# skycrapers/TecoGAN-PyTorch

Measured on AMD Instinct MI355X. Metric: HR frames/sec/GPU at 4xSR 3x134x320 LR; Vid4 PSNR vs reference, higher is better.
Workload: dtype f32; 1 GPU; TecoGAN 4xSR BD generator-only inference (FRNet.infer_sequence) of a synthetic 2140-frame 3x134x320 LR clip -> 3x536x1280 HR uint8, 1 clip/GPU, random-init weights (BASELINE configs[1]); a step = one recurrent frame; parallelism=clip-sharded x1, no data-path collective, launches_per_frame=29

## Files before the change

### include/tecogan_hip.h

```cpp
#ifndef TECOGAN_HIP_H
#define TECOGAN_HIP_H

#include <stddef.h>
#include <stdint.h>

#ifdef __cplusplus
extern "C" {
#endif

typedef void* tg_stream_t;

enum {
  TG_OK = 0,
  TG_E_SHAPE = -1,
  TG_E_ARG = -2,
  TG_E_HIP = -3
};

enum {
  TG_ACT_NONE = 0,
  TG_ACT_RELU = 1,
  TG_ACT_LRELU02 = 2,
  TG_ACT_TANH24 = 3
};

enum {
  TG_UP_NONE = 0,
  TG_UP_BICUBIC = 1,
  TG_UP_BILINEAR = 2
};

#define TG_ABI_MAJOR 2
int tg_version(void);
const char* tg_last_error_string(void);
const char* tg_build_info(void);

int tg_conv3x3_pick_ocb(int cout);
size_t tg_conv3x3_packed_floats(int cin, int cout, int ocb);
int tg_conv3x3_pack(const float* w, float* w_packed, int cin, int cout, int ocb,
                    int transposed, tg_stream_t stream);

int tg_conv3x3_fwd(
    const float* x, int64_t x_nstride, int c1,
    const float* x2, int64_t x2_nstride,
    const float* w_packed, int ocb, const float* bias ,
    const float* res, int64_t res_nstride,
    float* y, int64_t y_nstride,
    int n, int cin, int cout, int h, int w, int act, tg_stream_t stream);

int tg_conv3x3_fwd_phased(const float* x, int64_t x_nstride, const float* w_packed, int ocb,
                          const float* bias, float* y, int64_t y_nstride, int n, int cin,
                          int cout, int h, int w, int act, int tapsel, int cphase,
                          int taps_phase0, int taps_phase1, tg_stream_t stream);
int tg_conv4x4s2_supported(int n, int ci, int co, int h, int w);
size_t tg_conv4x4s2_packed_floats(int ci, int co);
int tg_conv4x4s2_pack(const float* w, float* w_fwd, float* w_dgrad, int ci, int co, tg_stream_t stream);
size_t tg_conv4x4s2_workspace_floats(int n, int ci, int co, int h, int w, int dgrad);
int tg_conv4x4s2_fwd(const float* x, const float* w_fwd, float* y, float* workspace, int n, int ci, int co, int h, int w,
                     tg_stream_t stream);
int tg_conv4x4s2_dgrad(const float* g, const float* w_dgrad, const float* act_y, int act, float* dx, float* workspace,
                       int n, int ci, int co, int h, int w, tg_stream_t stream);
int tg_conv3x3s2_supported(int n, int cin, int cout, int h_out, int w_out);
int tg_conv3x3s2_fwd(const float* x, int64_t x_nstride, const float* w_packed, const float* bias,
                     const float* relu_mask, int64_t mask_nstride, float* y, int64_t y_nstride, int n,
                     int cin, int cout, int h_out, int w_out, int act, tg_stream_t stream);
int tg_conv3x3_fwd_phased_masked(const float* x, int64_t x_nstride, const float* w_packed, int ocb,
                                 const float* bias, const float* relu_mask, int64_t mask_nstride,
                                 float* y, int64_t y_nstride, int n, int cin, int cout, int h, int w,
                                 int act, int tapsel, int cphase, int taps_phase0, int taps_phase1,
                                 tg_stream_t stream);
int tg_conv3x3_phased_pick_ksplit(int n, int cin, int cout, int h, int w, int ocb);
int tg_conv3x3_fwd_phased_splitk(const float* x, int64_t x_nstride, const float* w_packed, int ocb,
                                 const float* bias, float* y, int n, int cin, int cout, int h, int w,
                                 int act, int tapsel, int cphase, int taps_phase0, int taps_phase1,
                                 int ksplit, float* partials, tg_stream_t stream);
int tg_conv3x3_fwd_masked(const float* x, int64_t x_nstride, int c1, const float* x2,
                          int64_t x2_nstride, const float* w_packed, int ocb,
                          const float* bias, const float* res, int64_t res_nstride,
                          const float* relu_mask, int64_t mask_nstride, float* y,
                          int64_t y_nstride, int n, int cin, int cout, int h, int w, int act,
                          tg_stream_t stream);

int64_t tg_conv3x3_wino_packed_floats(int cin, int cout);
int tg_conv3x3_prefers_wino(int n, int cin, int cout, int h, int w);
int tg_pack_conv3x3_wino(const float* w, float* out, int cin, int cout, int transposed,
                         tg_stream_t stream);
int tg_conv3x3_wino_fwd(const float* x, int64_t x_nstride, int c1, const float* x2,
                        int64_t x2_nstride, const float* u_packed, const float* bias,
                        const float* res, int64_t res_nstride, const float* relu_mask,
                        int64_t mask_nstride, float* y, int64_t y_nstride, int n, int cin,
                        int cout, int h, int w, int act, tg_stream_t stream);

typedef struct {
  const float* x; const float* x2; const float* u_packed; const float* bias; const float* res;
  float* y;
  int64_t x_nstride, x2_nstride, res_nstride, y_nstride;
  int c1, cin, act;
} tg_wino_layer;
int64_t tg_conv3x3_wino_chain_flag_ints(int n_layers, int n, int h, int w);
int tg_conv3x3_wino_chain(const tg_wino_layer* layers, int n_layers, int n, int cout, int h, int w,
                          int32_t* flags, int epoch, tg_stream_t stream);

int tg_conv3x3_wino_resident_supported(int n, int cout, int h, int w);
int64_t tg_conv3x3_wino_resident_ws_bytes(int h, int w);
int tg_conv3x3_wino_resident(const tg_wino_layer* layers, int n_layers, int cout, int h, int w,
                             void* workspace, int epoch, tg_stream_t stream);
typedef struct tg_wres_convt {
  const float* u_packed;
  const float* bias;
  float* y;
  int act;
} tg_wres_convt;
size_t tg_conv3x3_wino_resident_ct_floats(void);
int tg_conv3x3_wino_resident_ct_pack(const float* w_iohw, float* out, tg_stream_t stream);
int tg_conv3x3_wino_resident_ct(const tg_wino_layer* layers, int n_layers, int cout, int h, int w,
                                void* workspace, int epoch, const tg_wres_convt* convt, tg_stream_t stream);

typedef struct {
  const float* x; const float* x2; const float* w_packed; const float* bias; const float* res;
  const float* relu_mask;
  float* y;
  int64_t x_nstride, x2_nstride, res_nstride, mask_nstride, y_nstride;
  int c1, cin, cout, act;
} tg_chain_layer;
int64_t tg_conv3x3_chain_flag_ints(int n_layers, int n, int h, int w);
int tg_conv3x3_chain_supported(int n, int h, int w, int cmax);
size_t tg_conv3x3_pack16_floats(void);
int tg_conv3x3_pack16(const float* w, float* w_packed, int cin, int cout, int transposed, tg_stream_t stream);
typedef struct tg_pack_item {
  const float* w;
  float* out;
  int cin, cout, transposed, i_total, i_off;
} tg_pack_item;
size_t tg_conv3x3_chain_packed_floats(int pack_layout, int cin);
int tg_conv3x3_chain_pack(const tg_pack_item* items, int n_items, int pack_layout, tg_stream_t stream);
int tg_conv3x3_chain(const tg_chain_layer* layers, int n_layers, int n, int h, int w, int pack_layout,
                     int32_t* flags, int32_t* err, uint32_t epoch, int poll_limit, tg_stream_t stream);
typedef struct { const float* w; const float* b; } tg_packed_layer;
int tg_srnet_body_fwd(const tg_packed_layer* layers, int pack_layout, int nb, const float* lr, int c_lr,
                      const float* tran, int c_tran, float* acts, int n, int nf, int h, int w, int32_t* flags,
                      int32_t* err, uint32_t epoch, int poll_limit, tg_stream_t stream);
int tg_srnet_body_bwd(const tg_packed_layer* dgrad, int pack_layout, int nb, const float* acts, float* dz,
                      float* d_tran, int c_tran, int n, int nf, int h, int w, int32_t* flags, int32_t* err,
                      uint32_t epoch, int poll_limit, tg_stream_t stream);

size_t tg_wgrad3x3_body_workspace_floats(int nframes, int n_per_frame, int nlayers, int c, int h, int w);
int tg_wgrad3x3_body(const float* const* dz_bases, const float* const* act_bases, int nframes, int64_t layer_stride, int nlayers, float* const* grads, float* workspace,
                     int n_per_frame, int c, int h, int w, int accumulate, tg_stream_t stream);
int tg_wgrad3x3_body_bias(const float* const* dz_bases, const float* const* act_bases, int nframes,
                          int64_t layer_stride, int nlayers, float* const* grads, float* const* dbs,
                          float* workspace, int n_per_frame, int c, int h, int w, int accumulate,
                          tg_stream_t stream);
int tg_bias_grad_body(const float* const* dz_bases, int nframes,
                      int64_t layer_stride, int nlayers, float* const* dbs, int n_per_frame, int c, int hw,
                      tg_stream_t stream);

int tg_conv3x3_pick_ksplit(int n, int cin, int cout, int h, int w);
int tg_conv3x3_splitk_fwd(const float* x, int64_t x_nstride, int c1, const float* x2,
                          int64_t x2_nstride, const float* w_packed, int ocb,
                          const float* bias, float* y, int n, int cin, int cout, int h,
                          int w, int act, int ksplit, float* partials, int pool,
                          tg_stream_t stream);

int tg_convt3x3s2_fwd(const float* x, int64_t x_nstride, const float* w_packed,
                      const float* bias, float* y, int64_t y_nstride, int n,
                      int cin, int cout, int h, int w, int act,
                      tg_stream_t stream);
int tg_convt_pack_wz(const float* w_out_oihw, float* wz, int cz, int nf, tg_stream_t stream);
int tg_convt3x3s2_z_fwd(const float* x, int64_t x_nstride, const float* w_packed,
                        const float* bias, const float* wz, int cz, float* z,
                        int64_t z_nstride, int n, int cin, int cout, int h, int w, int act,
                        tg_stream_t stream);
int tg_convt3x3s2_z_fwd_form(const float* x, int64_t x_nstride, const float* w_packed,
                             const float* bias, const float* wz, int cz, float* z,
                             int64_t z_nstride, int n, int cin, int cout, int h, int w, int act,
                             int form, tg_stream_t stream);
#define TG_CONVT_WINO_FLOATS (16 * 64 * 64)
int tg_convt_pack_wino(const float* w_packed, float* w_wino, int cin, int cout, tg_stream_t stream);
int tg_convt3x3s2_z_wino_fwd(const float* x, int64_t x_nstride, const float* w_wino, const float* bias,
                             const float* wz, int cz, float* z, int64_t z_nstride, int n, int cin, int cout,
                             int h, int w, int act, int split, tg_stream_t stream);
int tg_convout_tail(const float* z, int64_t z_nstride, int cz, const float* bias,
                    const float* up_src, int up_mode, int up_scale, float* y,
                    int64_t y_nstride, uint8_t* u8_out, int n, int h, int w,
                    tg_stream_t stream);
int tg_convout_tail_form(const float* z, int64_t z_nstride, int cz, const float* bias,
                         const float* up_src, int up_mode, int up_scale, float* y,
                         int64_t y_nstride, uint8_t* u8_out, int n, int h, int w, int form,
                         tg_stream_t stream);

int tg_conv3x3_small_fwd(const float* x, int64_t x_nstride, const float* w_oihw,
                         const float* bias, const float* up_src, int up_mode,
                         int up_scale, float* y, int64_t y_nstride, int n,
                         int cin, int cout, int h, int w, int act,
                         tg_stream_t stream);
int tg_conv3x3_small_fwd_u8(const float* x, int64_t x_nstride, const float* w_oihw,
                            const float* bias, const float* up_src, int up_mode,
                            int up_scale, float* y, int64_t y_nstride, uint8_t* u8_out,
                            int n, int cin, int cout, int h, int w, int act,
                            tg_stream_t stream);
int tg_conv3x3_small_can_fuse_u8(const float* x, int64_t x_nstride, const float* y,
                                 int64_t y_nstride, int n, int cin, int h, int w);
int tg_conv3x3_fewin_fwd(const float* x, int64_t x_nstride, const float* w_oihw, const float* relu_mask,
                         int64_t mask_nstride, float* y, int64_t y_nstride, int n, int cin, int cout,
                         int h, int w, tg_stream_t stream);
int tg_conv3x3_small_fwd_res(const float* x, int64_t x_nstride, const float* w_oihw, const float* bias,
                             const float* res, int64_t res_nstride, float* y, int64_t y_nstride, int n,
                             int cin, int cout, int h, int w, int act, tg_stream_t stream);

int tg_flowup_warp_s2d_fwd(const float* lr_flow, int fh, int fw,
                           const float* hr_prev, float* out,
                           int64_t out_nstride, float* hr_flow_out, int n,
                           int c, int h, int w, int scale, int up_mode,
                           tg_stream_t stream);
int tg_copy_ceiling(const void* src, void* dst, int64_t bytes, int blocks, int threads, tg_stream_t stream);

int tg_backward_warp_fwd(const float* x, const float* flow, float* y, int n,
                         int c, int h, int w, tg_stream_t stream);

int tg_space_to_depth(const float* x, float* y, int64_t y_nstride, int n, int c,
                      int h, int w, int scale, tg_stream_t stream);

int tg_upsample_fwd(const float* x, float* y, int nc, int h, int w, int scale,
                    int up_mode, float mul, tg_stream_t stream);

int tg_maxpool2_fwd(const float* x, float* y, int nc, int h, int w,
                    tg_stream_t stream);

int tg_quantize_u8_hwc(const float* x, uint8_t* y, int c, int h, int w,
                       tg_stream_t stream);

int tg_dequantize_u8_hwc(const uint8_t* x, float* y, int n, int c, int h, int w,
                         tg_stream_t stream);

int tg_psnr_sse_u8(const uint8_t* true_hwc, const uint8_t* pred_hwc, uint64_t* sse,
                   int frames, int h, int w, int y_only, tg_stream_t stream);
int tg_luma_u8(const uint8_t* rgb, uint8_t* y, int64_t n, tg_stream_t stream);

int tg_lpips_conv_fwd(const void* x0, const void* x1, int n0, const float* lut, const float* wt,
                      const float* bias, float* y, int n, int cin, int h, int w, int cout, int ks,
                      int stride, int pad, tg_stream_t stream);
int tg_maxpool3s2_fwd(const float* x, float* y, int nc, int h, int w, tg_stream_t stream);
int64_t tg_lpips_head_workspace_bytes(int frames, int h, int w);
int tg_lpips_head(const float* feat_true, const float* feat_pred, const float* lin, int frames, int c,
// ... 210 lines not shown
```

### tecogan-pytorch_amd/_lib.py

```python
import ctypes as C
import os

_HERE = os.path.dirname(os.path.abspath(__file__))
LIB_PATH = os.environ.get('TECOGAN_HIP_LIB') or os.path.join(_HERE, 'libtecogan_hip.so')

TG_OK = 0
ABI_MAJOR = 2
ACT_NONE, ACT_RELU, ACT_LRELU02, ACT_TANH24 = 0, 1, 2, 3
UP_NONE, UP_BICUBIC, UP_BILINEAR = 0, 1, 2
PREC_F32, PREC_F16 = 0, 1

P, I, I64, F, SZ = C.c_void_p, C.c_int, C.c_int64, C.c_float, C.c_size_t


class FrnetCfg(C.Structure):
    _fields_ = [(k, C.c_int) for k in
                ('in_nc', 'out_nc', 'nf', 'nb', 'scale', 'up_mode', 'n', 'h', 'w', 'fnet_only')]


class WinoLayer(C.Structure):
    _fields_ = [('x', C.c_void_p), ('x2', C.c_void_p), ('u_packed', C.c_void_p), ('bias', C.c_void_p),
                ('res', C.c_void_p), ('y', C.c_void_p), ('x_nstride', C.c_int64), ('x2_nstride', C.c_int64),
                ('res_nstride', C.c_int64), ('y_nstride', C.c_int64), ('c1', C.c_int), ('cin', C.c_int),
                ('act', C.c_int)]


class ChainLayer(C.Structure):
    _fields_ = [('x', C.c_void_p), ('x2', C.c_void_p), ('w_packed', C.c_void_p), ('bias', C.c_void_p),
                ('res', C.c_void_p), ('relu_mask', C.c_void_p), ('y', C.c_void_p),
                ('x_nstride', C.c_int64), ('x2_nstride', C.c_int64), ('res_nstride', C.c_int64),
                ('mask_nstride', C.c_int64), ('y_nstride', C.c_int64),
                ('c1', C.c_int), ('cin', C.c_int), ('cout', C.c_int), ('act', C.c_int)]


class PackedLayer(C.Structure):
    _fields_ = [('w', C.c_void_p), ('b', C.c_void_p)]


class PackItem(C.Structure):
    _fields_ = [('w', C.c_void_p), ('out', C.c_void_p), ('cin', C.c_int), ('cout', C.c_int), ('transposed', C.c_int),
                ('i_total', C.c_int), ('i_off', C.c_int)]


class WresConvT(C.Structure):
    _fields_ = [('u_packed', C.c_void_p), ('bias', C.c_void_p), ('y', C.c_void_p), ('act', C.c_int)]


class LayerWeights(C.Structure):
    _fields_ = [('w', C.c_void_p), ('b', C.c_void_p), ('u', C.c_void_p)]


SIGNATURES = {
    'tg_version': (I, []),
    'tg_last_error_string': (C.c_char_p, []),
    'tg_build_info': (C.c_char_p, []),
    'tg_conv3x3_pick_ocb': (I, [I]),
    'tg_conv3x3_packed_floats': (SZ, [I, I, I]),
    'tg_conv3x3_pack': (I, [P, P, I, I, I, I, P]),
    'tg_conv3x3_fwd': (I, [P, I64, I, P, I64, P, I, P, P, I64, P, I64, I, I, I, I, I, I, P]),
    'tg_conv3x3_fwd_phased': (I, [P, I64, P, I, P, P, I64, I, I, I, I, I, I, I, I, I, I, P]),
    'tg_conv3x3_fwd_phased_masked': (I, [P, I64, P, I, P, P, I64, P, I64, I, I, I, I, I, I, I, I, I, I, P]),
    'tg_conv3x3s2_supported': (I, [I, I, I, I, I]),
    'tg_conv3x3s2_fwd': (I, [P, I64, P, P, P, I64, P, I64, I, I, I, I, I, I, P]),
    'tg_conv3x3_fwd_masked': (I, [P, I64, I, P, I64, P, I, P, P, I64, P, I64, P, I64, I, I, I, I, I, I, P]),
    'tg_conv3x3_pick_ksplit': (I, [I, I, I, I, I]),
    'tg_conv3x3_splitk_fwd': (I, [P, I64, I, P, I64, P, I, P, P, I, I, I, I, I, I, I, P, I, P]),
    'tg_convt3x3s2_fwd': (I, [P, I64, P, P, P, I64, I, I, I, I, I, I, P]),
    'tg_convt_pack_wz': (I, [P, P, I, I, P]),
    'tg_convt3x3s2_z_fwd': (I, [P, I64, P, P, P, I, P, I64, I, I, I, I, I, I, P]),
    'tg_convt3x3s2_z_fwd_form': (I, [P, I64, P, P, P, I, P, I64, I, I, I, I, I, I, I, P]),
    'tg_convt_pack_wino': (I, [P, P, I, I, P]),
    'tg_convt3x3s2_z_wino_fwd': (I, [P, I64, P, P, P, I, P, I64, I, I, I, I, I, I, I, P]),
    'tg_convout_tail': (I, [P, I64, I, P, P, I, I, P, I64, P, I, I, I, P]),
    'tg_convout_tail_form': (I, [P, I64, I, P, P, I, I, P, I64, P, I, I, I, I, P]),
    'tg_conv3x3_small_fwd': (I, [P, I64, P, P, P, I, I, P, I64, I, I, I, I, I, I, P]),
    'tg_conv3x3_fewin_fwd': (I, [P, I64, P, P, I64, P, I64, I, I, I, I, I, P]),
    'tg_conv3x3_small_fwd_res': (I, [P, I64, P, P, P, I64, P, I64, I, I, I, I, I, I, P]),
    'tg_conv3x3_small_fwd_u8': (I, [P, I64, P, P, P, I, I, P, I64, P, I, I, I, I, I, I, P]),
    'tg_conv3x3_small_can_fuse_u8': (I, [P, I64, P, I64, I, I, I, I]),
    'tg_flowup_warp_s2d_fwd': (I, [P, I, I, P, P, I64, P, I, I, I, I, I, I, P]),
    'tg_copy_ceiling': (I, [P, P, I64, I, I, P]),
    'tg_backward_warp_fwd': (I, [P, P, P, I, I, I, I, P]),
    'tg_space_to_depth': (I, [P, P, I64, I, I, I, I, I, P]),
    'tg_upsample_fwd': (I, [P, P, I, I, I, I, I, F, P]),
    'tg_maxpool2_fwd': (I, [P, P, I, I, I, P]),
    'tg_quantize_u8_hwc': (I, [P, P, I, I, I, P]),
    'tg_dequantize_u8_hwc': (I, [P, P, I, I, I, I, P]),
    'tg_psnr_sse_u8': (I, [P, P, P, I, I, I, I, P]),
    'tg_luma_u8': (I, [P, P, I64, P]),
    'tg_lpips_conv_fwd': (I, [P, P, I, P, P, P, P, I, I, I, I, I, I, I, I, P]),
    'tg_maxpool3s2_fwd': (I, [P, P, I, I, I, P]),
    'tg_lpips_head_workspace_bytes': (I64, [I, I, I]),
    'tg_lpips_head': (I, [P, P, P, I, I, I, I, P, P, I, P, P]),
    'tg_ssim_workspace_bytes': (I64, [I, I, I]),
    'tg_ssim_y_u8': (I, [P, P, I, I, I, I, I, I, I, I, I, P, P, SZ, P]),
    'tg_psnr_yfloat_partials': (I64, [I, I]),
    'tg_psnr_yfloat_sse_u8': (I, [P, P, I, I, I, I, I, I, I, I, I, P, P]),
    'tg_wgrad3x3_workspace_floats': (SZ, [I, I, I, I, I]),
    'tg_wgrad3x3': (I, [P, I64, P, I64, P, P, I, I, I, I, I, I, I, I, P]),
    'tg_wgrad3x3_multi': (I, [P, P, I, I64, I64, P, P, I, I, I, I, I, I, I, I, P]),
    'tg_wgrad3x3_multi_bias': (I, [P, P, I, I64, I64, P, P, P, I, I, I, I, I, I, I, I, P]),
    'tg_wgrad3x3_multi_phased': (I, [P, P, I, I64, I64, P, P, I, I, I, I, I, I, I, I, I, P]),
    'tg_conv3x3_phased_pick_ksplit': (I, [I, I, I, I, I, I]),
    'tg_conv3x3_fwd_phased_splitk': (I, [P, I64, P, I, P, P, I, I, I, I, I, I, I, I, I, I, I, P, P]),
    'tg_wgrad3x3_convt_workspace_floats': (SZ, [I, I, I, I, I]),
    'tg_wgrad3x3_convt_multi': (I, [P, P, I, P, P, P, I, I, I, I, I, I, P]),
    'tg_bias_grad_multi': (I, [P, I, P, I, I, I, I, P]),
    'tg_act_bwd': (I, [P, P, P, I64, I, P]),
    'tg_bias_grad': (I, [P, P, I, I, I, I, P]),
    'tg_maxpool2_bwd': (I, [P, P, P, I, I, I, P]),
    'tg_upsample_bwd': (I, [P, P, I, I, I, I, I, F, P]),
    'tg_backward_warp_bwd': (I, [P, P, P, P, P, I, I, I, I, P]),
    'tg_backward_warp_bwd_acc': (I, [P, P, P, P, P, I, I, I, I, P]),
    'tg_conv3x3_wino_resident_ct_floats': (SZ, []),
    'tg_conv3x3_wino_resident_ct_pack': (I, [P, P, P]),
    'tg_conv3x3_wino_resident_ct': (I, [P, I, I, I, I, P, I, P, P]),
    'tg_conv4x4s2_supported': (I, [I, I, I, I, I]),
    'tg_conv4x4s2_packed_floats': (SZ, [I, I]),
    'tg_conv4x4s2_pack': (I, [P, P, P, I, I, P]),
    'tg_conv4x4s2_workspace_floats': (SZ, [I, I, I, I, I, I]),
    'tg_conv4x4s2_fwd': (I, [P, P, P, P, I, I, I, I, I, P]),
    'tg_conv4x4s2_dgrad': (I, [P, P, P, I, P, P, I, I, I, I, I, P]),
    'tg_backward_warp_s2d_fwd': (I, [P, P, P, I, I, I, I, I, P]),
    'tg_backward_warp_s2d_bwd': (I, [P, P, P, P, I, P, I, I, I, I, I, P]),
    'tg_depth_to_space': (I, [P, P, I, I, I, I, I, P]),
    'tg_depth_to_space_act_bwd_supported': (I, [P, P, P, I, I]),
    'tg_depth_to_space_act_bwd': (I, [P, P, I, P, I, I, I, I, I, P]),
    'tg_charbonnier': (I, [P, P, I64, F, F, P, F, P, P]),
    'tg_channel_norm': (I, [P, P, P, P, I, I, I64, P]),
    'tg_cosine_loss': (I, [P, P, I, I, I64, F, F, P, F, P, P]),
    'tg_pixel_loss': (I, [P, P, I64, I, F, P, F, P, P]),
    'tg_bce_logits': (I, [P, I64, F, F, P, F, P, P]),
    'tg_lsgan_loss': (I, [P, I64, F, F, P, F, P, P]),
    'tg_adam_step': (I, [P, P, P, P, I64, F, F, F, F, F, I, P]),
    'tg_adam_step_guarded': (I, [P, P, P, P, I64, F, F, F, F, F, I, P, P]),
    'tg_fault_to_slot': (I, [P, P, P]),
    'tg_axpy': (I, [P, P, F, I64, P]),
    'tg_div_scalar': (I, [P, P, F, I64, P]),
    'tg_bn_lrelu_train_fwd': (I, [P, P, P, P, P, F, F, F, P, P, P, I, I, I, P]),
    'tg_bn_lrelu_train_bwd': (I, [P, P, P, P, P, P, F, P, P, P, I, P, I, I, I, P]),
    'tg_bn_local_stats': (I, [P, P, I, I, I, P]),
    'tg_bn_merge_stats': (I, [P, I, F, F, F, P, P, P, P, I, P]),
    'tg_bn_lrelu_apply': (I, [P, P, P, P, P, F, P, I, I, I, P]),
    'tg_bn_lrelu_bwd_reduce': (I, [P, P, P, P, P, F, P, I, I, I, P]),
    'tg_bn_lrelu_bwd_apply': (I, [P, P, P, P, P, P, P, F, F, P, I, I, I, P]),
    'tg_linear1_fwd': (I, [P, P, P, P, I, I, P]),
    'tg_linear1_bwd': (I, [P, P, P, P, P, P, I, I, I, P]),
    'tg_downsample_bd': (I, [P, P, P, I, I, I, I, I, I, P]),
    'tg_conv3x3_wino_packed_floats': (I64, [I, I]),
    'tg_conv3x3_wino_chain_flag_ints': (I64, [I, I, I, I]),
    'tg_conv3x3_wino_chain': (I, [C.POINTER(WinoLayer), I, I, I, I, I, P, I, P]),
    'tg_conv3x3_wino_resident_supported': (I, [I, I, I, I]),
    'tg_conv3x3_wino_resident_ws_bytes': (I64, [I, I]),
    'tg_conv3x3_wino_resident': (I, [C.POINTER(WinoLayer), I, I, I, I, P, I, P]),
    'tg_conv3x3_chain_flag_ints': (I64, [I, I, I, I]),
    'tg_conv3x3_chain_supported': (I, [I, I, I, I]),
    'tg_conv3x3_pack16_floats': (SZ, []),
    'tg_conv3x3_pack16': (I, [P, P, I, I, I, P]),
    'tg_conv3x3_chain_packed_floats': (SZ, [I, I]),
    'tg_conv3x3_chain_pack': (I, [P, I, I, P]),
    'tg_conv3x3_chain': (I, [C.POINTER(ChainLayer), I, I, I, I, I, P, P, C.c_uint32, I, P]),
    'tg_srnet_body_fwd': (I, [C.POINTER(PackedLayer), I, I, P, I, P, I, P, I, I, I, I, P, P, C.c_uint32, I, P]),
    'tg_srnet_body_bwd': (I, [C.POINTER(PackedLayer), I, I, P, P, P, I, I, I, I, I, P, P, C.c_uint32, I, P]),
    'tg_wgrad3x3_body_workspace_floats': (SZ, [I, I, I, I, I, I]),
    'tg_wgrad3x3_body': (I, [P, P, I, I64, I, P, P, I, I, I, I, I, P]),
    'tg_wgrad3x3_body_bias': (I, [P, P, I, I64, I, P, P, P, I, I, I, I, I, P]),
    'tg_bias_grad_body': (I, [P, I, I64, I, P, I, I, I, P]),
    'tg_conv3x3_prefers_wino': (I, [I, I, I, I, I]),
    'tg_pack_conv3x3_wino': (I, [P, P, I, I, I, P]),
    'tg_conv3x3_wino_fwd': (I, [P, I64, I, P, I64, P, P, P, I64, P, I64, P, I64, I, I, I, I, I, I, P]),
    'tg_time_gather': (I, [P, P, P, I, I, I, I64, P]),
    'tg_transpose01': (I, [P, P, I, I, I64, P]),
    'tg_stack_time': (I, [P, I, P, I, I64, P]),
    'tg_index_gather': (I, [P, P, P, I64, I64, I, P]),
    'tg_pingpong_grad': (I, [P, P, I, I, I64, P]),
    'tg_d_assemble_fwd': (I, [P, I, P, P, I, P, I, I, I, I, I, I, I, P]),
    'tg_d_assemble_bwd': (I, [P, P, I, P, I, I, I, I, I, I, I, P]),
    'tg_gather_clips_u8': (I, [P, P, P, P, I, I, I, I, P]),
    'tg_comm_get_unique_id': (I, [P]),
    'tg_comm_init_rank': (I, [P, I, I, C.POINTER(C.c_void_p)]),
    'tg_comm_destroy': (I, [P]),
    'tg_comm_world': (I, [P]),
    'tg_comm_rank': (I, [P]),
    'tg_comm_query': (I, [P, C.POINTER(C.c_int), C.POINTER(C.c_int)]),
    'tg_comm_library_origin': (C.c_char_p, []),
    'tg_allreduce_sum_f32': (I, [P, P, I64, P]),
    'tg_allgather_f32': (I, [P, P, P, I64, P]),
    'tg_frnet_workspace_floats': (SZ, [C.POINTER(FrnetCfg)]),
    'tg_frnet_plan_create': (I, [C.POINTER(FrnetCfg), C.POINTER(LayerWeights), I, P,
                                 C.POINTER(C.c_void_p)]),
    'tg_frnet_plan_destroy': (None, [P]),
    'tg_frnet_plan_chain_status': (I, [P, C.POINTER(C.c_int), C.POINTER(C.c_int)]),
    'tg_frnet_plan_set_chain_poll_limit': (I, [P, I]),
    'tg_frnet_plan_set_chain_rearm': (I, [P, I]),
    'tg_frnet_plan_chain_rearms': (I, [P, P, P]),
    'tg_frnet_step': (I, [P, P, P, P, P, P, P]),
    'tg_frnet_step_phase': (I, [P, I, I, P, P, P, P, P, P]),
    'tg_frnet_plan_launches': (I, [P]),
    'tg_frnet_plan_flow': (P, [P, I]),
    'tg_frnet_step_srnet': (I, [P, P, P, P, P, P, P]),
    'tg_frnet_plan_kinds': (I, []),
    'tg_frnet_kind_name': (C.c_char_p, [I]),
    'tg_frnet_plan_kind_stats': (I, [P, I, C.POINTER(C.c_int), C.POINTER(C.c_double),
                                     C.POINTER(C.c_double)]),
    'tg_frnet_replay': (I, [P, P, P, P, P, C.c_uint, I, P]),
    'tg_frnet_step_masked': (I, [P, P, P, P, P, P, C.c_uint, P]),
    'tg_conv3x3_f16_supported': (I, [I, I, I, I, I]),
    'tg_conv3x3_f16_packed_halves': (SZ, [I, I]),
    'tg_conv3x3_f16_act_halves': (I64, [I, I, I]),
    'tg_conv3x3_f16_pack_weights': (I, [P, I, I, I, P, P]),
    'tg_conv3x3_f16_pack_input': (I, [P, I64, I, P, I64, I, P, I, I, I, P]),
    'tg_conv3x3_f16_fwd': (I, [P, P, P, P, P, I, I, I, I, I, I, P]),
    'tg_convt3x3s2_f16_fwd': (I, [P, P, P, P, I64, I, I, I, I, I, I, P]),
    'tg_frnet_f16_workspace_bytes': (SZ, [C.POINTER(FrnetCfg)]),
    'tg_frnet_plan_set_precision': (I, [P, I, C.POINTER(LayerWeights), I, P]),
    'tg_frnet_plan_precision': (I, [P]),
}

_lib = None


class TecoganHipError(RuntimeError):
    pass


def lib():
    global _lib
    if _lib is None:
        if not os.path.isfile(LIB_PATH):
            raise TecoganHipError(
                f'{LIB_PATH} not found: build it with '
                f'`bash {os.path.join(_HERE, "csrc", "build.sh")}` '
                '(hipcc --offload-arch=gfx950).  There is no CPU/ATen fallback.')
        import torch
        handle = C.CDLL(LIB_PATH)
        handle.tg_version.restype = I
        if handle.tg_version() // 100 != ABI_MAJOR:
            raise TecoganHipError(f'{LIB_PATH}: ABI {handle.tg_version()} but this binding is written for '
                                  f'major {ABI_MAJOR} (include/tecogan_hip.h TG_ABI_MAJOR): rebuild the library')
        for name, (res, args) in SIGNATURES.items():
            fn = getattr(handle, name)
            fn.restype = res
            fn.argtypes = args
        _lib = handle
    return _lib


def check(rc, what):
    if rc != TG_OK:
        msg = lib().tg_last_error_string().decode('utf-8', 'replace')
        raise TecoganHipError(f'{what} failed (code {rc}): {msg}')
```

### tecogan-pytorch_amd/csrc/tg_api.hip

```cpp
#include <new>
#include <vector>

#include "tg_common.h"

namespace tg {
static thread_local char g_err[512] = "ok";
void set_error(const char* fmt, ...) {
  va_list ap;
  va_start(ap, fmt);
  vsnprintf(g_err, sizeof(g_err), fmt, ap);
  va_end(ap);
}
}

extern "C" int tg_version(void) { return TG_ABI_MAJOR * 100 + 1; }
extern "C" const char* tg_last_error_string(void) { return tg::g_err; }

#ifndef TG_BUILD_FLAGS_STR
#define TG_BUILD_FLAGS_STR "unknown (not built by csrc/build.sh)"
#endif
#ifndef TG_FILE_FLAGS_STR
#define TG_FILE_FLAGS_STR ""
#endif
namespace tg { int wres_lab_bits(); }
// ... 119 lines not shown
  off[5] = o; o += (c->scale == 4) ? sr * align64(n * c->nf * 16 * hw) : 0;
  off[6] = o; o += sr * align64(fnet_partial_floats(c));
  off[7] = o; o += align64(n * 64 * hw);
  off[8] = o; o += align64(n * 64 * hw);
  off[9] = o; o += align64(fnet_partial_floats(c));
  off[10] = o; o += align64(n * 2 * hw);
  off[11] = o; o += sr * (2048 + TG_CONVT_WINO_FLOATS);
  off[12] = o;
  o += sr * align64((size_t)CHAIN_MAX_LAYERS * n * ((c->h + 1) / 2) * ((c->w + 31) / 32) + 16);
  off[13] = o;
  {
    const int64_t rb = (sr && n == 1) ? tg::conv3x3_wino_resident_ws_bytes(c->h, c->w) : 0;
    o += align64((size_t)(rb + 3) / 4);
  }
  off[14] = o;
}

static int cfg_ok(const tg_frnet_cfg* c) {
  return c && c->in_nc == 3 && c->out_nc >= 1 && c->out_nc <= 4 && c->nf >= 1 && c->nf <= 64 &&
         c->nb >= 0 && (c->scale == 2 || c->scale == 4) &&
         (c->up_mode == TG_UP_BICUBIC || c->up_mode == TG_UP_BILINEAR) && c->n >= 1 &&
         c->h >= 8 && c->w >= 8;
}

extern "C" size_t tg_frnet_workspace_floats(const tg_frnet_cfg* cfg) {
  if (!cfg_ok(cfg)) return 0;
  size_t off[15];
  carve(cfg, off);
  return off[14];
}

extern "C" int tg_frnet_plan_create(const tg_frnet_cfg* cfg, const tg_layer_weights* layers,
                                    int n_layers, float* workspace, tg_frnet_plan** out) {
  TG_REQUIRE(cfg && layers && workspace && out, TG_E_ARG, "frnet_plan_create: null pointer");
  TG_REQUIRE(cfg_ok(cfg), TG_E_SHAPE,
             "frnet_plan_create: unsupported cfg (in_nc=3, out_nc<=4, nf<=64, scale 2|4, h,w>=8)");
  int nup = cfg->scale == 4 ? 2 : 1;
  int need = 14 + 1 + 2 * cfg->nb + nup + 1;
  TG_REQUIRE(n_layers == need, TG_E_ARG, "frnet_plan_create: %d layers given, %d expected",
             n_layers, need);
  for (int i = 0; i < n_layers; ++i)
    TG_REQUIRE(layers[i].w && layers[i].b, TG_E_ARG, "frnet_plan_create: layer %d null", i);
  tg_frnet_plan* p = new (std::nothrow) tg_frnet_plan();
  TG_REQUIRE(p, TG_E_ARG, "frnet_plan_create: out of host memory");
  p->cfg = *cfg;
  p->L.assign(layers, layers + n_layers);
  size_t off[15];
  carve(cfg, off);
  p->f16 = false; p->f16_ready = false; p->HWT = p->HA = p->HB = nullptr;
  p->WZ = workspace + off[11]; p->wz_ready = false;
  p->WA = p->WZ + 2048; p->wa_ready = false;
  p->RESWS = workspace + off[13]; p->res_ready = false;
  p->CHAINF = reinterpret_cast<int32_t*>(workspace + off[12]); p->chain_ready = false; p->epoch = 0; p->chain_layers = 0;
  p->chain_err = nullptr; p->chain_disabled = false; p->chain_faults = 0; p->chain_poll_limit = tg::TG_CHAIN_POLL_LIMIT_DEFAULT;
  p->rearm_first = 64; p->rearm_wait = 0; p->clean_frames = 0; p->rearms = 0; p->rearm_fence = nullptr; p->fence_set = false;
  if (!cfg->fnet_only) {
    void* hp = nullptr;
    if (hipHostMalloc(&hp, 64, hipHostMallocMapped | hipHostMallocCoherent) == hipSuccess && hp) {
      p->chain_err = static_cast<int32_t*>(hp);
      for (int i = 0; i < 16; ++i) p->chain_err[i] = 0;
    } else {
      (void)hipGetLastError();
    }
  }
  p->FA = workspace + off[7]; p->FB = workspace + off[8]; p->FPART = workspace + off[9];
  p->FLOW2 = workspace + off[10];
  p->PART = workspace + off[6];
  p->A = workspace + off[0]; p->B = workspace + off[1]; p->FLOW = workspace + off[2];
  p->S2D = workspace + off[3]; p->U1 = workspace + off[4];
  p->U2 = cfg->scale == 4 ? workspace + off[5] : nullptr;
  p->fh = cfg->h / 8 * 8; p->fw = cfg->w / 8 * 8;
  account(p);
  *out = p;
  return TG_OK;
}

extern "C" void tg_frnet_plan_destroy(tg_frnet_plan* plan) {
  if (!plan) return;
  if (plan->chain_err) (void)hipHostFree(plan->chain_err);
  if (plan->rearm_fence) (void)hipEventDestroy(plan->rearm_fence);
  delete plan;
}
extern "C" int tg_frnet_plan_launches(const tg_frnet_plan* plan) { return plan ? plan->launches : 0; }

enum {
  K_CONV64_R2 = 0,
  K_CONV64_R4 = 1,
  K_CONV32 = 2,
  K_CONVT = 3,
  K_SMALL = 4,
  K_WARP = 5,
  K_POOL = 6,
  K_UPSAMPLE = 7,
  K_QUANT = 8,
  K_FINAL = 9,
  K_CONV64_KS = 10,
  K_CONVT_Z = 11,
  K_TAIL = 12,
  K_CONV_ONESHOT = 13,
  K_CONV_WINO = 14,
  K_WINO_CHAIN = 15,
  K_WINO_RES = 16,
  K_F16_PACK = 17,
  K_F16_CONV = 18,
  K_F16_CONVT = 19,
  K_COUNT = 20
};

static bool hr_fuse_enabled() {
  static const int v = TG_LAB_ENV("TG_HR_FUSE", 1);
  return v != 0;
}
static bool convtz_wino_enabled() {
  static const int v = TG_LAB_ENV("TG_CONVTZ_WINO", 1);
  return v != 0;
}
static bool chain_wanted(long long ntile) {
  static const int v = [] { const char* e = getenv("TG_WINO_CHAIN"); return e && *e ? atoi(e) : -1; }();
  if (v >= 0) return v != 0;
  return ntile > 768 && ntile <= 3000;
}
static bool resident_wanted(bool layer_prefers_wino) {
  static const int v = [] { const char* e = getenv("TG_WINO_RES"); return e && *e ? atoi(e) : -1; }();
  return v >= 0 ? v != 0 : layer_prefers_wino;
}
static bool plan_u8_ok(const tg_frnet_plan* p) {
  if (p->f16 && p->cfg.scale == 2) return p->cfg.n == 1;
  return p->cfg.n == 1 || (hr_fuse_enabled() && p->cfg.out_nc <= 3 && p->cfg.nf <= 64);
}

static int step_impl(tg_frnet_plan* p, const float* lr_curr, const float* lr_prev,
                     const float* hr_prev, float* hr_out, uint8_t* u8_out, tg_stream_t st,
                     unsigned mask, bool dry, int phases, int slot, const float* flow_ext) {
  const tg_frnet_cfg& c = p->cfg;
  float* const flow_buf = flow_ext ? const_cast<float*>(flow_ext) : (slot ? p->FLOW2 : p->FLOW);
  bool active = (phases & 1) != 0;
  float* part_buf = p->FPART;
  const int n = c.n, h = c.h, w = c.w, s = c.scale;
  const int64_t hw = (int64_t)h * w;
  int li = 0;
  float *A = p->FA, *B = p->FB;
  int rc = TG_OK;
  if (!dry && (phases & 2) && mask == 0xFFFFFFFFu) chain_rearm_tick(p, st);
  auto go = [&](int kind, double flops, double bytes, auto&& fn) {
    if (rc != TG_OK) return;
    if (dry) {
      p->st_launch[kind] += 1; p->st_flops[kind] += flops; p->st_bytes[kind] += bytes;
      return;
    }
    if (active && (mask & (1u << kind))) rc = fn();
  };
  auto conv = [&](const float* x, int64_t xns, int c1, const float* x2, int64_t x2ns, int cin,
                  int cout, int hh, int ww, int act, const float* res, int64_t rns, float* y,
                  int64_t yns, bool pool = false, float* pool_tmp = nullptr) {
    const tg_layer_weights lw = p->L[li++];
    int ocb = tg_conv3x3_pick_ocb(cout);
    int kind = ocb == 32 ? K_CONV32
                         : (tg::conv3x3_rows_per_wg(ocb, (long long)n * hh * ww) == 4 ? K_CONV64_R4
                                                                                       : K_CONV64_R2);
    double px = (double)n * hh * ww;
    double fl = 2.0 * cin * 9 * cout * px;
    double by = 4.0 * px * (cin + cout + (res ? cout : 0)) + 4.0 * 9 * cin * cout;
    if (lw.u && tg_conv3x3_prefers_wino(n, cin, cout, hh, ww)) {
      float* yw = pool ? pool_tmp : y;
      go(K_CONV_WINO, fl, by, [&] {
        return tg::conv3x3_wino_launch(x, xns, c1, x2, x2ns, lw.u, lw.b, res, rns, nullptr, 0, yw,
                                       pool ? (int64_t)cout * hh * ww : yns, n, cin, cout, hh, ww, act, st);
      });
      if (pool)
        go(K_POOL, 0, 4.0 * n * cout * (hh * ww + (hh / 2) * (ww / 2)),
           [&] { return tg_maxpool2_fwd(yw, y, n * cout, hh, ww, st); });
      return;
    }
    int ks = res ? 1 : tg_conv3x3_pick_ksplit(n, cin, cout, hh, ww);
    if (ks == 1 && kind == K_CONV64_R2 && tg::conv3x3_uses_wg_ksplit(n, cin, cout, hh, ww))
      kind = tg::conv3x3_uses_oneshot(n, cin, cout, hh, ww) ? K_CONV_ONESHOT : K_CONV64_KS;
    if (ks > 1) {
      go(kind, fl, by, [&] {
        return tg::conv3x3_splitk_conv(x, xns, c1, x2, x2ns, lw.w, ocb, n, cin, cout, hh, ww, ks,
                                       part_buf, st);
      });
      go(K_FINAL, 0, 4.0 * px * cout * (ks + 1), [&] {
        return tg::conv3x3_splitk_finalize(part_buf, ks, lw.b, act, pool ? 1 : 0, y, n, cout, hh, ww,
                                           st);
      });
      return;
    }
    float* yc = pool ? pool_tmp : y;
    go(kind, fl, by, [&] {
      return tg_conv3x3_fwd(x, xns, c1, x2, x2ns, lw.w, ocb, lw.b, res, rns, yc,
                            pool ? (int64_t)cout * hh * ww : yns, n, cin, cout, hh, ww, act, st);
    });
    if (pool)
      go(K_POOL, 0, 4.0 * n * cout * (hh * ww + (hh / 2) * (ww / 2)),
         [&] { return tg_maxpool2_fwd(yc, y, n * cout, hh, ww, st); });
  };
  int hh = h, ww = w;
  const int enc[3] = {32, 64, 128};
  int cin = 2 * c.in_nc;
  const float* src = nullptr;
  for (int e = 0; e < 3; ++e) {
    int co = enc[e];
    if (e == 0)
      conv(lr_curr, c.in_nc * hw, c.in_nc, lr_prev, c.in_nc * hw, cin, co, hh, ww, TG_ACT_LRELU02,
           nullptr, 0, A, (int64_t)co * hh * ww);
    else
      conv(src, (int64_t)cin * hh * ww, cin, nullptr, 0, cin, co, hh, ww, TG_ACT_LRELU02, nullptr,
           0, A, (int64_t)co * hh * ww);
    conv(A, (int64_t)co * hh * ww, co, nullptr, 0, co, co, hh, ww, TG_ACT_LRELU02, nullptr, 0, A,
         (int64_t)co * (hh / 2) * (ww / 2), true, B);
    hh /= 2; ww /= 2; cin = co;
    float* t = A; A = B; B = t;
    src = B;
  }
  const int dec[3] = {256, 128, 64};
  for (int d = 0; d < 3; ++d) {
    int co = dec[d];
    conv(src, (int64_t)cin * hh * ww, cin, nullptr, 0, cin, co, hh, ww, TG_ACT_LRELU02, nullptr, 0,
         A, (int64_t)co * hh * ww);
    conv(A, (int64_t)co * hh * ww, co, nullptr, 0, co, co, hh, ww, TG_ACT_LRELU02, nullptr, 0, B,
         (int64_t)co * hh * ww);
    {
      float *pi = B, *po = A; int ph = hh, pw = ww;
      go(K_UPSAMPLE, 0, 4.0 * n * co * ph * pw * 5.0,
         [&] { return tg_upsample_fwd(pi, po, n * co, ph, pw, 2, TG_UP_BILINEAR, 1.0f, st); });
    }
    hh *= 2; ww *= 2; cin = co;
    float* t = A; A = B; B = t;
    src = B;
  }
  conv(src, (int64_t)cin * hh * ww, cin, nullptr, 0, cin, 32, hh, ww, TG_ACT_LRELU02, nullptr, 0, A,
       (int64_t)32 * hh * ww);
  {
    const tg_layer_weights lw = p->L[li++];
    float* ai = A; int fh_ = hh, fw_ = ww;
    go(K_SMALL, 2.0 * 32 * 9 * 2 * n * fh_ * fw_, 4.0 * n * fh_ * fw_ * 34, [&] {
      return tg_conv3x3_small_fwd(ai, (int64_t)32 * fh_ * fw_, lw.w, lw.b, nullptr, TG_UP_NONE, 1,
                                  flow_buf, (int64_t)2 * fh_ * fw_, n, 32, 2, fh_, fw_,
                                  TG_ACT_TANH24, st);
    });
  }
  active = (phases & 2) != 0;
  part_buf = p->PART;
  const int s2dc = s * s * c.in_nc;
  go(K_WARP, 0,
     4.0 * n * ((double)c.in_nc * s * s * hw * 2 + 2.0 * p->fh * p->fw), [&] {
       return tg_flowup_warp_s2d_fwd(flow_buf, p->fh, p->fw, hr_prev, p->S2D, s2dc * hw, nullptr, n,
                                     c.in_nc, h, w, s, c.up_mode, st);
     });
  A = p->A; B = p->B;
  const int nf = c.nf;
  const bool in_wino = p->L[li].u && tg_conv3x3_prefers_wino(n, c.in_nc + s2dc, nf, h, w);
  const int skip = in_wino ? 0 : 1;
  const int nchain = 1 + 2 * c.nb - skip;
  bool chain = p->chain_err && !p->chain_disabled && nf <= 64 && nchain >= 2 && nchain <= CHAIN_MAX_LAYERS &&
               chain_wanted((long long)n * tg::cdiv(h, 2) * tg::cdiv(w, 32)) &&
               tg_conv3x3_prefers_wino(n, nf, nf, h, w);
  for (int i = skip; i < 1 + 2 * c.nb && chain; ++i) chain = p->L[li + i].u != nullptr;
  bool resident = p->chain_err && !p->chain_disabled && n == 1 && nchain >= 2 && nchain <= CHAIN_MAX_LAYERS &&
                  resident_wanted(tg_conv3x3_prefers_wino(n, nf, nf, h, w) != 0) && (skip || c.in_nc + s2dc <= 64) && tg::conv3x3_wino_resident_ok(n, nf, h, w);
  for (int i = skip; i < 1 + 2 * c.nb && resident; ++i) resident = p->L[li + i].u != nullptr && p->L[li + i].b != nullptr;
  if (resident) chain = true;
  bool ct_fold = false;
  if (p->f16) {
    const int nbody = 1 + 2 * c.nb;
    const size_t wstep = tg_conv3x3_f16_packed_halves(64, 64);
    if (!dry && !p->f16_ready && (phases & 2)) {
      for (int k = 0; k <= nbody && rc == TG_OK; ++k)
        rc = tg_conv3x3_f16_pack_weights(p->HL[k].w, k == 0 ? c.in_nc + s2dc : nf, nf, k == nbody ? 1 : 0,
                                         p->HWT + k * wstep, st);
      p->f16_ready = rc == TG_OK;
    }
    const double px = (double)n * h * w;
    const double lfl = 2.0 * nf * 9 * nf * px, lby = 2.0 * px * 2 * nf + 2.0 * 9 * nf * nf;
    uint16_t *HA = p->HA, *HB = p->HB;
    go(K_F16_PACK, 0, px * (4.0 * (c.in_nc + s2dc) + 2.0 * 64), [&] {
      return tg_conv3x3_f16_pack_input(lr_curr, c.in_nc * hw, c.in_nc, p->S2D, s2dc * hw, s2dc, HB, n, h, w, st);
    });
    auto hconv = [&](int k, const uint16_t* xin, const uint16_t* res, uint16_t* y, int act) {
      go(K_F16_CONV, lfl, lby + (res ? 2.0 * px * nf : 0), [&] {
        return tg_conv3x3_f16_fwd(xin, p->HWT + k * wstep, p->HL[k].b, res, y, n, 64, 64, h, w, act, st);
      });
    };
    hconv(0, HB, nullptr, HA, TG_ACT_RELU);
    for (int b = 0; b < c.nb; ++b) {
      hconv(1 + 2 * b, HA, nullptr, HB, TG_ACT_RELU);
      hconv(2 + 2 * b, HB, HA, HA, TG_ACT_NONE);
    }
    go(K_F16_CONVT, lfl, 2.0 * px * nf + 4.0 * px * nf * 4 + 2.0 * 9 * nf * nf, [&] {
      return tg_convt3x3s2_f16_fwd(HA, p->HWT + nbody * wstep, p->HL[nbody].b, p->U1, (int64_t)nf * 4 * hw, n, 64, 64,
                                   h, w, TG_ACT_RELU, st);
    });
    li += nbody;
    ct_fold = true;
  } else if (chain) {
    if (skip)
      conv(lr_curr, c.in_nc * hw, c.in_nc, p->S2D, s2dc * hw, c.in_nc + s2dc, nf, h, w, TG_ACT_RELU,
           nullptr, 0, A, nf * hw);
    tg_wino_layer cl[CHAIN_MAX_LAYERS];
    double fl = 0, by = 0;
    const double px = (double)n * h * w;
    for (int k = 0; k < nchain; ++k) {
      const int i = k + skip;
      const tg_layer_weights lw = p->L[li + k];
      tg_wino_layer& d = cl[k];
      const bool first = i == 0, conv2 = !first && (i % 2 == 0);
      d.x = first ? lr_curr : (conv2 ? B : A);
      d.x2 = first ? p->S2D : nullptr;
      d.u_packed = lw.u; d.bias = lw.b;
      d.res = conv2 ? A : nullptr;
      d.y = (first || conv2) ? A : B;
      d.x_nstride = first ? c.in_nc * hw : nf * hw;
      d.x2_nstride = first ? s2dc * hw : 0;
      d.res_nstride = nf * hw; d.y_nstride = nf * hw;
      d.c1 = first ? c.in_nc : nf;
      d.cin = first ? c.in_nc + s2dc : nf;
      d.act = conv2 ? TG_ACT_NONE : TG_ACT_RELU;
      fl += 2.0 * d.cin * 9 * nf * px;
      by += 4.0 * px * (d.cin + nf + (conv2 ? nf : 0)) + 4.0 * 9 * d.cin * nf;
    }
    li += nchain;
    p->chain_layers = nchain;
    if (resident) {
      ct_fold = s == 4 && p->L[li].u != nullptr && p->L[li].b != nullptr;
      if (ct_fold) { fl += 2.0 * nf * 9 * nf * px; by += 4.0 * px * nf * 4.0 + 4.0 * 9 * nf * nf; }
      go(K_WINO_RES, fl, by, [&] {
        if (!p->res_ready) {
          if (hipMemsetAsync(p->RESWS, 0, (size_t)tg::conv3x3_wino_resident_ws_bytes(h, w), (hipStream_t)st) != hipSuccess)
            return tg::check_launch("wino_resident workspace memset");
          p->res_ready = true;
        }
        if (++p->epoch == 0) p->epoch = 1;
        tg_wres_convt ct{p->L[li].u, p->L[li].b, p->U1, TG_ACT_RELU};
        return tg::conv3x3_wino_resident_launch(cl, nchain, nf, h, w, p->RESWS, p->chain_err, p->epoch << 5,
                                                p->chain_poll_limit, st, ct_fold ? &ct : nullptr);
      });
    } else
    go(K_WINO_CHAIN, fl, by, [&] {
      if (!p->chain_ready) {
        const size_t ints = (size_t)tg_conv3x3_wino_chain_flag_ints(nchain, n, h, w);
        if (hipMemsetAsync(p->CHAINF, 0, ints * sizeof(int32_t), (hipStream_t)st) != hipSuccess)
          return tg::check_launch("wino_chain flags memset");
        p->chain_ready = true;
      }
      if (++p->epoch == 0) p->epoch = 1;
      return tg::conv3x3_wino_chain_launch(cl, nchain, n, nf, h, w, p->CHAINF, p->chain_err, p->epoch,
                                           p->chain_poll_limit, st);
    });
  } else {
    conv(lr_curr, c.in_nc * hw, c.in_nc, p->S2D, s2dc * hw, c.in_nc + s2dc, nf, h, w, TG_ACT_RELU,
         nullptr, 0, A, nf * hw);
    for (int b = 0; b < c.nb; ++b) {
      conv(A, nf * hw, nf, nullptr, 0, nf, nf, h, w, TG_ACT_RELU, nullptr, 0, B, nf * hw);
      conv(B, nf * hw, nf, nullptr, 0, nf, nf, h, w, TG_ACT_NONE, A, nf * hw, A, nf * hw);
    }
  }
  const bool fuse = hr_fuse_enabled() && c.out_nc <= 3 && nf <= 64 && !(p->f16 && s == 2);
  const tg_layer_weights lw_up1 = p->L[li++];
  const tg_layer_weights lw_up2 = s == 4 ? p->L[li++] : tg_layer_weights{nullptr, nullptr, nullptr};
  const tg_layer_weights lw_out = p->L[li++];
  const double hpx = (double)n * s * s * hw;
  if (fuse) {
    if (!dry && !p->wz_ready && (phases & 2)) {
      rc = tg_convt_pack_wz(lw_out.w, p->WZ, c.out_nc, nf, st);
      p->wz_ready = rc == TG_OK;
    }
    float* zbuf = s == 4 ? p->U2 : p->U1;
    const int zh = s * h / 2, zw = s * w / 2;
    const float* zin = A;
    if (s == 4) {
      float* ai = A;
      if (!ct_fold)
        go(K_CONVT, 2.0 * nf * 9 * nf * n * hw, 4.0 * n * hw * nf * 5.0, [&] {
          return tg_convt3x3s2_fwd(ai, nf * hw, lw_up1.w, lw_up1.b, p->U1, nf * 4 * hw, n, nf, nf, h, w,
                                   TG_ACT_RELU, st);
        });
      zin = p->U1;
    }
    const tg_layer_weights lw_last = s == 4 ? lw_up2 : lw_up1;
    const bool wino = convtz_wino_enabled() && nf == 64;
    if (wino && !dry && !p->wa_ready && (phases & 2) && rc == TG_OK) {
      rc = tg_convt_pack_wino(lw_last.w, p->WA, nf, nf, st);
      p->wa_ready = rc == TG_OK;
    }
    if (dry && (wino ? tg::convt_z_wino_split_rule(n, zh, zw, -1) : tg::convt_z_split_rule(n, zh, zw, -1)))
// ... 198 lines not shown
```

### tecogan-pytorch_amd/csrc/tg_common.h

```cpp
#pragma once
#include <hip/hip_runtime.h>
#include <stdarg.h>
#include <stdint.h>
#include <stdio.h>

#include <stdlib.h>

#include "../../include/tecogan_hip.h"

#ifndef TG_LAB
#define TG_LAB 0
#endif
#if TG_LAB
#define TG_LAB_ENV(name, dflt) ([] { const char* e_ = getenv(name); return e_ ? atoi(e_) : (dflt); }())
#else
#define TG_LAB_ENV(name, dflt) (dflt)
#endif

namespace tg {

void set_error(const char* fmt, ...);

inline int check_launch(const char* what) {
  hipError_t e = hipGetLastError();
  if (e != hipSuccess) {
    set_error("%s: %s", what, hipGetErrorString(e));
    return TG_E_HIP;
  }
  return TG_OK;
}

#define TG_REQUIRE(cond, code, ...) \
  do {                              \
    if (!(cond)) {                  \
      tg::set_error(__VA_ARGS__);   \
      return (code);                \
    }                               \
  } while (0)

bool convt_z_split_rule(int n, int h, int w, int form);
bool convt_z_wino_split_rule(int n, int h, int w, int split);

int conv3x3_splitk_conv(const float* x, int64_t x_nstride, int c1, const float* x2,
                        int64_t x2_nstride, const float* w_packed, int ocb, int n, int cin,
                        int cout, int h, int w, int ksplit, float* partials, tg_stream_t stream);
int conv3x3_splitk_finalize(const float* partials, int ksplit, const float* bias, int act, int pool,
                            float* y, int n, int cout, int h, int w, tg_stream_t stream);

inline int conv3x3_rows_per_wg(int ocb, long long pixels) {
  if (ocb == 32) return 4;
  return pixels >= 200000 ? 4 : 2;
}

__host__ __device__ inline int cdiv(int a, int b) { return (a + b - 1) / b; }

bool conv3x3_uses_wg_ksplit(int n, int cin, int cout, int h, int w);
bool conv3x3_uses_oneshot(int n, int cin, int cout, int h, int w);
int conv3x3_wino_launch(const float* x, int64_t x_ns, int c1, const float* x2, int64_t x2_ns, const float* u,
                        const float* bias, const float* res, int64_t res_ns, const float* mask,
                        int64_t mask_ns, float* y, int64_t y_ns, int n, int cin, int cout, int h, int w,
                        int act, tg_stream_t stream);

constexpr int TG_CHAIN_POLL_LIMIT_DEFAULT = 1 << 21;
int conv3x3_wino_chain_launch(const tg_wino_layer* layers, int n_layers, int n, int cout, int h, int w,
                              int32_t* flags, int32_t* err, unsigned epoch, int poll_limit, tg_stream_t stream);

bool conv3x3_wino_resident_ok(int n, int cout, int h, int w);
int64_t conv3x3_wino_resident_ws_bytes(int h, int w);
int conv3x3_wino_resident_launch(const tg_wino_layer* layers, int n_layers, int cout, int h, int w, void* ws,
                                 int32_t* err, unsigned base, int poll_limit, tg_stream_t stream,
                                 const tg_wres_convt* ct = nullptr);

typedef float f32x16 __attribute__((ext_vector_type(16)));
typedef float f32x4 __attribute__((ext_vector_type(4)));

constexpr int CK = 8;

__device__ __forceinline__ float apply_act(float v, int act) {
  switch (act) {
    case TG_ACT_RELU: return v > 0.f ? v : 0.f;
    case TG_ACT_LRELU02: return v >= 0.f ? v : v * 0.2f;
    case TG_ACT_TANH24: return tanhf(v) * 24.f;
    default: return v;
  }
}

__device__ __forceinline__ float act_slope(int act) {
  return act == TG_ACT_RELU ? 0.f : (act == TG_ACT_LRELU02 ? 0.2f : 1.f);
}

inline float act_slope_host(int act) {
  return act == TG_ACT_RELU ? 0.f : (act == TG_ACT_LRELU02 ? 0.2f : 1.f);
}

__device__ __forceinline__ void bicubic_w(int d, int f, float k[4]) {
  const float a = -0.75f;
  float s = (float)d / (float)f;
  float s2 = s * s, s3 = s2 * s;
  k[0] = ((0.f * 1.f + a * s) + (-2.f * a) * s2) + a * s3;
  k[1] = ((1.f * 1.f + 0.f * s) + (-(a + 3.f)) * s2) + (a + 2.f) * s3;
  k[2] = ((0.f * 1.f + (-a) * s) + (2.f * a + 3.f) * s2) + (-(a + 2.f)) * s3;
  k[3] = ((0.f * 1.f + 0.f * s) + a * s2) + (-a) * s3;
}

__device__ __forceinline__ void bilinear_src(int dst, int scale, int in_size,
                                             int& i0, int& i1, float& l0,
                                             float& l1) {
  float src = ((float)dst + 0.5f) * (1.0f / (float)scale) - 0.5f;
  src = src < 0.f ? 0.f : src;
  i0 = (int)floorf(src);
  i1 = i0 + 1 < in_size ? i0 + 1 : in_size - 1;
  l1 = src - (float)i0;
  l0 = 1.0f - l1;
}

__device__ __forceinline__ float linspace_m1p1(int i, int n, float step) {
  const int mirror = n - 1 - i;
  const int j = i < mirror ? i : mirror;
  const unsigned flip = (unsigned)(n / 2 - 1 - i) & 0x80000000u;
  return __builtin_bit_cast(float, __builtin_bit_cast(unsigned, __builtin_fmaf(step, (float)j, -1.0f)) ^ flip);
}

__device__ __forceinline__ float warp_coord(int i, int n, float flow) {
  float step = 2.0f / (float)(n - 1);
  float half = (float)(n - 1) / 2.0f;
  float g = linspace_m1p1(i, n, step) + flow / half;
  float p = (g + 1.0f) * half;
  p = __builtin_fmaxf(p, 0.f);
  p = __builtin_fminf(p, (float)(n - 1));
  return p;
}

}
```

### tecogan-pytorch_amd/csrc/tg_conv3x3_mfma.hip

```cpp
#include "tg_common.h"
#include <cstdlib>

namespace tg {

constexpr int TW = 32;
constexpr int PW = TW + 2;
constexpr int RS = 34;

struct Conv3x3Args {
  const float* x;
  const float* x2;
  const float* wpk;
  const float* bias;
  const float* res;
  float* y;
  long long x_ns, x2_ns, res_ns, y_ns;
  int c1, cin, cout, h, w, act;
  int tiles_x, tiles_y, nchunk, nocg;
  int ksplit;
  float* part;
  long long part_ss;
  int vec_ok;
  long long* dbg;
  int nblocks;
  const float* mask;
  long long mask_ns;
  int tapsel, cphase;
  unsigned char rowsets[2];
};

__global__ void pack3x3_kernel(const float* __restrict__ w, float* __restrict__ out,
                               int cin, int cout, int ocb, int nchunk, int nocg,
                               int transposed) {
  int total = nocg * nchunk * 9 * CK * ocb;
  for (int i = blockIdx.x * blockDim.x + threadIdx.x; i < total;
       i += gridDim.x * blockDim.x) {
    int j = i & 3;
    int t = i >> 2;
    int o = t % ocb; t /= ocb;
    int half = t & 1; t >>= 1;
    int tap = t % 9; t /= 9;
    int ch = t % nchunk;
    int g = t / nchunk;
    int oc = g * ocb + o, ci = ch * CK + 4 * half + j;
    float v = 0.f;
    if (oc < cout && ci < cin) {
      if (transposed == 2) v = w[((size_t)ci * cout + oc) * 9 + (8 - tap)];
      else if (transposed == 1) v = w[((size_t)ci * cout + oc) * 9 + tap];
      else v = w[((size_t)oc * cin + ci) * 9 + tap];
    }
    out[i] = v;
  }
}

__device__ __forceinline__ float buf_load(__amdgpu_buffer_rsrc_t r, unsigned voff) {
  return __builtin_bit_cast(float, __builtin_amdgcn_raw_buffer_load_b32(r, (int)voff, 0, 0));
}

constexpr unsigned OOB = 0x80000000u;

enum { TAPS_ALL = 0, TAPS_01 = 1, TAPS_12 = 2, TAPS_1 = 3 };
__host__ __device__ constexpr int taps_first(int code) { return (code == TAPS_12 || code == TAPS_1) ? 1 : 0; }
__host__ __device__ constexpr int taps_count(int code) { return code == TAPS_ALL ? 3 : (code == TAPS_1 ? 1 : 2); }

template <int NT, int OCB, int RY, int RX>
__device__ __forceinline__ void chunk_taps(const float* si, const float* sw, f32x16 (&acc)[NT]) {
  constexpr int Y0 = taps_first(RY), NY = taps_count(RY), X0 = taps_first(RX), NX = taps_count(RX);
  constexpr int N = NY * NX;
  f32x4 bq[2], aq[2][NT];
  auto fetch = [&](int i, int slot) {
    const int ky = Y0 + i / NX, kx = X0 + i % NX;
    bq[slot] = *reinterpret_cast<const f32x4*>(si + (ky * 2 * 34 + kx) * 4);
#pragma unroll
    for (int t = 0; t < NT; ++t)
      aq[slot][t] = *reinterpret_cast<const f32x4*>(sw + (ky * 3 + kx) * (2 * OCB * 4) + t * 128);
  };
  fetch(0, 0);
#pragma unroll
  for (int i = 0; i < N; ++i) {
    const int cur = i & 1;
    if (i + 1 < N) fetch(i + 1, cur ^ 1);
#pragma unroll
    for (int kk = 0; kk < 4; ++kk) {
#pragma unroll
      for (int t = 0; t < NT; ++t)
        acc[t] = __builtin_amdgcn_mfma_f32_32x32x2f32(aq[cur][t][kk], bq[cur][kk], acc[t], 0, 0, 0);
    }
  }
}

template <int NT, int OCB>
__device__ __forceinline__ void chunk_taps_sel(int ry, int rx, const float* si, const float* sw,
                                               f32x16 (&acc)[NT]) {
  switch (ry * 4 + rx) {
    case TAPS_01 * 4 + TAPS_01: chunk_taps<NT, OCB, TAPS_01, TAPS_01>(si, sw, acc); break;
    case TAPS_01 * 4 + TAPS_12: chunk_taps<NT, OCB, TAPS_01, TAPS_12>(si, sw, acc); break;
    case TAPS_12 * 4 + TAPS_01: chunk_taps<NT, OCB, TAPS_12, TAPS_01>(si, sw, acc); break;
    case TAPS_12 * 4 + TAPS_12: chunk_taps<NT, OCB, TAPS_12, TAPS_12>(si, sw, acc); break;
    case TAPS_01 * 4 + TAPS_1: chunk_taps<NT, OCB, TAPS_01, TAPS_1>(si, sw, acc); break;
    case TAPS_1 * 4 + TAPS_01: chunk_taps<NT, OCB, TAPS_1, TAPS_01>(si, sw, acc); break;
    case TAPS_1 * 4 + TAPS_1: chunk_taps<NT, OCB, TAPS_1, TAPS_1>(si, sw, acc); break;
    case TAPS_12 * 4 + TAPS_1: chunk_taps<NT, OCB, TAPS_12, TAPS_1>(si, sw, acc); break;
    case TAPS_1 * 4 + TAPS_12: chunk_taps<NT, OCB, TAPS_1, TAPS_12>(si, sw, acc); break;
    default: chunk_taps<NT, OCB, TAPS_ALL, TAPS_ALL>(si, sw, acc); break;
  }
}

template <int WM, int WN, int NT, bool DUAL, int ABL = 0, int KS = 1>
__global__ __launch_bounds__(WM* WN* KS * 64) void conv3x3_mfma_kernel(Conv3x3Args a) {
  static_assert(KS == 1 || KS == 2, "wave groups over K: one or two");
  constexpr int NTHREADS = WM * WN * KS * 64;
  constexpr int OCB = WN * NT * 32;
  constexpr int PH = WM + 2;
  constexpr int IN_ITEMS = PH * 2 * PW;
  constexpr int IN_FLOATS = PH * 2 * RS * 4;
  constexpr int W_FLOATS = 9 * CK * OCB;
  constexpr int I_PER_T = (IN_ITEMS + NTHREADS - 1) / NTHREADS;

  extern __shared__ __attribute__((aligned(16))) float smem[];
  float* s_in = smem;
  float* s_w = smem + 2 * KS * IN_FLOATS;

  const int tid = threadIdx.x;
  const int lane = tid & 63;
  const int wave = tid >> 6;
  const int wm = wave % WM;
  const int wn = (wave / WM) % WN;
  const int wk = wave / (WM * WN);
  auto bufof = [](int ch) { return KS == 1 ? (ch & 1) : ((ch >> 1) & 1); };

  int b = blockIdx.x;
  if (a.nblocks > 0) {
    const int per = (a.nblocks + 7) >> 3;
    b = (b & 7) * per + (b >> 3);
    if (b >= a.nblocks) return;
  }
  const int tx = b % a.tiles_x; b /= a.tiles_x;
  const int ty = b % a.tiles_y; b /= a.tiles_y;
  const int ocg = b % a.nocg; b /= a.nocg;
  const int ks = b % a.ksplit;
  const int n = b / a.ksplit;
  const int x0 = tx * TW, y0 = ty * WM;
  const int hw = a.h * a.w;
  const int ch_begin = (int)((long long)ks * a.nchunk / a.ksplit);
  const int ch_end = (int)((long long)(ks + 1) * a.nchunk / a.ksplit);

  unsigned voff[I_PER_T];
  int lds_item[I_PER_T];
#pragma unroll
  for (int i = 0; i < I_PER_T; ++i) {
    int q = tid + i * NTHREADS;
    int r = q / (2 * PW), rem = q - r * (2 * PW);
    int hf = rem / PW, col = rem - hf * PW;
    int gy = y0 - 1 + r, gx = x0 - 1 + col;
    bool ok = q < IN_ITEMS && gy >= 0 && gy < a.h && gx >= 0 && gx < a.w;
    voff[i] = ok ? (unsigned)((4 * hf * hw + gy * a.w + gx) * 4) : OOB;
    lds_item[i] = q < IN_ITEMS ? ((r * 2 + hf) * RS + col) * 4 : -1;
  }
  const __amdgpu_buffer_rsrc_t rs1 = __builtin_amdgcn_make_buffer_rsrc(
      const_cast<float*>(a.x + (long long)n * a.x_ns), 0, a.c1 * hw * 4, 0x00020000);
  const __amdgpu_buffer_rsrc_t rs2 = __builtin_amdgcn_make_buffer_rsrc(
      const_cast<float*>(DUAL ? a.x2 + (long long)n * a.x2_ns : a.x), 0,
      DUAL ? (a.cin - a.c1) * hw * 4 : 0, 0x00020000);
  const unsigned plane = (unsigned)hw * 4u;

  const f32x4* wsrc =
      reinterpret_cast<const f32x4*>(a.wpk + (size_t)ocg * a.nchunk * W_FLOATS);

  f32x4 rin[KS][I_PER_T];

  auto load_chunk = [&](int ch) {
    if (!((ABL & 32) && ch != ch_begin))
#pragma unroll
    for (int k = 0; k < KS; ++k) {
      const unsigned cbase = (unsigned)((ch + k) * CK) * plane;
#pragma unroll
      for (int i = 0; i < I_PER_T; ++i) {
#pragma unroll
        for (int j = 0; j < 4; ++j) {
          unsigned o1 = voff[i] + cbase + (unsigned)j * plane;
          float v = buf_load(rs1, o1);
          if (DUAL) v += buf_load(rs2, o1 - (unsigned)a.c1 * plane);
          rin[k][i][j] = v;
        }
      }
    }
    if ((ABL & 64) && ch != ch_begin) return;
    constexpr int PIECES = W_FLOATS * 4 / 1024;
    constexpr int NWAVES = NTHREADS / 64;
    const char* src = reinterpret_cast<const char*>(wsrc + (size_t)ch * (W_FLOATS / 4)) + lane * 16;
    char* dst = reinterpret_cast<char*>(s_w + bufof(ch) * KS * W_FLOATS);
    const int valid = (ch_end - ch < KS ? ch_end - ch : KS) * PIECES;
#pragma unroll
    for (int i = 0; i < (KS * PIECES + NWAVES - 1) / NWAVES; ++i) {
      int piece = wave + i * NWAVES;
      if (piece < valid)
        __builtin_amdgcn_global_load_lds(
            (const __attribute__((address_space(1))) void*)(src + piece * 1024),
            (__attribute__((address_space(3))) void*)(dst + piece * 1024), 16, 0, 0);
    }
  };
  auto store_chunk = [&](int buf) {
#pragma unroll
    for (int k = 0; k < KS; ++k) {
      float* si = s_in + (buf * KS + k) * IN_FLOATS;
#pragma unroll
      for (int i = 0; i < I_PER_T; ++i)
        if (lds_item[i] >= 0) *reinterpret_cast<f32x4*>(si + lds_item[i]) = rin[k][i];
    }
  };

  f32x16 acc[NT];
#pragma unroll
  for (int t = 0; t < NT; ++t)
#pragma unroll
    for (int r = 0; r < 16; ++r) acc[t][r] = 0.f;

  const int lh = lane >> 5, ll = lane & 31;
  const int b_off = ((wm * 2 + lh) * RS + ll) * 4;
  const int a_off = (lh * OCB + wn * (NT * 32) + ll) * 4;

  long long tk0 = 0, tk1 = 0, t_mfma = 0, t_sync = 0, t_issue = 0;
  if constexpr (ABL & 16) tk0 = clock64();
  load_chunk(ch_begin);
  store_chunk(bufof(ch_begin));
  __syncthreads();
  if constexpr (ABL & 16) tk1 = clock64();

  for (int ch = ch_begin; ch < ch_end; ch += KS) {
    long long ta = 0, tb = 0, tc = 0;
    if constexpr (ABL & 16) ta = clock64();
    const int buf = bufof(ch);
    const bool more = (ch + KS < ch_end) && !(ABL & 1);
    if (more) load_chunk(ch + KS);

    if constexpr (ABL & 16) tb = clock64();
    const float* si = s_in + (buf * KS + wk) * IN_FLOATS + b_off;
    const float* sw = s_w + (buf * KS + wk) * W_FLOATS + a_off;
    if (KS == 1 || ch + wk < ch_end) {
    if (a.tapsel) {
      const int ph = a.tapsel == 1 ? ((ch + wk) * CK) / a.cphase : (ocg * OCB) / a.cphase;
      chunk_taps_sel<NT, OCB>(a.rowsets[(ph >> 1) & 1], a.rowsets[ph & 1], si, sw, acc);
    } else {
    f32x4 bq[2], aq[2][NT];
    bq[0] = *reinterpret_cast<const f32x4*>(si);
#pragma unroll
    for (int t = 0; t < NT; ++t) aq[0][t] = *reinterpret_cast<const f32x4*>(sw + t * 128);
#pragma unroll
    for (int tap = 0; tap < 9; ++tap) {
      const int cur = tap & 1, nxt = cur ^ 1;
      if (tap + 1 < 9 && !(ABL & 8)) {
        const int ky = (tap + 1) / 3, kx = (tap + 1) % 3;
        bq[nxt] = *reinterpret_cast<const f32x4*>(si + (ky * 2 * RS + kx) * 4);
#pragma unroll
        for (int t = 0; t < NT; ++t)
          aq[nxt][t] = *reinterpret_cast<const f32x4*>(sw + (tap + 1) * (2 * OCB * 4) + t * 128);
      }
#pragma unroll
      for (int kk = 0; kk < 4; ++kk) {
#pragma unroll
        for (int t = 0; t < NT; ++t)
          acc[t] = __builtin_amdgcn_mfma_f32_32x32x2f32(aq[cur][t][kk], bq[cur][kk], acc[t], 0, 0, 0);
      }
    }
    }
    }
    if constexpr (ABL & 16) {
      asm volatile("s_nop 0" ::"v"(acc[0][0]));
      tc = clock64();
    }
    if (more) store_chunk(buf ^ 1);
    if (!(ABL & 2)) __syncthreads();
    if constexpr (ABL & 16) {
      long long td = clock64();
      t_issue += tb - ta; t_mfma += tc - tb; t_sync += td - tc;
    }
  }
  if constexpr (ABL & 16) {
    if (a.dbg && tid == 0) {
      long long* d = a.dbg + (long long)blockIdx.x * 8;
      d[0] = tk0; d[1] = tk1 - tk0; d[2] = t_issue; d[3] = t_mfma; d[4] = t_sync; d[5] = clock64();
      d[6] = __builtin_amdgcn_s_getreg((20 << 0) | (0 << 6) | ((4 - 1) << 11));
    }
  }

  if constexpr (KS == 2) {
    float* red = smem;
    if (wk == 1) {
#pragma unroll
      for (int t = 0; t < NT; ++t)
#pragma unroll
        for (int r = 0; r < 16; ++r)
          red[(((wn * WM + wm) * NT + t) * 16 + r) * 64 + lane] = acc[t][r];
    }
    __syncthreads();
    if (wk == 0) {
#pragma unroll
      for (int t = 0; t < NT; ++t)
#pragma unroll
        for (int r = 0; r < 16; ++r)
          acc[t][r] += red[(((wn * WM + wm) * NT + t) * 16 + r) * 64 + lane];
    }
    __syncthreads();
  }
  const bool do_ep = wk == 0;
  const int px = x0 + ll, py = y0 + wm;
  const bool inimg = px < a.w && py < a.h;
  const long long opix = (long long)py * a.w + px;
  const int ocb0 = ocg * OCB + wn * (NT * 32) + 4 * lh;
  if (a.ksplit > 1) {
    if (inimg) {
      float* pb = a.part + (long long)ks * a.part_ss + (long long)n * a.cout * hw + opix;
#pragma unroll
      for (int t = 0; t < NT; ++t)
#pragma unroll
        for (int r = 0; r < 16; ++r) {
          int oc = ocb0 + t * 32 + (r & 3) + 8 * (r >> 2);
          if (oc < a.cout) pb[(long long)oc * hw] = acc[t][r];
        }
    }
    return;
  }
  const float slope = act_slope(a.act);
  if (a.vec_ok) {
    constexpr int ES = 36;
    float* ep = smem + (wave % (WM * WN)) * (NT * 32 * ES);
    if (do_ep) {
#pragma unroll
      for (int t = 0; t < NT; ++t)
#pragma unroll
        for (int r = 0; r < 16; ++r)
          ep[(t * 32 + (r & 3) + 8 * (r >> 2) + 4 * lh) * ES + ll] = acc[t][r];
    }
    __syncthreads();
    const int ocw = ocg * OCB + wn * (NT * 32);
    if (do_ep && py < a.h) {
#pragma unroll
      for (int j = 0; j < NT * 4; ++j) {
        int idx4 = j * 64 + lane;
        int ol = idx4 >> 3, p4 = (idx4 & 7) * 4;
        int oc = ocw + ol;
        int gx = x0 + p4;
        if (oc < a.cout && gx < a.w) {
          f32x4 v = *reinterpret_cast<const f32x4*>(ep + ol * ES + p4);
          float bb = a.bias ? a.bias[oc] : 0.f;
          long long off = (long long)oc * hw + (long long)py * a.w + gx;
          f32x4 rr = {0.f, 0.f, 0.f, 0.f};
          if (a.res) rr = *reinterpret_cast<const f32x4*>(a.res + (long long)n * a.res_ns + off);
          f32x4 mm = {1.f, 1.f, 1.f, 1.f};
          if (a.mask) mm = *reinterpret_cast<const f32x4*>(a.mask + (long long)n * a.mask_ns + off);
#pragma unroll
          for (int e = 0; e < 4; ++e) {
            float q = v[e] + bb;
            q = (q >= 0.f ? q : q * slope + 0.f) + rr[e];
            v[e] = mm[e] > 0.f ? q : 0.f;
          }
          *reinterpret_cast<f32x4*>(a.y + (long long)n * a.y_ns + off) = v;
        }
      }
    }
    return;
  }
  if (!do_ep) return;
  float bv[NT][16], rv[NT][16];
  unsigned dead[NT];
#pragma unroll
  for (int t = 0; t < NT; ++t) dead[t] = 0u;
#pragma unroll
  for (int t = 0; t < NT; ++t)
#pragma unroll
    for (int r = 0; r < 16; ++r) {
      int oc = ocb0 + t * 32 + (r & 3) + 8 * (r >> 2);
      int occ = oc < a.cout ? oc : a.cout - 1;
      bv[t][r] = a.bias ? a.bias[occ] : 0.f;
      rv[t][r] = (a.res && inimg) ? a.res[(long long)n * a.res_ns + opix + (long long)occ * hw] : 0.f;
      if (a.mask && inimg && a.mask[(long long)n * a.mask_ns + opix + (long long)occ * hw] <= 0.f)
        dead[t] |= 1u << r;
    }
  if (inimg) {
    float* yb = a.y + (long long)n * a.y_ns + opix;
#pragma unroll
    for (int t = 0; t < NT; ++t)
#pragma unroll
      for (int r = 0; r < 16; ++r) {
        int oc = ocb0 + t * 32 + (r & 3) + 8 * (r >> 2);
        float v = acc[t][r] + bv[t][r];
        v = (v >= 0.f ? v : v * slope + 0.f) + rv[t][r];
        if (dead[t] & (1u << r)) v = 0.f;
        if (oc < a.cout && (!(ABL & 4) || v == 12345.678f)) yb[(long long)oc * hw] = v;
      }
  }
}

template <bool DUAL>
__global__ __launch_bounds__(512) void conv3x3_oneshot_kernel(Conv3x3Args a) {
  constexpr int OCB = 64, KG = 4, MAXCH = 8;
  constexpr int IN_FLOATS = 3 * 2 * RS * 4;
  constexpr int ITEMS_PER_CH = 3 * 2 * PW;
  constexpr int W_VEC4 = 9 * CK * OCB / 4;
  extern __shared__ __attribute__((aligned(16))) float smem[];
  float* s_in = smem;
  float* red = smem + MAXCH * IN_FLOATS;

  const int tid = threadIdx.x, lane = tid & 63, wave = tid >> 6;
  const int wn = wave & 1, wk = wave >> 1;
  const int lh = lane >> 5, ll = lane & 31;
  int b = blockIdx.x;
  const int tx = b % a.tiles_x; b /= a.tiles_x;
  const int ty = b % a.tiles_y;
  const int n = b / a.tiles_y;
  const int x0 = tx * TW, y0 = ty;
  const int hw = a.h * a.w;
  const unsigned plane = (unsigned)hw * 4u;
  const int nchunk = a.nchunk;
  const __amdgpu_buffer_rsrc_t rs1 = __builtin_amdgcn_make_buffer_rsrc(
      const_cast<float*>(a.x + (long long)n * a.x_ns), 0, a.c1 * hw * 4, 0x00020000);
  const __amdgpu_buffer_rsrc_t rs2 = __builtin_amdgcn_make_buffer_rsrc(
      const_cast<float*>(DUAL ? a.x2 + (long long)n * a.x2_ns : a.x), 0,
      DUAL ? (a.cin - a.c1) * hw * 4 : 0, 0x00020000);

  const int cpw = (nchunk + KG - 1) / KG;
  const int c0 = wk * cpw;
  const f32x4* wlane = reinterpret_cast<const f32x4*>(a.wpk) + (lh * OCB + wn * 32 + ll);
  f32x4 aw[2][9];
#pragma unroll
  for (int ci = 0; ci < 2; ++ci) {
    const int c = c0 + ci;
    const bool on = ci < cpw && c < nchunk;
#pragma unroll
    for (int tap = 0; tap < 9; ++tap) {
      f32x4 v = {0.f, 0.f, 0.f, 0.f};
      if (on) v = wlane[(size_t)c * W_VEC4 + tap * (2 * OCB)];
      aw[ci][tap] = v;
    }
  }
  const int total = nchunk * ITEMS_PER_CH;
  constexpr int MAXQ = (MAXCH * ITEMS_PER_CH + 511) / 512;
#pragma unroll
  for (int k0 = 0; k0 < MAXQ; k0 += 2) {
    f32x4 v[2];
#pragma unroll
    for (int k = 0; k < 2; ++k) {
      const int q = tid + (k0 + k) * 512;
      const int ch = q / ITEMS_PER_CH, rem = q - ch * ITEMS_PER_CH;
      const int r = rem / (2 * PW), rem2 = rem - r * (2 * PW);
      const int hf = rem2 / PW, col = rem2 - hf * PW;
      const int gy = y0 - 1 + r, gx = x0 - 1 + col;
      const bool ok = q < total && gy >= 0 && gy < a.h && gx >= 0 && gx < a.w;
      const unsigned base = ok ? (unsigned)(((ch * CK + 4 * hf) * hw + gy * a.w + gx) * 4) : OOB;
#pragma unroll
      for (int j = 0; j < 4; ++j) {
        const unsigned o1 = base + (unsigned)j * plane;
        float t = buf_load(rs1, o1);
        if (DUAL) t += buf_load(rs2, o1 - (unsigned)a.c1 * plane);
        v[k][j] = t;
      }
    }
#pragma unroll
    for (int k = 0; k < 2; ++k) {
      const int q = tid + (k0 + k) * 512;
      const int ch = q / ITEMS_PER_CH, rem = q - ch * ITEMS_PER_CH;
      const int r = rem / (2 * PW), rem2 = rem - r * (2 * PW);
      const int hf = rem2 / PW, col = rem2 - hf * PW;
      if (q < total) *reinterpret_cast<f32x4*>(s_in + ch * IN_FLOATS + ((r * 2 + hf) * RS + col) * 4) = v[k];
    }
  }
  __syncthreads();

  f32x16 acc;
#pragma unroll
  for (int r = 0; r < 16; ++r) acc[r] = 0.f;
#pragma unroll
  for (int ci = 0; ci < 2; ++ci) {
    const int c = c0 + ci;
    if (ci < cpw && c < nchunk) {
      const float* si = s_in + c * IN_FLOATS + (lh * RS + ll) * 4;
// ... 23 lines not shown
    for (int r = 0; r < 16; ++r) ep[(wn * 32 + (r & 3) + 8 * (r >> 2) + 4 * lh) * ES + ll] = acc[r];
  }
  __syncthreads();
  const float slope = act_slope(a.act);
  const int py = y0;
  if (a.vec_ok) {
    const int oc = tid >> 3, p4 = (tid & 7) * 4;
    const int gx = x0 + p4;
    if (oc < a.cout && gx < a.w) {
      f32x4 v = *reinterpret_cast<const f32x4*>(ep + oc * ES + p4);
      const float bb = a.bias ? a.bias[oc] : 0.f;
      const long long off = (long long)oc * hw + (long long)py * a.w + gx;
      f32x4 rr = {0.f, 0.f, 0.f, 0.f};
      if (a.res) rr = *reinterpret_cast<const f32x4*>(a.res + (long long)n * a.res_ns + off);
      f32x4 mm = {1.f, 1.f, 1.f, 1.f};
      if (a.mask) mm = *reinterpret_cast<const f32x4*>(a.mask + (long long)n * a.mask_ns + off);
#pragma unroll
      for (int e = 0; e < 4; ++e) {
        float q = v[e] + bb;
        q = (q >= 0.f ? q : q * slope + 0.f) + rr[e];
        v[e] = mm[e] > 0.f ? q : 0.f;
      }
      *reinterpret_cast<f32x4*>(a.y + (long long)n * a.y_ns + off) = v;
    }
  } else {
    for (int i = tid; i < 64 * TW; i += 512) {
      const int oc = i >> 5, p = i & 31;
      const int gx = x0 + p;
      if (oc < a.cout && gx < a.w) {
        const long long off = (long long)oc * hw + (long long)py * a.w + gx;
        float q = ep[oc * ES + p] + (a.bias ? a.bias[oc] : 0.f);
        q = (q >= 0.f ? q : q * slope + 0.f) + (a.res ? a.res[(long long)n * a.res_ns + off] : 0.f);
        if (a.mask && a.mask[(long long)n * a.mask_ns + off] <= 0.f) q = 0.f;
        a.y[(long long)n * a.y_ns + off] = q;
      }
    }
  }
}

constexpr int RS2 = 2 * TW + 2;
__global__ __launch_bounds__(512) void conv3x3s2_oneshot_kernel(Conv3x3Args a) {
  constexpr int OCB = 64, KG = 4, MAXCH = 8;
  constexpr int IN_FLOATS = 3 * 2 * RS2 * 4;
  constexpr int ITEMS_PER_CH = 3 * 2 * RS2;
  constexpr int W_VEC4 = 9 * CK * OCB / 4;
  extern __shared__ __attribute__((aligned(16))) float smem[];
  float* s_in = smem;
  float* red = smem + MAXCH * IN_FLOATS;
  const int tid = threadIdx.x, lane = tid & 63, wave = tid >> 6;
  const int wn = wave & 1, wk = wave >> 1;
  const int lh = lane >> 5, ll = lane & 31;
  int b = blockIdx.x;
  const int tx = b % a.tiles_x; b /= a.tiles_x;
  const int ty = b % a.tiles_y;
  const int n = b / a.tiles_y;
  const int x0 = tx * TW, y0 = ty;
  const int hw = a.h * a.w;
  const int ih = 2 * a.h, iw = 2 * a.w, ihw = ih * iw;
  const unsigned plane = (unsigned)ihw * 4u;
  const int nchunk = a.nchunk;
  const __amdgpu_buffer_rsrc_t rs1 = __builtin_amdgcn_make_buffer_rsrc(
      const_cast<float*>(a.x + (long long)n * a.x_ns), 0, a.cin * ihw * 4, 0x00020000);
  const int cpw = (nchunk + KG - 1) / KG;
  const int c0 = wk * cpw;
  const f32x4* wlane = reinterpret_cast<const f32x4*>(a.wpk) + (lh * OCB + wn * 32 + ll);
  f32x4 aw[2][9];
#pragma unroll
  for (int ci = 0; ci < 2; ++ci) {
    const int c = c0 + ci;
    const bool on = ci < cpw && c < nchunk;
#pragma unroll
    for (int tap = 0; tap < 9; ++tap) {
      f32x4 v = {0.f, 0.f, 0.f, 0.f};
      if (on) v = wlane[(size_t)c * W_VEC4 + tap * (2 * OCB)];
      aw[ci][tap] = v;
    }
  }
  const int total = nchunk * ITEMS_PER_CH;
  constexpr int MAXQ = (MAXCH * ITEMS_PER_CH + 511) / 512;
#pragma unroll
  for (int k0 = 0; k0 < MAXQ; k0 += 2) {
    f32x4 v[2];
#pragma unroll
    for (int k = 0; k < 2; ++k) {
      const int q = tid + (k0 + k) * 512;
      const int ch = q / ITEMS_PER_CH, rem = q - ch * ITEMS_PER_CH;
      const int r = rem / (2 * RS2), rem2 = rem - r * (2 * RS2);
      const int hf = rem2 / RS2, col = rem2 - hf * RS2;
      const int gy = 2 * y0 - 1 + r, gx = 2 * x0 - 1 + col;
      const bool ok = (k0 + k) < MAXQ && q < total && gy >= 0 && gy < ih && gx >= 0 && gx < iw;
      const unsigned base = ok ? (unsigned)(((ch * CK + 4 * hf) * ihw + gy * iw + gx) * 4) : OOB;
#pragma unroll
      for (int j = 0; j < 4; ++j) v[k][j] = buf_load(rs1, base + (unsigned)j * plane);
    }
#pragma unroll
    for (int k = 0; k < 2; ++k) {
      const int q = tid + (k0 + k) * 512;
      const int ch = q / ITEMS_PER_CH, rem = q - ch * ITEMS_PER_CH;
      const int r = rem / (2 * RS2), rem2 = rem - r * (2 * RS2);
      const int hf = rem2 / RS2, col = rem2 - hf * RS2;
      if ((k0 + k) < MAXQ && q < total) *reinterpret_cast<f32x4*>(s_in + ch * IN_FLOATS + ((r * 2 + hf) * RS2 + col) * 4) = v[k];
    }
  }
  __syncthreads();
  f32x16 acc;
#pragma unroll
  for (int r = 0; r < 16; ++r) acc[r] = 0.f;
#pragma unroll
  for (int ci = 0; ci < 2; ++ci) {
    const int c = c0 + ci;
    if (ci < cpw && c < nchunk) {
      const float* si = s_in + c * IN_FLOATS + (lh * RS2 + 2 * ll) * 4;
#pragma unroll
      for (int tap = 0; tap < 9; ++tap) {
        const int ky = tap / 3, kx = tap % 3;
        const f32x4 bq = *reinterpret_cast<const f32x4*>(si + (ky * 2 * RS2 + kx) * 4);
#pragma unroll
        for (int kk = 0; kk < 4; ++kk)
          acc = __builtin_amdgcn_mfma_f32_32x32x2f32(aw[ci][tap][kk], bq[kk], acc, 0, 0, 0);
      }
    }
  }
  if (wk > 0) {
#pragma unroll
    for (int r = 0; r < 16; ++r) red[((wn * (KG - 1) + wk - 1) * 16 + r) * 64 + lane] = acc[r];
  }
  __syncthreads();
  constexpr int ES = 36;
  float* ep = smem;
  if (wk == 0) {
#pragma unroll
    for (int g = 0; g < KG - 1; ++g)
#pragma unroll
      for (int r = 0; r < 16; ++r) acc[r] += red[((wn * (KG - 1) + g) * 16 + r) * 64 + lane];
#pragma unroll
    for (int r = 0; r < 16; ++r) ep[(wn * 32 + (r & 3) + 8 * (r >> 2) + 4 * lh) * ES + ll] = acc[r];
  }
  __syncthreads();
  const float slope = act_slope(a.act);
  for (int i = tid; i < 64 * TW; i += 512) {
    const int oc = i >> 5, p = i & 31;
    const int gx = x0 + p;
    if (oc < a.cout && gx < a.w) {
      const long long off = (long long)oc * hw + (long long)y0 * a.w + gx;
      float q = ep[oc * ES + p] + (a.bias ? a.bias[oc] : 0.f);
      q = (q >= 0.f ? q : q * slope + 0.f) + (a.res ? a.res[(long long)n * a.res_ns + off] : 0.f);
      if (a.mask && a.mask[(long long)n * a.mask_ns + off] <= 0.f) q = 0.f;
      a.y[(long long)n * a.y_ns + off] = q;
    }
  }
}


template <int WM, int WN, int NT, int KS = 1>
static int launch_conv(const Conv3x3Args& a0, int n, hipStream_t stream) {
  Conv3x3Args a = a0;
  a.vec_ok = (a.w % 4 == 0) && ((uintptr_t)a.y % 16 == 0) && (a.y_ns % 4 == 0) &&
             (!a.res || (((uintptr_t)a.res % 16 == 0) && (a.res_ns % 4 == 0))) &&
             (!a.mask || (((uintptr_t)a.mask % 16 == 0) && (a.mask_ns % 4 == 0)));
  constexpr int OCB = WN * NT * 32;
  a.tiles_x = cdiv(a.w, TW);
  a.tiles_y = cdiv(a.h, WM);
  a.nocg = cdiv(a.cout, OCB);
  a.nchunk = cdiv(a.cin, CK);
  size_t lds = 2 * KS * (size_t)((WM + 2) * 2 * RS * 4 + 9 * CK * OCB) * sizeof(float);
  if (a.ksplit < 1) a.ksplit = 1;
  TG_REQUIRE(KS == 1 || a.ksplit == 1, TG_E_ARG, "conv3x3: in-workgroup K split excludes ksplit");
  if (KS > 1) {
    static bool attr_set = false;
    if (!attr_set) {
      (void)hipFuncSetAttribute(reinterpret_cast<const void*>(
                              conv3x3_mfma_kernel<WM, WN, NT, true, 0, KS>),
                          hipFuncAttributeMaxDynamicSharedMemorySize, (int)lds);
      (void)hipFuncSetAttribute(reinterpret_cast<const void*>(
                              conv3x3_mfma_kernel<WM, WN, NT, false, 0, KS>),
                          hipFuncAttributeMaxDynamicSharedMemorySize, (int)lds);
      attr_set = true;
    }
  }
  long long blocks = (long long)a.tiles_x * a.tiles_y * a.nocg * n * a.ksplit;
  TG_REQUIRE(blocks > 0 && blocks < (1ll << 31), TG_E_SHAPE, "conv3x3: grid %lld", blocks);
  static const int xcd_env = TG_LAB_ENV("TG_CONV_XCD", -1);
  const bool xcd = xcd_env >= 0 ? xcd_env != 0 : blocks >= 512;
  a.nblocks = xcd ? (int)blocks : 0;
  const unsigned grid = xcd ? (unsigned)(8 * ((blocks + 7) / 8)) : (unsigned)blocks;
  if (a.x2)
    hipLaunchKernelGGL((conv3x3_mfma_kernel<WM, WN, NT, true, 0, KS>),
                       dim3(grid), dim3(WM * WN * KS * 64), lds, stream, a);
  else
    hipLaunchKernelGGL((conv3x3_mfma_kernel<WM, WN, NT, false, 0, KS>),
                       dim3(grid), dim3(WM * WN * KS * 64), lds, stream, a);
  return check_launch("conv3x3_mfma");
}

__global__ void splitk_finalize_kernel(const float* __restrict__ part, int S, long long part_ss,
                                       const float* __restrict__ bias, float slope, int pool,
                                       float* __restrict__ y, int n, int c, int h, int w) {
  const int oh = pool ? h / 2 : h, ow = pool ? w / 2 : w;
  const long long total = (long long)n * c * oh * ow;
  for (long long i = (long long)blockIdx.x * blockDim.x + threadIdx.x; i < total;
       i += (long long)gridDim.x * blockDim.x) {
    int ox = (int)(i % ow); long long t = i / ow;
    int oy = (int)(t % oh); t /= oh;
    int ch = (int)(t % c);
    long long plane = t * h * (long long)w;
    float b = bias ? bias[ch] : 0.f;
    auto at = [&](int yy, int xx) {
      const float* p = part + plane + (long long)yy * w + xx;
      float v = 0.f;
      for (int s = 0; s < S; ++s) v += p[(long long)s * part_ss];
      v += b;
      return v >= 0.f ? v : v * slope + 0.f;
    };
    float v;
    if (pool) {
      v = fmaxf(fmaxf(at(2 * oy, 2 * ox), at(2 * oy, 2 * ox + 1)),
                fmaxf(at(2 * oy + 1, 2 * ox), at(2 * oy + 1, 2 * ox + 1)));
    } else {
      v = at(oy, ox);
    }
    y[i] = v;
  }
}

}

namespace tg {
bool conv3x3_uses_oneshot(int n, int cin, int cout, int h, int w) {
  static const int env = TG_LAB_ENV("TG_CONV_ONESHOT", 1);
  return env && cout <= 64 && cdiv(cin, CK) <= 8 && conv3x3_uses_wg_ksplit(n, cin, cout, h, w);
}

bool conv3x3_uses_wg_ksplit(int n, int cin, int cout, int h, int w) {
  static const int ks_env = TG_LAB_ENV("TG_CONV_WG_KSPLIT", 1);
  if (!ks_env || tg_conv3x3_pick_ocb(cout) != 64 || conv3x3_rows_per_wg(64, (long long)n * h * w) != 2)
    return false;
  const long long wgs2 = (long long)cdiv(w, TW) * cdiv(h, 2) * cdiv(cout, 64) * n;
  return wgs2 <= 128 && cdiv(cin, CK) >= 6;
}
}

using namespace tg;

extern "C" int tg_conv3x3_pick_ksplit(int n, int cin, int cout, int h, int w) {
  int ocb = tg_conv3x3_pick_ocb(cout);
  int rows = conv3x3_rows_per_wg(ocb, (long long)n * h * w);
  const double wgs = (double)cdiv(w, TW) * cdiv(h, rows) * cdiv(cout, ocb) * n;
  const int nchunk = cdiv(cin, CK);
  if (conv3x3_uses_oneshot(n, cin, cout, h, w)) return 1;
  static const int legacy = TG_LAB_ENV("TG_KSPLIT_LEGACY", 0);
  if (legacy) {
    if (wgs >= 400 || nchunk < 4) return 1;
    int ks = 1;
    while (ks < 8 && wgs * ks < 640 && nchunk / (ks * 2) >= 2) ks *= 2;
    return ks;
  }
  auto cost = [&](int ks) {
    double share = wgs * ks / 256.0;
    return 4.0 + 1.15 * ((double)nchunk / ks) * (share > 1.0 ? share : 1.0) + (ks > 1 ? 4.5 : 0.0);
  };
  int best = 1;
  double tbest = cost(1);
  for (int ks = 2; ks <= 8 && nchunk / ks >= 2; ks *= 2) {
    double t = cost(ks);
    if (t < 0.85 * tbest) { best = ks; tbest = t; }
  }
  return best;
}

extern "C" int tg_conv3x3_pick_ocb(int cout) { return cout <= 32 ? 32 : 64; }

extern "C" size_t tg_conv3x3_packed_floats(int cin, int cout, int ocb) {
  if (cin <= 0 || cout <= 0 || (ocb != 32 && ocb != 64)) return 0;
  return (size_t)cdiv(cout, ocb) * cdiv(cin, CK) * 9 * CK * ocb;
}

extern "C" int tg_conv3x3_pack(const float* w, float* w_packed, int cin, int cout,
                               int ocb, int transposed, tg_stream_t stream) {
  TG_REQUIRE(w && w_packed, TG_E_ARG, "conv3x3_pack: null pointer");
  TG_REQUIRE(cin > 0 && cout > 0 && (ocb == 32 || ocb == 64), TG_E_SHAPE,
             "conv3x3_pack: cin=%d cout=%d ocb=%d", cin, cout, ocb);
  int nchunk = cdiv(cin, CK), nocg = cdiv(cout, ocb);
  int total = nocg * nchunk * 9 * CK * ocb;
  int blocks = cdiv(total, 256);
  if (blocks > 4096) blocks = 4096;
  hipLaunchKernelGGL(pack3x3_kernel, dim3(blocks), dim3(256), 0, (hipStream_t)stream, w,
                     w_packed, cin, cout, ocb, nchunk, nocg, transposed);
  return check_launch("pack3x3");
}

static int conv3x3_impl(const float* x, int64_t x_nstride, int c1, const float* x2,
                        int64_t x2_nstride, const float* w_packed, int ocb, const float* bias,
                        const float* res, int64_t res_nstride, float* y, int64_t y_nstride, int n,
                        int cin, int cout, int h, int w, int act, int ksplit, float* partials,
                        tg_stream_t stream, const float* mask = nullptr, int64_t mask_nstride = 0,
                        int tapsel = 0, int cphase = 0, int set_p0 = 0, int set_p1 = 0) {
  TG_REQUIRE(x && w_packed && y, TG_E_ARG, "conv3x3_fwd: null pointer");
  TG_REQUIRE(!mask || ksplit <= 1, TG_E_ARG, "conv3x3_fwd: the ReLU mask is applied in the epilogue (no split-K)");
  TG_REQUIRE(n > 0 && cin > 0 && cout > 0 && h > 0 && w > 0, TG_E_SHAPE,
             "conv3x3_fwd: n=%d cin=%d cout=%d h=%d w=%d", n, cin, cout, h, w);
  TG_REQUIRE(c1 > 0 && c1 <= cin && (c1 == cin || x2), TG_E_ARG,
             "conv3x3_fwd: c1=%d cin=%d needs a second source", c1, cin);
  TG_REQUIRE(act >= TG_ACT_NONE && act <= TG_ACT_LRELU02, TG_E_ARG,
             "conv3x3_fwd: act=%d (none|relu|lrelu; tanh*24 only in tg_conv3x3_small_fwd)", act);
  TG_REQUIRE(ocb == 32 || ocb == 64, TG_E_ARG, "conv3x3_fwd: ocb=%d", ocb);
  TG_REQUIRE((long long)(cin + CK) * h * w * 4 < (1ll << 31), TG_E_SHAPE,
             "conv3x3_fwd: one batch item must be < 2 GiB (cin=%d h=%d w=%d)", cin, h, w);
  Conv3x3Args a{};
  a.x = x; a.x2 = (c1 < cin) ? x2 : nullptr; a.wpk = w_packed; a.bias = bias; a.res = res;
  a.y = y; a.x_ns = x_nstride; a.x2_ns = x2_nstride; a.res_ns = res_nstride; a.y_ns = y_nstride;
  a.c1 = c1; a.cin = cin; a.cout = cout; a.h = h; a.w = w; a.act = act;
  a.ksplit = ksplit; a.part = partials; a.part_ss = (long long)n * cout * h * w;
  a.mask = mask; a.mask_ns = mask_nstride;
  a.tapsel = tapsel; a.cphase = cphase; a.rowsets[0] = (unsigned char)set_p0; a.rowsets[1] = (unsigned char)set_p1;
  if (tapsel) {
    TG_REQUIRE((tapsel == 1 || tapsel == 2) && cphase > 0 && cphase % CK == 0 && set_p0 >= 0 && set_p0 <= 3 &&
                   set_p1 >= 0 && set_p1 <= 3, TG_E_ARG, "conv3x3: tapsel=%d cphase=%d sets %d/%d", tapsel,
               cphase, set_p0, set_p1);
    TG_REQUIRE(tapsel == 1 ? cin == 4 * cphase : (cout == 4 * cphase && cphase % 64 == 0), TG_E_SHAPE,
               "conv3x3: phased taps need 4 phases of %d channels (cin=%d cout=%d)", cphase, cin, cout);
  }
  hipStream_t s = (hipStream_t)stream;
  if (ocb == 32) return launch_conv<4, 1, 1>(a, n, s);
  if (conv3x3_rows_per_wg(ocb, (long long)n * h * w) == 4) return launch_conv<4, 1, 2>(a, n, s);
  if (a.ksplit <= 1 && !tapsel && conv3x3_uses_oneshot(n, cin, cout, h, w)) {
    a.vec_ok = (a.w % 4 == 0) && ((uintptr_t)a.y % 16 == 0) && (a.y_ns % 4 == 0) &&
               (!a.res || (((uintptr_t)a.res % 16 == 0) && (a.res_ns % 4 == 0))) &&
               (!a.mask || (((uintptr_t)a.mask % 16 == 0) && (a.mask_ns % 4 == 0)));
    a.tiles_x = cdiv(a.w, TW); a.tiles_y = a.h; a.nocg = 1; a.nchunk = cdiv(a.cin, CK);
    const size_t lds = (size_t)(8 * 3 * 2 * RS * 4 + 2 * 3 * 16 * 64) * sizeof(float);
    static bool attr_set = false;
    if (!attr_set) {
      (void)hipFuncSetAttribute(reinterpret_cast<const void*>(conv3x3_oneshot_kernel<true>),
                                hipFuncAttributeMaxDynamicSharedMemorySize, (int)lds);
      (void)hipFuncSetAttribute(reinterpret_cast<const void*>(conv3x3_oneshot_kernel<false>),
                                hipFuncAttributeMaxDynamicSharedMemorySize, (int)lds);
      attr_set = true;
    }
    const unsigned grid = (unsigned)(a.tiles_x * a.tiles_y * n);
    if (a.x2) hipLaunchKernelGGL(conv3x3_oneshot_kernel<true>, dim3(grid), dim3(512), lds, s, a);
    else hipLaunchKernelGGL(conv3x3_oneshot_kernel<false>, dim3(grid), dim3(512), lds, s, a);
    return check_launch("conv3x3_oneshot");
  }
  if (a.ksplit <= 1 && conv3x3_uses_wg_ksplit(n, cin, cout, h, w)) return launch_conv<1, 2, 1, 2>(a, n, s);
  return launch_conv<2, 2, 1>(a, n, s);
}

extern "C" int tg_conv3x3_fwd(const float* x, int64_t x_nstride, int c1, const float* x2,
                              int64_t x2_nstride, const float* w_packed, int ocb,
                              const float* bias, const float* res, int64_t res_nstride,
                              float* y, int64_t y_nstride, int n, int cin, int cout, int h,
                              int w, int act, tg_stream_t stream) {
  return conv3x3_impl(x, x_nstride, c1, x2, x2_nstride, w_packed, ocb, bias, res, res_nstride, y,
                      y_nstride, n, cin, cout, h, w, act, 1, nullptr, stream);
}

extern "C" int tg_conv3x3_fwd_phased(const float* x, int64_t x_nstride, const float* w_packed, int ocb,
                                     const float* bias, float* y, int64_t y_nstride, int n, int cin,
                                     int cout, int h, int w, int act, int tapsel, int cphase,
                                     int taps_phase0, int taps_phase1, tg_stream_t stream) {
  TG_REQUIRE(tapsel == 1 || tapsel == 2, TG_E_ARG, "conv3x3_fwd_phased: tapsel=%d (1 input | 2 output phases)", tapsel);
  return conv3x3_impl(x, x_nstride, cin, nullptr, 0, w_packed, ocb, bias, nullptr, 0, y, y_nstride, n, cin,
                      cout, h, w, act, 1, nullptr, stream, nullptr, 0, tapsel, cphase, taps_phase0,
                      taps_phase1);
}

extern "C" int tg_conv3x3_fwd_phased_masked(const float* x, int64_t x_nstride, const float* w_packed, int ocb,
                                            const float* bias, const float* relu_mask, int64_t mask_nstride,
                                            float* y, int64_t y_nstride, int n, int cin, int cout, int h,
                                            int w, int act, int tapsel, int cphase, int taps_phase0,
                                            int taps_phase1, tg_stream_t stream) {
  TG_REQUIRE(tapsel == 1 || tapsel == 2, TG_E_ARG, "conv3x3_fwd_phased: tapsel=%d (1 input | 2 output phases)", tapsel);
  return conv3x3_impl(x, x_nstride, cin, nullptr, 0, w_packed, ocb, bias, nullptr, 0, y, y_nstride, n, cin,
                      cout, h, w, act, 1, nullptr, stream, relu_mask, mask_nstride, tapsel, cphase, taps_phase0,
                      taps_phase1);
}

extern "C" int tg_conv3x3_phased_pick_ksplit(int n, int cin, int cout, int h, int w, int ocb) {
  if (n <= 0 || cin <= 0 || cout <= 0 || h <= 0 || w <= 0 || (ocb != 32 && ocb != 64)) return 1;
  const int rows = conv3x3_rows_per_wg(ocb, (long long)n * h * w);
  const long long wgs = (long long)cdiv(w, TW) * cdiv(h, rows) * cdiv(cout, ocb) * n;
  const int nchunk = cdiv(cin, CK);
  if (wgs >= 384 || nchunk < 16) return 1;
  int ks = 2;
  while (ks < 8 && wgs * ks * 2 <= 1024 && nchunk / (ks * 2) >= 4) ks *= 2;
  return ks;
}

extern "C" int tg_conv3x3_fwd_phased_splitk(const float* x, int64_t x_nstride, const float* w_packed, int ocb,
                                            const float* bias, float* y, int n, int cin, int cout, int h, int w,
                                            int act, int tapsel, int cphase, int taps_phase0, int taps_phase1,
                                            int ksplit, float* partials, tg_stream_t stream) {
  TG_REQUIRE(y && partials, TG_E_ARG, "conv3x3_fwd_phased_splitk: null pointer");
  TG_REQUIRE(tapsel == 1 || tapsel == 2, TG_E_ARG, "conv3x3_fwd_phased_splitk: tapsel=%d", tapsel);
  TG_REQUIRE(ksplit >= 2 && ksplit <= 16 && ksplit <= cdiv(cin, CK), TG_E_ARG,
             "conv3x3_fwd_phased_splitk: ksplit=%d for cin=%d", ksplit, cin);
  TG_REQUIRE(act >= TG_ACT_NONE && act <= TG_ACT_LRELU02, TG_E_ARG, "conv3x3_fwd_phased_splitk: act=%d", act);
  int rc = conv3x3_impl(x, x_nstride, cin, nullptr, 0, w_packed, ocb, nullptr, nullptr, 0, partials,
                        (int64_t)cout * h * w, n, cin, cout, h, w, TG_ACT_NONE, ksplit, partials, stream, nullptr, 0,
                        tapsel, cphase, taps_phase0, taps_phase1);
  if (rc != TG_OK) return rc;
  return conv3x3_splitk_finalize(partials, ksplit, bias, act, 0, y, n, cout, h, w, stream);
}

static const int S2_MAX_TILES = 1024;
extern "C" int tg_conv3x3s2_supported(int n, int cin, int cout, int h_out, int w_out) {
  if (n <= 0 || cin <= 0 || cin > 64 || cout <= 0 || cout > 64 || h_out <= 0 || w_out <= 0) return 0;
  return (long long)n * h_out * cdiv(w_out, TW) <= S2_MAX_TILES ? 1 : 0;
}

extern "C" int tg_conv3x3s2_fwd(const float* x, int64_t x_nstride, const float* w_packed, const float* bias,
                                const float* relu_mask, int64_t mask_nstride, float* y, int64_t y_nstride, int n,
                                int cin, int cout, int h_out, int w_out, int act, tg_stream_t stream) {
  TG_REQUIRE(x && w_packed && y, TG_E_ARG, "conv3x3s2_fwd: null pointer");
  TG_REQUIRE(tg_conv3x3s2_supported(n, cin, cout, h_out, w_out), TG_E_SHAPE,
             "conv3x3s2_fwd: n=%d cin=%d cout=%d out %dx%d (cin, cout <= 64, <= 1024 row tiles)", n, cin, cout, h_out, w_out);
  TG_REQUIRE(act >= TG_ACT_NONE && act <= TG_ACT_LRELU02, TG_E_ARG, "conv3x3s2_fwd: act=%d", act);
  TG_REQUIRE((long long)(cin + CK) * 4 * h_out * w_out * 4 < (1ll << 31), TG_E_SHAPE, "conv3x3s2_fwd: item too large");
  Conv3x3Args a{};
  a.x = x; a.wpk = w_packed; a.bias = bias; a.y = y; a.x_ns = x_nstride; a.y_ns = y_nstride;
  a.mask = relu_mask; a.mask_ns = mask_nstride;
  a.c1 = cin; a.cin = cin; a.cout = cout; a.h = h_out; a.w = w_out; a.act = act;
  a.tiles_x = cdiv(w_out, TW); a.tiles_y = h_out; a.nocg = 1; a.nchunk = cdiv(cin, CK);
  const size_t lds = (size_t)(8 * 3 * 2 * RS2 * 4 + 2 * 3 * 16 * 64) * sizeof(float);
  static bool attr_set = false;
  if (!attr_set) {
    (void)hipFuncSetAttribute(reinterpret_cast<const void*>(conv3x3s2_oneshot_kernel),
                              hipFuncAttributeMaxDynamicSharedMemorySize, (int)lds);
    attr_set = true;
  }
  hipLaunchKernelGGL(conv3x3s2_oneshot_kernel, dim3((unsigned)(a.tiles_x * a.tiles_y * n)), dim3(512), lds,
                     (hipStream_t)stream, a);
  return check_launch("conv3x3s2_oneshot");
}

extern "C" int tg_conv3x3_fwd_masked(const float* x, int64_t x_nstride, int c1, const float* x2,
                                     int64_t x2_nstride, const float* w_packed, int ocb,
                                     const float* bias, const float* res, int64_t res_nstride,
                                     const float* relu_mask, int64_t mask_nstride, float* y,
                                     int64_t y_nstride, int n, int cin, int cout, int h, int w,
                                     int act, tg_stream_t stream) {
  return conv3x3_impl(x, x_nstride, c1, x2, x2_nstride, w_packed, ocb, bias, res, res_nstride, y,
                      y_nstride, n, cin, cout, h, w, act, 1, nullptr, stream, relu_mask, mask_nstride);
}

namespace tg {
int conv3x3_splitk_conv(const float* x, int64_t x_nstride, int c1, const float* x2,
                        int64_t x2_nstride, const float* w_packed, int ocb, int n, int cin,
                        int cout, int h, int w, int ksplit, float* partials, tg_stream_t stream) {
  return conv3x3_impl(x, x_nstride, c1, x2, x2_nstride, w_packed, ocb, nullptr, nullptr, 0,
                      partials, (int64_t)cout * h * w, n, cin, cout, h, w, TG_ACT_NONE, ksplit,
                      partials, stream);
}
int conv3x3_splitk_finalize(const float* partials, int ksplit, const float* bias, int act, int pool,
                            float* y, int n, int cout, int h, int w, tg_stream_t stream) {
  long long total = (long long)n * cout * (pool ? (h / 2) * (w / 2) : h * w);
  int blocks = (int)((total + 255) / 256);
  if (blocks > 4096) blocks = 4096;
  hipLaunchKernelGGL(splitk_finalize_kernel, dim3(blocks), dim3(256), 0, (hipStream_t)stream,
                     partials, ksplit, (long long)n * cout * h * w, bias, act_slope_host(act), pool,
                     y, n, cout, h, w);
  return check_launch("splitk_finalize");
}
}

extern "C" int tg_conv3x3_splitk_fwd(const float* x, int64_t x_nstride, int c1, const float* x2,
                                     int64_t x2_nstride, const float* w_packed, int ocb,
                                     const float* bias, float* y, int n, int cin, int cout, int h,
                                     int w, int act, int ksplit, float* partials, int pool,
                                     tg_stream_t stream) {
  TG_REQUIRE(y && partials, TG_E_ARG, "conv3x3_splitk_fwd: null pointer");
  TG_REQUIRE(ksplit >= 2 && ksplit <= 16 && ksplit <= cdiv(cin, CK), TG_E_ARG,
             "conv3x3_splitk_fwd: ksplit=%d for cin=%d", ksplit, cin);
  TG_REQUIRE(act >= TG_ACT_NONE && act <= TG_ACT_LRELU02, TG_E_ARG, "conv3x3_splitk_fwd: act=%d", act);
  TG_REQUIRE(!pool || (h >= 2 && w >= 2), TG_E_SHAPE, "conv3x3_splitk_fwd: pool needs h,w >= 2");
  int rc = conv3x3_splitk_conv(x, x_nstride, c1, x2, x2_nstride, w_packed, ocb, n, cin, cout, h, w,
                               ksplit, partials, stream);
  if (rc != TG_OK) return rc;
  return conv3x3_splitk_finalize(partials, ksplit, bias, act, pool, y, n, cout, h, w, stream);
}
```

### tecogan-pytorch_amd/csrc/tg_conv3x3_wino.hip

```cpp
#include <stdlib.h>

#include "tg_common.h"

namespace tg {

struct WinoArgs {
  const float* x;
  const float* x2;
  const float* u;
  const float* bias;
  const float* res;
  const float* mask;
  float* y;
  long long x_ns, x2_ns, res_ns, mask_ns, y_ns;
  int c1, cin, cout, h, w, act;
  int tiles_x, tiles_y, nstage, nocg, nocb;
  int nblocks;
  int vec_ok;
};

constexpr int W_ICS = 16;
constexpr int W_RS = 40;
constexpr int W_ICSTR = 4 * W_RS;
constexpr int W_VS = 20;

__global__ void wino_pack_kernel(const float* __restrict__ w, float* __restrict__ out, int cin, int cout,
                                 int nchunk, int nocb, int transposed) {
  const int total = nchunk * nocb * 4 * 64 * 4;
  for (int i = blockIdx.x * blockDim.x + threadIdx.x; i < total; i += gridDim.x * blockDim.x) {
    const int e = i & 3, lane = (i >> 2) & 63, j = (i >> 8) & 3;
    const int rest = i >> 10;
    const int ocb = rest % nocb, chunk = rest / nocb;
    const int p = 4 * j + e;
    const int oc = 16 * ocb + (lane & 15), ic = 4 * chunk + (lane >> 4);
    float v = 0.f;
    if (oc < cout && ic < cin) {
      float g[3][3];
#pragma unroll
      for (int a = 0; a < 3; ++a)
#pragma unroll
        for (int b = 0; b < 3; ++b)
          g[a][b] = transposed == 2 ? w[((size_t)ic * cout + oc) * 9 + (8 - (a * 3 + b))]
                                    : w[((size_t)oc * cin + ic) * 9 + a * 3 + b];
      const int pi = p >> 2, pj = p & 3;
      float col[3];
#pragma unroll
      for (int b = 0; b < 3; ++b) {
        col[b] = pi == 0 ? g[0][b]
               : pi == 1 ? 0.5f * ((g[0][b] + g[1][b]) + g[2][b])
               : pi == 2 ? 0.5f * ((g[0][b] - g[1][b]) + g[2][b])
                         : g[2][b];
      }
      v = pj == 0 ? col[0]
        : pj == 1 ? 0.5f * ((col[0] + col[1]) + col[2])
        : pj == 2 ? 0.5f * ((col[0] - col[1]) + col[2])
                  : col[2];
    }
    out[i] = v;
  }
}

template <bool COH> __device__ __forceinline__ float2 ld2(const float* p) {
  if constexpr (COH) {
    const unsigned long long v = __hip_atomic_load(reinterpret_cast<const unsigned long long*>(p), __ATOMIC_RELAXED, __HIP_MEMORY_SCOPE_AGENT);
    return make_float2(__builtin_bit_cast(float, (unsigned)v), __builtin_bit_cast(float, (unsigned)(v >> 32)));
  } else {
    return *reinterpret_cast<const float2*>(p);
  }
}
template <bool COH> __device__ __forceinline__ float ld1(const float* p) {
  if constexpr (COH) return __hip_atomic_load(p, __ATOMIC_RELAXED, __HIP_MEMORY_SCOPE_AGENT);
  else return *p;
}
template <bool COH> __device__ __forceinline__ void st2(float* p, float v0, float v1) {
  if constexpr (COH) {
    const unsigned long long v = (unsigned long long)__builtin_bit_cast(unsigned, v0) | ((unsigned long long)__builtin_bit_cast(unsigned, v1) << 32);
    __hip_atomic_store(reinterpret_cast<unsigned long long*>(p), v, __ATOMIC_RELAXED, __HIP_MEMORY_SCOPE_AGENT);
  } else {
    *reinterpret_cast<float2*>(p) = make_float2(v0, v1);
  }
}
template <bool COH> __device__ __forceinline__ void st1(float* p, float v) {
  if constexpr (COH) __hip_atomic_store(p, v, __ATOMIC_RELAXED, __HIP_MEMORY_SCOPE_AGENT);
  else *p = v;
}

constexpr int AUX_SC1 = 16;

template <int TR> struct WGeo3 {
  static constexpr int TC = 16 / TR;
  static constexpr int PR = 2 * TR + 2, PC = 2 * TC + 2;
  static constexpr int PE = PR * PC;
  static constexpr int RS = TR == 1 ? W_RS : (TR == 2 ? 24 : 12);
  static_assert(PR * RS <= W_ICSTR, "patch of one channel fits the channel stride");
};

template <bool COH, int TR = 1>
__device__ __forceinline__ void wino_tile(const WinoArgs& a, int tx, int ty, int ocg, int n) {
  using G = WGeo3<TR>;
  __shared__ __attribute__((aligned(16))) float s_raw[W_ICS * W_ICSTR];
  __shared__ __attribute__((aligned(16))) float s_v[2 * W_ICS * 16 * W_VS];

  const int t = threadIdx.x, l = t & 63;
  const int wv = __builtin_amdgcn_readfirstlane(t >> 6);
  const int x0 = tx * (2 * G::TC), y0 = ty * (2 * TR);
  const int hw = a.h * a.w;

  constexpr int RAW_ELEMS = W_ICS * G::PE;
  constexpr int RAW_PER_T = (RAW_ELEMS + 255) / 256;
  constexpr unsigned OOB = 0x80000000u;
  unsigned roff[RAW_PER_T];
#pragma unroll
  for (int k = 0; k < RAW_PER_T; ++k) {
    const int e = t + 256 * k;
    const int ic = e / G::PE, rem = e - ic * G::PE, r = rem / G::PC, c = rem - r * G::PC;
    const int gy = y0 - 1 + r, gx = x0 - 1 + c;
    roff[k] = (e < RAW_ELEMS && gy >= 0 && gy < a.h && gx >= 0 && gx < a.w)
                  ? (unsigned)(ic * hw + gy * a.w + gx) * 4u : OOB;
  }
  const __amdgpu_buffer_rsrc_t rx = __builtin_amdgcn_make_buffer_rsrc(
      const_cast<float*>(a.x + (size_t)n * a.x_ns), 0, (unsigned)a.c1 * hw * 4u, 0x00020000);
  const __amdgpu_buffer_rsrc_t rx2 = __builtin_amdgcn_make_buffer_rsrc(
      const_cast<float*>(a.x2 ? a.x2 + (size_t)n * a.x2_ns : a.x), 0,
      a.x2 ? (unsigned)(a.cin - a.c1) * hw * 4u : 0u, 0x00020000);
  const bool dual = a.x2 != nullptr;
  auto load_raw = [&](int s, float (&reg)[RAW_PER_T]) {
    const unsigned so = (unsigned)(s * W_ICS) * hw * 4u;
#pragma unroll
    for (int k = 0; k < RAW_PER_T; ++k) {
      float v = __builtin_bit_cast(float, __builtin_amdgcn_raw_buffer_load_b32(rx, (int)(roff[k] + so), 0, COH ? AUX_SC1 : 0));
      if (dual)
        v += __builtin_bit_cast(float, __builtin_amdgcn_raw_buffer_load_b32(
                 rx2, (int)(roff[k] + so - (unsigned)a.c1 * hw * 4u), 0, COH ? AUX_SC1 : 0));
      reg[k] = v;
    }
  };
  auto store_raw = [&](const float (&reg)[RAW_PER_T]) {
#pragma unroll
    for (int k = 0; k < RAW_PER_T; ++k) {
      const int e = t + 256 * k;
      const int ic = e / G::PE, rem = e - ic * G::PE, r = rem / G::PC, c = rem - r * G::PC;
      if (e < RAW_ELEMS) s_raw[ic * W_ICSTR + r * G::RS + c] = reg[k];
    }
  };

  const f32x4* ug = reinterpret_cast<const f32x4*>(a.u) + ((size_t)(ocg * 4 + wv) * 4) * 64 + l;
  const size_t ustep = (size_t)a.nocb * 4 * 64;
  const int ktotal = 4 * a.nstage;
  auto load_uh = [&](int kstep, int half, f32x4 (&u)[4]) {
    kstep = kstep < ktotal ? kstep : ktotal - 1;
    const f32x4* p = ug + (size_t)kstep * ustep + half * 128;
    u[2 * half] = p[0];
    u[2 * half + 1] = p[64];
  };

  f32x4 acc[16];
#pragma unroll
  for (int p = 0; p < 16; ++p) acc[p] = f32x4{0.f, 0.f, 0.f, 0.f};

  constexpr int VBUF4 = W_ICS * 16 * W_VS / 4;
  const float* traw = s_raw + (t >> 4) * W_ICSTR + 2 * ((t & 15) / G::TC) * G::RS + 2 * ((t & 15) % G::TC);
  f32x4* tv = reinterpret_cast<f32x4*>(s_v + t * W_VS);
  const f32x4* bv = reinterpret_cast<const f32x4*>(s_v + ((l >> 4) * 16 + (l & 15)) * W_VS);

  auto mfma8 = [&](const f32x4 (&u)[4], int buf, int ks, int half) {
    f32x4 bq[2];
#pragma unroll
    for (int j = 0; j < 2; ++j) bq[j] = bv[buf * VBUF4 + ks * (4 * 16 * W_VS / 4) + 2 * half + j];
#pragma unroll
    for (int p = 0; p < 8; ++p)
      acc[8 * half + p] = __builtin_amdgcn_mfma_f32_16x16x4f32(u[2 * half + (p >> 2)][p & 3], bq[p >> 2][p & 3],
                                                               acc[8 * half + p], 0, 0, 0);
  };
  auto kstep = [&](int k, f32x4 (&u)[4], int buf, auto&& between) {
    mfma8(u, buf, k & 3, 0);
    __builtin_amdgcn_sched_barrier(0);
    load_uh(k + 2, 0, u);
    between();
    mfma8(u, buf, k & 3, 1);
    __builtin_amdgcn_sched_barrier(0);
    load_uh(k + 2, 1, u);
  };
  auto transform_half = [&](int buf, int hp) {
    float d[3][4];
#pragma unroll
    for (int r = 0; r < 3; ++r) {
      const float2 p0 = *reinterpret_cast<const float2*>(traw + (r + hp) * G::RS);
      const float2 p1 = *reinterpret_cast<const float2*>(traw + (r + hp) * G::RS + 2);
      d[r][0] = p0.x; d[r][1] = p0.y; d[r][2] = p1.x; d[r][3] = p1.y;
    }
    float qa[4], qb[4];
#pragma unroll
    for (int c = 0; c < 4; ++c) {
      qa[c] = hp == 0 ? d[0][c] - d[2][c] : d[1][c] - d[0][c];
      qb[c] = hp == 0 ? d[1][c] + d[2][c] : d[0][c] - d[2][c];
    }
    tv[buf * VBUF4 + 2 * hp] = f32x4{qa[0] - qa[2], qa[1] + qa[2], qa[2] - qa[1], qa[1] - qa[3]};
    tv[buf * VBUF4 + 2 * hp + 1] = f32x4{qb[0] - qb[2], qb[1] + qb[2], qb[2] - qb[1], qb[1] - qb[3]};
  };

  const int ox = x0 + 2 * ((l & 15) % G::TC);
  const int oy0 = y0 + 2 * ((l & 15) / G::TC);
  const int oc_base = ocg * 64 + wv * 16 + 4 * (l >> 4);
  const float* rn = a.res ? a.res + (size_t)n * a.res_ns : nullptr;
  const bool res_pre = rn && a.vec_ok;

  float rawreg[RAW_PER_T];
  f32x4 u0[4], u1[4];
  const int last = a.nstage - 1;
  load_raw(0, rawreg);
  load_uh(0, 0, u0); load_uh(0, 1, u0);
  load_uh(1, 0, u1); load_uh(1, 1, u1);
  store_raw(rawreg);
  __syncthreads();
  if (last > 0) load_raw(1, rawreg);
  transform_half(0, 0);
  transform_half(0, 1);
  __syncthreads();
  if (last > 0) store_raw(rawreg);

  auto nothing = [] {};
  for (int s = 0; s < last; ++s) {
    const int cur = s & 1, nxt = cur ^ 1;
    kstep(4 * s + 0, u0, cur, nothing);
    __syncthreads();
    if (s + 2 <= last) load_raw(s + 2, rawreg);
    kstep(4 * s + 1, u1, cur, [&] { transform_half(nxt, 0); });
    kstep(4 * s + 2, u0, cur, [&] { transform_half(nxt, 1); });
    kstep(4 * s + 3, u1, cur, nothing);
    __syncthreads();
    if (s + 2 <= last) store_raw(rawreg);
  }
  float2 rpre[4][2];
  {
    const int cur = last & 1;
    kstep(4 * last + 0, u0, cur, nothing);
    kstep(4 * last + 1, u1, cur, nothing);
    kstep(4 * last + 2, u0, cur, nothing);
#pragma unroll
    for (int r = 0; r < 4; ++r)
#pragma unroll
      for (int i = 0; i < 2; ++i) {
        rpre[r][i] = make_float2(0.f, 0.f);
        if (res_pre && oc_base + r < a.cout && ox < a.w && oy0 + i < a.h)
          rpre[r][i] = ld2<COH>(rn + (size_t)(oc_base + r) * hw + (size_t)(oy0 + i) * a.w + ox);
      }
    kstep(4 * last + 3, u1, cur, nothing);
  }

  const float slope = act_slope(a.act);
  float* yn = a.y + (size_t)n * a.y_ns;
  const float* mn = a.mask ? a.mask + (size_t)n * a.mask_ns : nullptr;
#pragma unroll
  for (int r = 0; r < 4; ++r) {
    const int oc = oc_base + r;
    float sr[2][4];
#pragma unroll
    for (int j = 0; j < 4; ++j) {
      sr[0][j] = (acc[0 + j][r] + acc[4 + j][r]) + acc[8 + j][r];
      sr[1][j] = (acc[4 + j][r] - acc[8 + j][r]) - acc[12 + j][r];
    }
    if (oc >= a.cout || ox >= a.w) continue;
    const float bz = a.bias ? a.bias[oc] : 0.f;
#pragma unroll
    for (int i = 0; i < 2; ++i) {
      const int oy = oy0 + i;
      if (oy >= a.h) continue;
      float v0 = ((sr[i][0] + sr[i][1]) + sr[i][2]) + bz;
      float v1 = ((sr[i][1] - sr[i][2]) - sr[i][3]) + bz;
      if (a.act == TG_ACT_TANH24) { v0 = apply_act(v0, a.act); v1 = apply_act(v1, a.act); }
      else {
        v0 = __builtin_fmaxf(v0, slope * v0);
        v1 = __builtin_fmaxf(v1, slope * v1);
      }
      const size_t o = (size_t)oc * hw + (size_t)oy * a.w + ox;
      const bool two = ox + 1 < a.w;
      if (a.vec_ok) {
        if (rn) { v0 += rpre[r][i].x; v1 += rpre[r][i].y; }
        if (mn) { const float2 mm = *reinterpret_cast<const float2*>(mn + o); v0 = mm.x > 0.f ? v0 : 0.f; v1 = mm.y > 0.f ? v1 : 0.f; }
        st2<COH>(yn + o, v0, v1);
      } else {
        if (rn) { v0 += ld1<COH>(rn + o); if (two) v1 += ld1<COH>(rn + o + 1); }
        if (mn) { v0 = mn[o] > 0.f ? v0 : 0.f; if (two) v1 = mn[o + 1] > 0.f ? v1 : 0.f; }
        st1<COH>(yn + o, v0);
        if (two) st1<COH>(yn + o + 1, v1);
      }
    }
  }
}

template <int TR>
__global__ __launch_bounds__(256, 3) void conv3x3_wino_kernel(WinoArgs a) {
  int b = blockIdx.x;
  if (a.nblocks > 0) {
    const int per = (a.nblocks + 7) >> 3;
    b = (b & 7) * per + (b >> 3);
    if (b >= a.nblocks) return;
  }
  const int tx = __builtin_amdgcn_readfirstlane(b % a.tiles_x); b /= a.tiles_x;
  const int ty = __builtin_amdgcn_readfirstlane(b % a.tiles_y); b /= a.tiles_y;
  const int ocg = __builtin_amdgcn_readfirstlane(b % a.nocg);
  const int n = __builtin_amdgcn_readfirstlane(b / a.nocg);
  wino_tile<false, TR>(a, tx, ty, ocg, n);
}

struct WinoLayer {
  const float *x, *x2, *u, *bias, *res;
  float* y;
  long long x_ns, x2_ns, res_ns, y_ns;
  int c1, cin, act, nstage;
};
constexpr int W_MAX_CHAIN = 24;
struct WinoChainArgs {
  WinoLayer L[W_MAX_CHAIN];
  int nlayer, bpl;
  int cout, h, w, tiles_x, tiles_y, ntile, vec_ok;
  int* flags;
  int* err;
  unsigned epoch;
  int poll_limit;
};

template <bool COHX>
__global__ __launch_bounds__(256, 3) void conv3x3_wino_chain_kernel(WinoChainArgs c) {
  const int layer = __builtin_amdgcn_readfirstlane((int)blockIdx.x / c.bpl);
  int b = (int)blockIdx.x - layer * c.bpl;
  {
    const int per = c.bpl >> 3;
    b = (b & 7) * per + (b >> 3);
    if (b >= c.ntile) return;
  }
  const int tile = b;
  const int tx = __builtin_amdgcn_readfirstlane(b % c.tiles_x); b /= c.tiles_x;
  const int ty = __builtin_amdgcn_readfirstlane(b % c.tiles_y);
  const int n = __builtin_amdgcn_readfirstlane(b / c.tiles_y);
  const WinoLayer& L = c.L[layer];
  WinoArgs a;
  a.x = L.x; a.x2 = L.x2; a.u = L.u; a.bias = L.bias; a.res = L.res; a.mask = nullptr; a.y = L.y;
  a.x_ns = L.x_ns; a.x2_ns = L.x2_ns; a.res_ns = L.res_ns; a.mask_ns = 0; a.y_ns = L.y_ns;
  a.c1 = L.c1; a.cin = L.cin; a.cout = c.cout; a.h = c.h; a.w = c.w; a.act = L.act;
  a.tiles_x = c.tiles_x; a.tiles_y = c.tiles_y; a.nstage = L.nstage; a.nocg = 1; a.nocb = 4;
  a.nblocks = 0; a.vec_ok = c.vec_ok;
  if (layer > 0) {
    const int t = threadIdx.x;
    if (t < 9) {
      const int ny = ty - 1 + t / 3, nx = tx - 1 + t % 3;
      if (ny >= 0 && ny < c.tiles_y && nx >= 0 && nx < c.tiles_x) {
        const unsigned* f = reinterpret_cast<const unsigned*>(c.flags) + (size_t)(layer - 1) * c.ntile + (n * c.tiles_y + ny) * c.tiles_x + nx;
        int polls = 0;
        bool fault = c.poll_limit < 0;
        while (!fault && __hip_atomic_load(f, __ATOMIC_RELAXED, __HIP_MEMORY_SCOPE_AGENT) != c.epoch) {
          __builtin_amdgcn_s_sleep(4);
          fault = ++polls > c.poll_limit;
        }
        if (fault) __hip_atomic_fetch_add(c.err, 1, __ATOMIC_RELAXED, __HIP_MEMORY_SCOPE_SYSTEM);
      }
    }
    __syncthreads();
  }
  wino_tile<COHX>(a, tx, ty, 0, n);
  __builtin_amdgcn_s_waitcnt(0);
  __syncthreads();
  if (threadIdx.x == 0)
    __hip_atomic_store(reinterpret_cast<unsigned*>(c.flags) + (size_t)layer * c.ntile + tile, c.epoch, __ATOMIC_RELAXED, __HIP_MEMORY_SCOPE_AGENT);
}

}

using namespace tg;

extern "C" int64_t tg_conv3x3_wino_packed_floats(int cin, int cout) {
  if (cin <= 0 || cout <= 0) return -1;
  const int64_t nchunk = 4 * ((cin + 15) / 16), nocb = 4 * ((cout + 63) / 64);
  return nchunk * nocb * 4 * 64 * 4;
}

extern "C" int tg_conv3x3_prefers_wino(int n, int cin, int cout, int h, int w) {
  static const int env = [] { const char* e = getenv("TG_CONV_WINO"); return e && *e ? atoi(e) : -1; }();
  if (env == 0) return 0;
  if (n <= 0 || cin < 16 || cout <= 0 || cout % 64 != 0 || h < 2 || w < 2) return 0;
  const long long wgs = (long long)cdiv(w, 32) * cdiv(h, 2) * (cout / 64) * n;
  return env == 1 ? 1 : (wgs >= 160 ? 1 : 0);
}

extern "C" int tg_pack_conv3x3_wino(const float* w, float* out, int cin, int cout, int transposed,
                                    tg_stream_t stream) {
  TG_REQUIRE(w && out, TG_E_ARG, "pack_conv3x3_wino: null pointer");
  TG_REQUIRE(cin > 0 && cout > 0 && (transposed == 0 || transposed == 2), TG_E_ARG,
             "pack_conv3x3_wino: cin=%d cout=%d transposed=%d (0 or 2)", cin, cout, transposed);
  const int nchunk = 4 * cdiv(cin, 16), nocb = 4 * cdiv(cout, 64);
  const int total = nchunk * nocb * 4 * 64 * 4;
  hipLaunchKernelGGL(wino_pack_kernel, dim3(cdiv(total, 256) > 1024 ? 1024 : cdiv(total, 256)), dim3(256), 0,
                     (hipStream_t)stream, w, out, cin, cout, nchunk, nocb, transposed);
  return check_launch("pack_conv3x3_wino");
}

namespace tg {
int conv3x3_wino_launch(const float* x, int64_t x_ns, int c1, const float* x2, int64_t x2_ns, const float* u,
                        const float* bias, const float* res, int64_t res_ns, const float* mask,
                        int64_t mask_ns, float* y, int64_t y_ns, int n, int cin, int cout, int h, int w,
                        int act, tg_stream_t stream) {
  WinoArgs a{};
  a.x = x; a.x2 = x2; a.u = u; a.bias = bias; a.res = res; a.mask = mask; a.y = y;
  a.x_ns = x_ns; a.x2_ns = x2_ns; a.res_ns = res_ns; a.mask_ns = mask_ns; a.y_ns = y_ns;
  a.c1 = x2 ? c1 : cin; a.cin = cin; a.cout = cout; a.h = h; a.w = w; a.act = act;
  int tr = 1;
  {
    long long best = (long long)cdiv(w, 32) * cdiv(h, 2);
    for (int cand = 2; cand <= 4; cand *= 2) {
      const long long c = (long long)cdiv(w, 32 / cand) * cdiv(h, 2 * cand);
      if (c < best) { best = c; tr = cand; }
    }
    static const int tr_env = TG_LAB_ENV("TG_WINO_TR", 0);
    if (tr_env == 1 || tr_env == 2 || tr_env == 4) tr = tr_env;
  }
  a.tiles_x = cdiv(w, 32 / tr); a.tiles_y = cdiv(h, 2 * tr);
  a.nstage = cdiv(cin, 16); a.nocg = cdiv(cout, 64); a.nocb = 4 * a.nocg;
  auto al8 = [](const void* p, int64_t ns) { return ((uintptr_t)p % 8) == 0 && ns % 2 == 0; };
  a.vec_ok = (w % 2 == 0) && ((int64_t)h * w) % 2 == 0 && al8(y, y_ns) && (!res || al8(res, res_ns)) &&
             (!mask || al8(mask, mask_ns));
  const long long blocks = (long long)a.tiles_x * a.tiles_y * a.nocg * n;
  static const int xcd_env = TG_LAB_ENV("TG_WINO_XCD", -1);
  const bool xcd = xcd_env >= 0 ? xcd_env != 0 : blocks >= 512;
  a.nblocks = xcd ? (int)blocks : 0;
  const unsigned grid = xcd ? (unsigned)(8 * ((blocks + 7) / 8)) : (unsigned)blocks;
  if (tr == 1) hipLaunchKernelGGL(conv3x3_wino_kernel<1>, dim3(grid), dim3(256), 0, (hipStream_t)stream, a);
  else if (tr == 2) hipLaunchKernelGGL(conv3x3_wino_kernel<2>, dim3(grid), dim3(256), 0, (hipStream_t)stream, a);
  else hipLaunchKernelGGL(conv3x3_wino_kernel<4>, dim3(grid), dim3(256), 0, (hipStream_t)stream, a);
  return check_launch("conv3x3_wino");
}
}

extern "C" int tg_conv3x3_wino_fwd(const float* x, int64_t x_nstride, int c1, const float* x2,
                                   int64_t x2_nstride, const float* u_packed, const float* bias,
                                   const float* res, int64_t res_nstride, const float* relu_mask,
                                   int64_t mask_nstride, float* y, int64_t y_nstride, int n, int cin,
                                   int cout, int h, int w, int act, tg_stream_t stream) {
  TG_REQUIRE(x && u_packed && y, TG_E_ARG, "conv3x3_wino: null pointer");
  TG_REQUIRE(n > 0 && cin > 0 && cout > 0 && h > 0 && w > 0, TG_E_SHAPE, "conv3x3_wino: n=%d cin=%d cout=%d h=%d w=%d",
             n, cin, cout, h, w);
  TG_REQUIRE(!x2 || (c1 > 0 && c1 < cin), TG_E_ARG, "conv3x3_wino: c1=%d of cin=%d", c1, cin);
  TG_REQUIRE(act >= TG_ACT_NONE && act <= TG_ACT_TANH24, TG_E_ARG, "conv3x3_wino: act=%d", act);
  TG_REQUIRE((long long)cin * h * w < (1ll << 29), TG_E_SHAPE, "conv3x3_wino: image too large");
  return conv3x3_wino_launch(x, x_nstride, c1, x2, x2_nstride, u_packed, bias, res, res_nstride, relu_mask,
                             mask_nstride, y, y_nstride, n, cin, cout, h, w, act, stream);
}

extern "C" int64_t tg_conv3x3_wino_chain_flag_ints(int n_layers, int n, int h, int w) {
  if (n_layers <= 0 || n_layers > W_MAX_CHAIN || n <= 0 || h <= 0 || w <= 0) return -1;
  return (int64_t)n_layers * n * cdiv(h, 2) * cdiv(w, 32) + 16;
}

namespace tg {
int conv3x3_wino_chain_launch(const tg_wino_layer* layers, int n_layers, int n, int cout, int h, int w,
                              int32_t* flags, int32_t* err, unsigned epoch, int poll_limit, tg_stream_t stream) {
  TG_REQUIRE(layers && flags && err, TG_E_ARG, "conv3x3_wino_chain: null pointer");
  TG_REQUIRE(n_layers >= 1 && n_layers <= W_MAX_CHAIN, TG_E_ARG, "conv3x3_wino_chain: %d layers (1..%d)", n_layers, W_MAX_CHAIN);
  TG_REQUIRE(n > 0 && h > 0 && w > 0 && cout > 0 && cout <= 64, TG_E_SHAPE,
             "conv3x3_wino_chain: n=%d cout=%d (<= 64: one output-channel group) h=%d w=%d", n, cout, h, w);
  TG_REQUIRE(epoch != 0, TG_E_ARG, "conv3x3_wino_chain: epoch 0 is the cleared state of the flags");
  WinoChainArgs c{};
  c.nlayer = n_layers; c.cout = cout; c.h = h; c.w = w;
  c.tiles_x = cdiv(w, 32); c.tiles_y = cdiv(h, 2);
  const long long ntile = (long long)c.tiles_x * c.tiles_y * n;
  TG_REQUIRE(ntile * n_layers < (1ll << 30), TG_E_SHAPE, "conv3x3_wino_chain: too many tiles");
  c.ntile = (int)ntile;
  c.bpl = (int)(8 * ((ntile + 7) / 8));
  c.flags = flags; c.err = err; c.epoch = epoch; c.poll_limit = poll_limit;
  bool vec = (w % 2 == 0) && ((int64_t)h * w) % 2 == 0;
  auto al8 = [](const void* p, int64_t ns) { return ((uintptr_t)p % 8) == 0 && ns % 2 == 0; };
  for (int i = 0; i < n_layers; ++i) {
    const tg_wino_layer& l = layers[i];
    TG_REQUIRE(l.x && l.u_packed && l.y, TG_E_ARG, "conv3x3_wino_chain: layer %d: null pointer", i);
    TG_REQUIRE(l.cin > 0 && (!l.x2 || (l.c1 > 0 && l.c1 < l.cin)), TG_E_ARG, "conv3x3_wino_chain: layer %d: cin=%d c1=%d", i, l.cin, l.c1);
    TG_REQUIRE((long long)l.cin * h * w < (1ll << 29), TG_E_SHAPE, "conv3x3_wino_chain: layer %d too large", i);
    TG_REQUIRE(l.act >= TG_ACT_NONE && l.act <= TG_ACT_TANH24, TG_E_ARG, "conv3x3_wino_chain: layer %d: act=%d", i, l.act);
    WinoLayer& d = c.L[i];
    d.x = l.x; d.x2 = l.x2; d.u = l.u_packed; d.bias = l.bias; d.res = l.res; d.y = l.y;
    d.x_ns = l.x_nstride; d.x2_ns = l.x2_nstride; d.res_ns = l.res_nstride; d.y_ns = l.y_nstride;
    d.c1 = l.x2 ? l.c1 : l.cin; d.cin = l.cin; d.act = l.act; d.nstage = cdiv(l.cin, 16);
    vec = vec && al8(l.y, l.y_nstride) && (!l.res || al8(l.res, l.res_nstride));
  }
  c.vec_ok = vec ? 1 : 0;
  const unsigned grid = (unsigned)(c.bpl * n_layers);
#if TG_LAB
  static const int noncoh = TG_LAB_ENV("TG_WINO_CHAIN_NONCOH", 0);
  static const int pad_lds = TG_LAB_ENV("TG_WINO_CHAIN_LDS", 0);
  if (noncoh) {
    hipLaunchKernelGGL(conv3x3_wino_chain_kernel<false>, dim3(grid), dim3(256), pad_lds, (hipStream_t)stream, c);
    return check_launch("conv3x3_wino_chain");
  }
  hipLaunchKernelGGL(conv3x3_wino_chain_kernel<true>, dim3(grid), dim3(256), pad_lds, (hipStream_t)stream, c);
#else
  hipLaunchKernelGGL(conv3x3_wino_chain_kernel<true>, dim3(grid), dim3(256), 0, (hipStream_t)stream, c);
#endif
  return check_launch("conv3x3_wino_chain");
}
}

extern "C" int tg_conv3x3_wino_chain(const tg_wino_layer* layers, int n_layers, int n, int cout, int h, int w,
                                     int32_t* flags, int epoch, tg_stream_t stream) {
  TG_REQUIRE(flags && n_layers >= 1 && n > 0 && h > 0 && w > 0, TG_E_ARG, "conv3x3_wino_chain: bad argument");
  const long long ntile = (long long)cdiv(w, 32) * cdiv(h, 2) * n;
  return conv3x3_wino_chain_launch(layers, n_layers, n, cout, h, w, flags, flags + (size_t)n_layers * ntile,
                                   (unsigned)epoch, TG_CHAIN_POLL_LIMIT_DEFAULT, stream);
}
```

### tecogan-pytorch_amd/ops.py

```python
import torch

from . import _lib as L
from ._lib import (ACT_NONE, ACT_RELU, ACT_LRELU02, ACT_TANH24,
                   UP_NONE, UP_BICUBIC, UP_BILINEAR)

UP_MODE = {'BD': UP_BICUBIC, 'BI': UP_BILINEAR}


_RAW_STREAM = getattr(torch._C, '_cuda_getCurrentRawStream', None)


def _stream():
    if _RAW_STREAM is not None:
        return _RAW_STREAM(torch.cuda.current_device())
    return torch.cuda.current_stream().cuda_stream


def _chk(t, name, dtype=torch.float32):
    if not (torch.is_tensor(t) and t.is_cuda):
        raise L.TecoganHipError(f'{name}: expected a CUDA/HIP tensor (no CPU path exists)')
    if t.dtype != dtype:
        raise L.TecoganHipError(f'{name}: expected {dtype}, got {t.dtype}')
    if not t.is_contiguous():
        raise L.TecoganHipError(f'{name}: tensor must be contiguous')
# ... 1003 lines not shown
    world = gathered.shape[0]
    count = float(per * h * w * world)
    y = torch.empty_like(x)
    stats = []
    for g in range(groups):
        part = gathered[:, g * 2 * c:(g + 1) * 2 * c].contiguous()
        mean = torch.empty(c, dtype=torch.float32, device=x.device)
        invstd = torch.empty(c, dtype=torch.float32, device=x.device)
        L.check(lib.tg_bn_merge_stats(part.data_ptr(), world, float(per * h * w), float(eps), float(momentum),
                                      mean.data_ptr(), invstd.data_ptr(), _ptr(running_mean), _ptr(running_var), c,
                                      _stream()), 'tg_bn_merge_stats')
        L.check(lib.tg_bn_lrelu_apply(x[g * per:(g + 1) * per].data_ptr(), mean.data_ptr(), invstd.data_ptr(),
                                      gamma.data_ptr(), beta.data_ptr(), float(slope), y[g * per:(g + 1) * per].data_ptr(),
                                      per, c, h * w, _stream()), 'tg_bn_lrelu_apply')
        stats.append((mean, invstd, count))
    return y, stats


def sync_bn_lrelu_train_bwd_groups(x, y, dy, groups, gamma, stats, dgamma=None, dbeta=None, need_dx=True, slope=0.2):
    from .utils import dist_utils
    n, c, h, w = x.shape
    per = n // groups
    lib = L.lib()
    sums = torch.empty(groups * 2 * c, dtype=torch.float32, device=x.device)
    for g in range(groups):
        sl = slice(g * per, (g + 1) * per)
        L.check(lib.tg_bn_lrelu_bwd_reduce(x[sl].data_ptr(), y[sl].data_ptr(), dy[sl].data_ptr(), stats[g][0].data_ptr(),
                                           stats[g][1].data_ptr(), float(slope), sums[g * 2 * c:].data_ptr(), per, c,
                                           h * w, _stream()), 'tg_bn_lrelu_bwd_reduce')
        if dgamma is not None:
            axpy_(dgamma, sums[g * 2 * c + c:(g + 1) * 2 * c], 1.0)
            axpy_(dbeta, sums[g * 2 * c:g * 2 * c + c], 1.0)
    dist_utils.all_reduce_sum_(sums)
    dx = None
    if need_dx:
        dx = torch.empty_like(x)
        for g in range(groups):
            sl = slice(g * per, (g + 1) * per)
            L.check(lib.tg_bn_lrelu_bwd_apply(x[sl].data_ptr(), y[sl].data_ptr(), dy[sl].data_ptr(), stats[g][0].data_ptr(),
                                              stats[g][1].data_ptr(), gamma.data_ptr(), sums[g * 2 * c:].data_ptr(),
                                              float(slope), 1.0 / stats[g][2], dx[sl].data_ptr(), per, c, h * w,
                                              _stream()), 'tg_bn_lrelu_bwd_apply')
    return dx


def time_gather(x, idx):
    import ctypes
    _chk(x, 'x')
    n, t = x.shape[:2]
    inner = x[0, 0].numel()
    out = torch.empty((n, len(idx)) + tuple(x.shape[2:]), dtype=torch.float32, device=x.device)
    arr = (ctypes.c_int * len(idx))(*[int(i) for i in idx])
    L.check(L.lib().tg_time_gather(x.data_ptr(), out.data_ptr(), arr, n, t, len(idx), inner, _stream()),
            'tg_time_gather')
    return out


def pingpong(x):
    t = x.shape[1]
    return time_gather(x, list(range(t)) + list(range(t - 2, -1, -1)))


def pingpong_grad(g, te):
    _chk(g, 'g')
    n = g.shape[0]
    inner = g[0, 0].numel()
    out = torch.empty((n, 2 * te - 1) + tuple(g.shape[2:]), dtype=torch.float32, device=g.device)
    L.check(L.lib().tg_pingpong_grad(g.data_ptr(), out.data_ptr(), n, te, inner, _stream()), 'tg_pingpong_grad')
    return out


def d_assemble_fwd(data, warped, cond, t, pad, crop, out=None):
    _chk(data, 'data'); _chk(warped, 'warped'); _chk(cond, 'cond')
    n, t_data, c, h, w = data.shape
    x = out if out is not None else torch.empty(n * t // 3, 9 * c, h, w, dtype=torch.float32, device=data.device)
    L.check(L.lib().tg_d_assemble_fwd(data.data_ptr(), t_data, warped.data_ptr(), cond.data_ptr(),
                                      cond.shape[1], x.data_ptr(), n, t, c, h, w, pad, crop, _stream()),
            'tg_d_assemble_fwd')
    return x


def d_assemble_bwd(g, n, t, t_data, c, pad, crop):
    _chk(g, 'g')
    h, w = g.shape[2:]
    g_data = torch.empty(n, t_data, c, h, w, dtype=torch.float32, device=g.device)
    g_warped = torch.empty(n * t, c, h, w, dtype=torch.float32, device=g.device)
    L.check(L.lib().tg_d_assemble_bwd(g.data_ptr(), g_data.data_ptr(), t_data, g_warped.data_ptr(), n, t, c,
                                      h, w, pad, crop, _stream()), 'tg_d_assemble_bwd')
    return g_data, g_warped


def transpose01(x):
    _chk(x, 'x')
    a, b = x.shape[:2]
    y = torch.empty((b, a) + tuple(x.shape[2:]), dtype=torch.float32, device=x.device)
    L.check(L.lib().tg_transpose01(x.data_ptr(), y.data_ptr(), a, b, x[0, 0].numel(), _stream()),
            'tg_transpose01')
    return y


def stack_time(frames):
    import ctypes
    for f in frames:
        _chk(f, 'frame')
    n = frames[0].shape[0]
    y = torch.empty((n, len(frames)) + tuple(frames[0].shape[1:]), dtype=torch.float32,
                    device=frames[0].device)
    arr = (ctypes.c_void_p * len(frames))(*[f.data_ptr() for f in frames])
    L.check(L.lib().tg_stack_time(arr, len(frames), y.data_ptr(), n, frames[0][0].numel(), _stream()),
            'tg_stack_time')
    return y


def index_gather(src, idx, out=None, accumulate=False):
    _chk(src, 'src'); _chk(idx, 'idx', torch.int64)
    if out is None:
        assert not accumulate
        out = torch.empty(idx.numel(), dtype=torch.float32, device=src.device)
    else:
        _chk(out, 'out')
        assert out.numel() == idx.numel()
    L.check(L.lib().tg_index_gather(src.data_ptr(), idx.data_ptr(), out.data_ptr(), idx.numel(),
                                    src.numel(), int(accumulate), _stream()), 'tg_index_gather')
    return out


def pack_conv3x3_wino(w, transposed=0):
    _chk(w, 'w')
    co, ci = (w.shape[0], w.shape[1]) if transposed == 0 else (w.shape[1], w.shape[0])
    nflt = L.lib().tg_conv3x3_wino_packed_floats(ci, co)
    out = torch.empty(nflt, dtype=torch.float32, device=w.device)
    L.check(L.lib().tg_pack_conv3x3_wino(w.data_ptr(), out.data_ptr(), ci, co, transposed, _stream()),
            'tg_pack_conv3x3_wino')
    return out


def conv3x3_wino(x, u_packed, bias, cin, cout, act=ACT_NONE, x2=None, res=None, mask=None, out=None):
    _chk(x, 'x'); _chk(u_packed, 'u_packed')
    n, c1, h, w = x.shape
    if x2 is not None:
        _chk(x2, 'x2')
        assert c1 + x2.shape[1] == cin
    else:
        assert c1 == cin
    y = out if out is not None else torch.empty(n, cout, h, w, dtype=torch.float32, device=x.device)
    L.check(L.lib().tg_conv3x3_wino_fwd(
        x.data_ptr(), x.stride(0), c1, _ptr(x2), x2.stride(0) if x2 is not None else 0,
        u_packed.data_ptr(), _ptr(bias), _ptr(res), res.stride(0) if res is not None else 0,
        _ptr(mask), mask.stride(0) if mask is not None else 0, y.data_ptr(), y.stride(0),
        n, cin, cout, h, w, act, _stream()), 'tg_conv3x3_wino_fwd')
    return y


class RowChain:

    def __init__(self, layers, n, h, w):
        lib = L.lib()
        self.n, self.h, self.w = n, h, w
        self.parts = lib.tg_conv3x3_chain_supported(n, h, w, 64)
        if self.parts == 0:
            raise L.TecoganHipError(f'RowChain: {n}x{h}x{w} cannot run as a chained launch on this device')
        self.layout = 16 if self.parts == 4 else 64
        self.keep = [layers]
        self.arr = (L.ChainLayer * len(layers))()
        for i, d in enumerate(layers):
            a = self.arr[i]
            wt = d['w']
            pk = pack_conv3x3_m16(wt) if self.layout == 16 else pack_conv3x3(wt, ocb=64)[0]
            self.keep.append(pk)
            x, x2, res, mask, y = d['x'], d.get('x2'), d.get('res'), d.get('mask'), d['y']
            a.x, a.x2, a.w_packed, a.bias = x.data_ptr(), _ptr(x2), pk.data_ptr(), _ptr(d.get('bias'))
            a.res, a.relu_mask, a.y = _ptr(res), _ptr(mask), y.data_ptr()
            a.x_nstride, a.y_nstride = x.stride(0), y.stride(0)
            a.x2_nstride = x2.stride(0) if x2 is not None else 0
            a.res_nstride = res.stride(0) if res is not None else 0
            a.mask_nstride = mask.stride(0) if mask is not None else 0
            a.c1, a.cin, a.cout, a.act = x.shape[1], wt.shape[1], wt.shape[0], d.get('act', ACT_NONE)
        self.nl = len(layers)
        self.flags = torch.zeros(lib.tg_conv3x3_chain_flag_ints(self.nl, n, h, w) + 16, dtype=torch.int32,
                                 device=layers[0]['x'].device)
        self.err = self.flags[-16:]
        self.epoch = 0

    def run(self, poll_limit=1 << 21):
        self.epoch += 1
        L.check(L.lib().tg_conv3x3_chain(self.arr, self.nl, self.n, self.h, self.w, self.layout, self.flags.data_ptr(),
                                         self.err.data_ptr(), self.epoch, poll_limit, _stream()), 'tg_conv3x3_chain')

    def faults(self):
        return int(self.err[0].item())


class WinoChain:

    def __init__(self, layers, n, cout, h, w):
        import ctypes
        self.n, self.cout, self.h, self.w = n, cout, h, w
        self.keep = layers
        self.arr = (L.WinoLayer * len(layers))()
        for i, d in enumerate(layers):
            a = self.arr[i]
            x, x2, res, y = d['x'], d.get('x2'), d.get('res'), d['y']
            a.x, a.x2, a.u_packed = x.data_ptr(), _ptr(x2), d['u'].data_ptr()
            a.bias, a.res, a.y = _ptr(d.get('bias')), _ptr(res), y.data_ptr()
            a.x_nstride, a.y_nstride = x.stride(0), y.stride(0)
            a.x2_nstride = x2.stride(0) if x2 is not None else 0
            a.res_nstride = res.stride(0) if res is not None else 0
            a.c1, a.cin, a.act = x.shape[1], d['cin'], d.get('act', ACT_NONE)
        nints = L.lib().tg_conv3x3_wino_chain_flag_ints(len(layers), n, h, w)
        self.flags = torch.zeros(nints, dtype=torch.int32, device=layers[0]['x'].device)
        self.epoch = 0

    def run(self):
        self.epoch += 1
        L.check(L.lib().tg_conv3x3_wino_chain(self.arr, len(self.keep), self.n, self.cout, self.h, self.w,
                                              self.flags.data_ptr(), self.epoch, _stream()),
                'tg_conv3x3_wino_chain')

    def bailouts(self):
        return int(self.flags[-16].item())


def pack_wres_convt(w):
    _chk(w, 'w')
    if tuple(w.shape) != (64, 64, 3, 3):
        raise L.TecoganHipError(f'pack_wres_convt: weight {tuple(w.shape)}, expected (64, 64, 3, 3)')
    lib = L.lib()
    out = torch.empty(lib.tg_conv3x3_wino_resident_ct_floats(), dtype=torch.float32, device=w.device)
    L.check(lib.tg_conv3x3_wino_resident_ct_pack(w.data_ptr(), out.data_ptr(), _stream()), 'tg_conv3x3_wino_resident_ct_pack')
    return out


class WinoResident(WinoChain):

    def __init__(self, layers, cout, h, w):
        WinoChain.__init__(self, layers, 1, cout, h, w)
        nbytes = L.lib().tg_conv3x3_wino_resident_ws_bytes(h, w)
        self.ws = torch.zeros(nbytes // 4, dtype=torch.int32, device=layers[0]['x'].device)

    @staticmethod
    def supported(cout, h, w, n=1):
        return bool(L.lib().tg_conv3x3_wino_resident_supported(n, cout, h, w))

    def run(self, convt=None):
        self.epoch += 1
        if convt is None:
            L.check(L.lib().tg_conv3x3_wino_resident(self.arr, len(self.keep), self.cout, self.h, self.w,
                                                     self.ws.data_ptr(), self.epoch, _stream()),
                    'tg_conv3x3_wino_resident')
            return
        import ctypes as C
        ct = L.WresConvT(convt['u'].data_ptr(), convt['bias'].data_ptr(), convt['y'].data_ptr(), convt.get('act', ACT_RELU))
        L.check(L.lib().tg_conv3x3_wino_resident_ct(self.arr, len(self.keep), self.cout, self.h, self.w,
                                                    self.ws.data_ptr(), self.epoch, C.byref(ct), _stream()),
                'tg_conv3x3_wino_resident_ct')

    def bailouts(self):
        return int(self.ws[-64].item())



def f16_supported(n, cin, cout, h, w):
    return bool(L.lib().tg_conv3x3_f16_supported(int(n), int(cin), int(cout), int(h), int(w)))


def f16_pack_index(transposed=False, cin=64, cout=64):
    import numpy as np
    i = np.arange(18 * 4 * 64 * 8, dtype=np.int64)
    j, lane, ct, ks = i & 7, (i >> 3) & 63, (i >> 9) & 3, i >> 11
    co, tap, ci = ct * 16 + (lane & 15), ks >> 1, (ks & 1) * 32 + (lane >> 4) * 8 + j
    src = ((ci * cout + co) if transposed else (co * cin + ci)) * 9 + tap
    return np.where((ci < cin) & (co < cout), src, -1)


def f16_pack_weights(w, transposed=False):
    _chk(w, 'w')
    cin, cout = (w.shape[0], w.shape[1]) if transposed else (w.shape[1], w.shape[0])
    lib = L.lib()
    nh = lib.tg_conv3x3_f16_packed_halves(int(cin), int(cout))
    if nh == 0 or tuple(w.shape[2:]) != (3, 3):
        raise L.TecoganHipError(f'f16_pack_weights: weight {tuple(w.shape)} (3x3, at most 64 channels each way)')
    out = torch.empty(nh, dtype=torch.float16, device=w.device)
    L.check(lib.tg_conv3x3_f16_pack_weights(w.data_ptr(), int(cin), int(cout), 1 if transposed else 0, out.data_ptr(),
                                            _stream()), 'tg_conv3x3_f16_pack_weights')
    return out


def f16_pack_input(x1, x2=None):
    _chk(x1, 'x1')
    n, c1, h, w = x1.shape
    c2 = 0
    if x2 is not None:
        _chk(x2, 'x2')
        c2 = x2.shape[1]
        if (x2.shape[0], x2.shape[2], x2.shape[3]) != (n, h, w):
            raise L.TecoganHipError('f16_pack_input: x1 / x2 shapes differ')
    y = torch.empty(n, h, w, 64, dtype=torch.float16, device=x1.device)
    L.check(L.lib().tg_conv3x3_f16_pack_input(x1.data_ptr(), c1 * h * w, c1, _ptr(x2), c2 * h * w, c2, y.data_ptr(),
                                              n, h, w, _stream()), 'tg_conv3x3_f16_pack_input')
    return y


def conv3x3_f16(x, w_packed, bias, act=ACT_NONE, res=None, out=None):
    _chk(x, 'x', torch.float16); _chk(w_packed, 'w_packed', torch.float16); _chk(bias, 'bias')
    n, h, w, c = x.shape
    if res is not None:
# ... 26 lines not shown
```

Baseline: 1530 frames/s.

## Fuse FNet maxpool into conv epilogue and bilinear upsample into conv input staging

The FNet encoder's 2x2 max-pool is folded into the epilogue of the preceding 3x3 conv, for both the Winograd and the 32-channel MFMA paths. The decoder's 2x bilinear upsample is folded into the input staging of the next conv, which samples the low-resolution tensor directly. This drops the separate pool and upsample launches and the round trips of full-resolution intermediates through memory. In exchange, the fused conv does four gathered loads plus interpolation per input element, and the buffer ping-pong logic becomes conditional, which risks aliasing mistakes.

Measured after the change: 1533 frames/s, median of 6. No clear change (+0.2%).

```diff
diff --git a/include/tecogan_hip.h b/include/tecogan_hip.h
--- a/include/tecogan_hip.h
+++ b/include/tecogan_hip.h
@@ -90,6 +90,18 @@
                         const float* res, int64_t res_nstride, const float* relu_mask,
                         int64_t mask_nstride, float* y, int64_t y_nstride, int n, int cin,
                         int cout, int h, int w, int act, tg_stream_t stream);
+
+#define TG_FUSE_POOL 1
+#define TG_FUSE_UP2X 2
+int tg_conv3x3_wino_fwd_fused(const float* x, int64_t x_nstride, const float* u_packed, const float* bias,
+                              float* y, int64_t y_nstride, int n, int cin, int cout, int h, int w, int act,
+                              int fuse, tg_stream_t stream);
+int tg_conv3x3_fwd_pool(const float* x, int64_t x_nstride, int c1, const float* x2, int64_t x2_nstride,
+                        const float* w_packed, int ocb, const float* bias, float* y, int64_t y_nstride,
+                        int n, int cin, int cout, int h, int w, int act, tg_stream_t stream);
+int tg_conv3x3_fwd_up2x(const float* x, int64_t x_nstride, const float* w_packed, int ocb, const float* bias,
+                        float* y, int64_t y_nstride, int n, int cin, int cout, int h, int w, int act,
+                        tg_stream_t stream);
 
 typedef struct {
   const float* x; const float* x2; const float* u_packed; const float* bias; const float* res;
diff --git a/tecogan-pytorch_amd/_lib.py b/tecogan-pytorch_amd/_lib.py
--- a/tecogan-pytorch_amd/_lib.py
+++ b/tecogan-pytorch_amd/_lib.py
@@ -169,6 +169,9 @@
     'tg_conv3x3_prefers_wino': (I, [I, I, I, I, I]),
     'tg_pack_conv3x3_wino': (I, [P, P, I, I, I, P]),
     'tg_conv3x3_wino_fwd': (I, [P, I64, I, P, I64, P, P, P, I64, P, I64, P, I64, I, I, I, I, I, I, P]),
+    'tg_conv3x3_wino_fwd_fused': (I, [P, I64, P, P, P, I64, I, I, I, I, I, I, I, P]),
+    'tg_conv3x3_fwd_pool': (I, [P, I64, I, P, I64, P, I, P, P, I64, I, I, I, I, I, I, P]),
+    'tg_conv3x3_fwd_up2x': (I, [P, I64, P, I, P, P, I64, I, I, I, I, I, I, P]),
     'tg_time_gather': (I, [P, P, P, I, I, I, I64, P]),
     'tg_transpose01': (I, [P, P, I, I, I64, P]),
     'tg_stack_time': (I, [P, I, P, I, I64, P]),
diff --git a/tecogan-pytorch_amd/csrc/tg_api.hip b/tecogan-pytorch_amd/csrc/tg_api.hip
--- a/tecogan-pytorch_amd/csrc/tg_api.hip
+++ b/tecogan-pytorch_amd/csrc/tg_api.hip
@@ -295,7 +295,7 @@
   };
   auto conv = [&](const float* x, int64_t xns, int c1, const float* x2, int64_t x2ns, int cin,
                   int cout, int hh, int ww, int act, const float* res, int64_t rns, float* y,
-                  int64_t yns, bool pool = false, float* pool_tmp = nullptr) {
+                  int64_t yns, bool pool = false, float* pool_tmp = nullptr, bool up = false) -> bool {
     const tg_layer_weights lw = p->L[li++];
     int ocb = tg_conv3x3_pick_ocb(cout);
     int kind = ocb == 32 ? K_CONV32
@@ -305,6 +305,16 @@
     double fl = 2.0 * cin * 9 * cout * px;
     double by = 4.0 * px * (cin + cout + (res ? cout : 0)) + 4.0 * 9 * cin * cout;
     if (lw.u && tg_conv3x3_prefers_wino(n, cin, cout, hh, ww)) {
+      if ((pool || up) && !x2 && !res) {
+        if (pool) by = 4.0 * px * cin + 1.0 * px * cout + 4.0 * 9 * cin * cout;
+        if (up) by = 1.0 * px * cin + 4.0 * px * cout + 4.0 * 9 * cin * cout;
+        float* yf = pool ? pool_tmp : y;
+        go(K_CONV_WINO, fl, by, [&] {
+          return tg_conv3x3_wino_fwd_fused(x, xns, lw.u, lw.b, yf, yns, n, cin, cout, hh, ww, act,
+                                           pool ? TG_FUSE_POOL : TG_FUSE_UP2X, st);
+        });
+        return pool;
+      }
       float* yw = pool ? pool_tmp : y;
       go(K_CONV_WINO, fl, by, [&] {
         return tg::conv3x3_wino_launch(x, xns, c1, x2, x2ns, lw.u, lw.b, res, rns, nullptr, 0, yw,
@@ -313,7 +323,7 @@
       if (pool)
         go(K_POOL, 0, 4.0 * n * cout * (hh * ww + (hh / 2) * (ww / 2)),
            [&] { return tg_maxpool2_fwd(yw, y, n * cout, hh, ww, st); });
-      return;
+      return false;
     }
     int ks = res ? 1 : tg_conv3x3_pick_ksplit(n, cin, cout, hh, ww);
     if (ks == 1 && kind == K_CONV64_R2 && tg::conv3x3_uses_wg_ksplit(n, cin, cout, hh, ww))
@@ -327,7 +337,19 @@
         return tg::conv3x3_splitk_finalize(part_buf, ks, lw.b, act, pool ? 1 : 0, y, n, cout, hh, ww,
                                            st);
       });
-      return;
+      return false;
+    }
+    if (pool && kind == K_CONV32 && !res) {
+      go(kind, fl, 4.0 * px * cin + 1.0 * px * cout + 4.0 * 9 * cin * cout, [&] {
+        return tg_conv3x3_fwd_pool(x, xns, c1, x2, x2ns, lw.w, ocb, lw.b, pool_tmp, yns, n, cin, cout, hh, ww, act, st);
+      });
+      return true;
+    }
+    if (up) {
+      go(kind, fl, 1.0 * px * cin + 4.0 * px * cout + 4.0 * 9 * cin * cout, [&] {
+        return tg_conv3x3_fwd_up2x(x, xns, lw.w, ocb, lw.b, y, yns, n, cin, cout, hh, ww, act, st);
+      });
+      return false;
     }
     float* yc = pool ? pool_tmp : y;
     go(kind, fl, by, [&] {
@@ -337,6 +359,7 @@
     if (pool)
       go(K_POOL, 0, 4.0 * n * cout * (hh * ww + (hh / 2) * (ww / 2)),
          [&] { return tg_maxpool2_fwd(yc, y, n * cout, hh, ww, st); });
+    return false;
   };
   int hh = h, ww = w;
   const int enc[3] = {32, 64, 128};
@@ -350,30 +373,37 @@
     else
       conv(src, (int64_t)cin * hh * ww, cin, nullptr, 0, cin, co, hh, ww, TG_ACT_LRELU02, nullptr,
            0, A, (int64_t)co * hh * ww);
-    conv(A, (int64_t)co * hh * ww, co, nullptr, 0, co, co, hh, ww, TG_ACT_LRELU02, nullptr, 0, A,
-         (int64_t)co * (hh / 2) * (ww / 2), true, B);
+    const bool in_b = conv(A, (int64_t)co * hh * ww, co, nullptr, 0, co, co, hh, ww, TG_ACT_LRELU02, nullptr, 0, A,
+                           (int64_t)co * (hh / 2) * (ww / 2), true, B);
     hh /= 2; ww /= 2; cin = co;
-    float* t = A; A = B; B = t;
+    if (!in_b) { float* t = A; A = B; B = t; }
     src = B;
   }
   const int dec[3] = {256, 128, 64};
+  auto up_fusable = [&](const tg_layer_weights& lw, int ci, int co, int hh_, int ww_) {
+    if (hh_ < 4 || ww_ < 4) return false;
+    if (lw.u && tg_conv3x3_prefers_wino(n, ci, co, hh_, ww_)) return true;
+    return tg_conv3x3_pick_ocb(co) == 32 && tg_conv3x3_pick_ksplit(n, ci, co, hh_, ww_) == 1;
+  };
+  bool up_pending = false;
   for (int d = 0; d < 3; ++d) {
     int co = dec[d];
-    conv(src, (int64_t)cin * hh * ww, cin, nullptr, 0, cin, co, hh, ww, TG_ACT_LRELU02, nullptr, 0,
-         A, (int64_t)co * hh * ww);
+    conv(src, (int64_t)cin * (up_pending ? (hh / 2) * (ww / 2) : hh * ww), cin, nullptr, 0, cin, co, hh, ww,
+         TG_ACT_LRELU02, nullptr, 0, A, (int64_t)co * hh * ww, false, nullptr, up_pending);
     conv(A, (int64_t)co * hh * ww, co, nullptr, 0, co, co, hh, ww, TG_ACT_LRELU02, nullptr, 0, B,
          (int64_t)co * hh * ww);
-    {
+    up_pending = up_fusable(p->L[li], co, d < 2 ? dec[d + 1] : 32, 2 * hh, 2 * ww);
+    if (!up_pending) {
       float *pi = B, *po = A; int ph = hh, pw = ww;
       go(K_UPSAMPLE, 0, 4.0 * n * co * ph * pw * 5.0,
          [&] { return tg_upsample_fwd(pi, po, n * co, ph, pw, 2, TG_UP_BILINEAR, 1.0f, st); });
     }
     hh *= 2; ww *= 2; cin = co;
-    float* t = A; A = B; B = t;
+    if (!up_pending) { float* t = A; A = B; B = t; }
     src = B;
   }
-  conv(src, (int64_t)cin * hh * ww, cin, nullptr, 0, cin, 32, hh, ww, TG_ACT_LRELU02, nullptr, 0, A,
-       (int64_t)32 * hh * ww);
+  conv(src, (int64_t)cin * (up_pending ? (hh / 2) * (ww / 2) : hh * ww), cin, nullptr, 0, cin, 32, hh, ww,
+       TG_ACT_LRELU02, nullptr, 0, A, (int64_t)32 * hh * ww, false, nullptr, up_pending);
   {
     const tg_layer_weights lw = p->L[li++];
     float* ai = A; int fh_ = hh, fw_ = ww;
diff --git a/tecogan-pytorch_amd/csrc/tg_common.h b/tecogan-pytorch_amd/csrc/tg_common.h
--- a/tecogan-pytorch_amd/csrc/tg_common.h
+++ b/tecogan-pytorch_amd/csrc/tg_common.h
@@ -59,7 +59,7 @@
 int conv3x3_wino_launch(const float* x, int64_t x_ns, int c1, const float* x2, int64_t x2_ns, const float* u,
                         const float* bias, const float* res, int64_t res_ns, const float* mask,
                         int64_t mask_ns, float* y, int64_t y_ns, int n, int cin, int cout, int h, int w,
-                        int act, tg_stream_t stream);
+                        int act, tg_stream_t stream, int fuse = 0);
 
 constexpr int TG_CHAIN_POLL_LIMIT_DEFAULT = 1 << 21;
 int conv3x3_wino_chain_launch(const tg_wino_layer* layers, int n_layers, int n, int cout, int h, int w,
diff --git a/tecogan-pytorch_amd/csrc/tg_conv3x3_mfma.hip b/tecogan-pytorch_amd/csrc/tg_conv3x3_mfma.hip
--- a/tecogan-pytorch_amd/csrc/tg_conv3x3_mfma.hip
+++ b/tecogan-pytorch_amd/csrc/tg_conv3x3_mfma.hip
@@ -106,9 +106,11 @@
   }
 }
 
-template <int WM, int WN, int NT, bool DUAL, int ABL = 0, int KS = 1>
+template <int WM, int WN, int NT, bool DUAL, int ABL = 0, int KS = 1, bool POOL = false, bool UP = false>
 __global__ __launch_bounds__(WM* WN* KS * 64) void conv3x3_mfma_kernel(Conv3x3Args a) {
+  static_assert(!UP || (!DUAL && KS == 1), "up-sampled staging: one source, no wave groups over K");
   static_assert(KS == 1 || KS == 2, "wave groups over K: one or two");
+  static_assert(!POOL || (WM == 4 && WN == 1 && KS == 1), "pooled epilogue: four rows x all output channels per workgroup");
   constexpr int NTHREADS = WM * WN * KS * 64;
   constexpr int OCB = WN * NT * 32;
   constexpr int PH = WM + 2;
@@ -142,11 +144,14 @@
   const int n = b / a.ksplit;
   const int x0 = tx * TW, y0 = ty * WM;
   const int hw = a.h * a.w;
+  const int xhw = UP ? (a.h >> 1) * (a.w >> 1) : hw;
   const int ch_begin = (int)((long long)ks * a.nchunk / a.ksplit);
   const int ch_end = (int)((long long)(ks + 1) * a.nchunk / a.ksplit);
 
   unsigned voff[I_PER_T];
   int lds_item[I_PER_T];
+  unsigned uoff[UP ? I_PER_T : 1][4];
+  float uwt[UP ? I_PER_T : 1][4];
 #pragma unroll
   for (int i = 0; i < I_PER_T; ++i) {
     int q = tid + i * NTHREADS;
@@ -156,13 +161,24 @@
     bool ok = q < IN_ITEMS && gy >= 0 && gy < a.h && gx >= 0 && gx < a.w;
     voff[i] = ok ? (unsigned)((4 * hf * hw + gy * a.w + gx) * 4) : OOB;
     lds_item[i] = q < IN_ITEMS ? ((r * 2 + hf) * RS + col) * 4 : -1;
+    if constexpr (UP) {
+      const int lh = a.h >> 1, lw = a.w >> 1;
+      int ya, yb, xa, xb;
+      bilinear_src(gy < 0 ? 0 : gy, 2, lh, ya, yb, uwt[i][2], uwt[i][3]);
+      bilinear_src(gx < 0 ? 0 : gx, 2, lw, xa, xb, uwt[i][0], uwt[i][1]);
+      const unsigned cb = (unsigned)(4 * hf * xhw);
+      uoff[i][0] = ok ? (cb + ya * lw + xa) * 4u : OOB;
+      uoff[i][1] = ok ? (cb + ya * lw + xb) * 4u : OOB;
+      uoff[i][2] = ok ? (cb + yb * lw + xa) * 4u : OOB;
+      uoff[i][3] = ok ? (cb + yb * lw + xb) * 4u : OOB;
+    }
   }
   const __amdgpu_buffer_rsrc_t rs1 = __builtin_amdgcn_make_buffer_rsrc(
-      const_cast<float*>(a.x + (long long)n * a.x_ns), 0, a.c1 * hw * 4, 0x00020000);
+      const_cast<float*>(a.x + (long long)n * a.x_ns), 0, a.c1 * xhw * 4, 0x00020000);
   const __amdgpu_buffer_rsrc_t rs2 = __builtin_amdgcn_make_buffer_rsrc(
       const_cast<float*>(DUAL ? a.x2 + (long long)n * a.x2_ns : a.x), 0,
       DUAL ? (a.cin - a.c1) * hw * 4 : 0, 0x00020000);
-  const unsigned plane = (unsigned)hw * 4u;
+  const unsigned plane = (unsigned)xhw * 4u;
 
   const f32x4* wsrc =
       reinterpret_cast<const f32x4*>(a.wpk + (size_t)ocg * a.nchunk * W_FLOATS);
@@ -178,6 +194,15 @@
       for (int i = 0; i < I_PER_T; ++i) {
 #pragma unroll
         for (int j = 0; j < 4; ++j) {
+          if constexpr (UP) {
+            const unsigned cj = cbase + (unsigned)j * plane;
+            const float ta = buf_load(rs1, uoff[i][0] + cj), tb = buf_load(rs1, uoff[i][1] + cj);
+            const float ba = buf_load(rs1, uoff[i][2] + cj), bb = buf_load(rs1, uoff[i][3] + cj);
+            const float top = uwt[i][0] * ta + uwt[i][1] * tb;
+            const float bot = uwt[i][0] * ba + uwt[i][1] * bb;
+            rin[k][i][j] = uwt[i][2] * top + uwt[i][3] * bot;
+            continue;
+          }
           unsigned o1 = voff[i] + cbase + (unsigned)j * plane;
           float v = buf_load(rs1, o1);
           if (DUAL) v += buf_load(rs2, o1 - (unsigned)a.c1 * plane);
@@ -322,6 +347,39 @@
     return;
   }
   const float slope = act_slope(a.act);
+  if constexpr (POOL) {
+    constexpr int ES = 36;
+    float* ep = smem + wave * (NT * 32 * ES);
+#pragma unroll
+    for (int t = 0; t < NT; ++t)
+#pragma unroll
+      for (int r = 0; r < 16; ++r)
+        ep[(t * 32 + (r & 3) + 8 * (r >> 2) + 4 * lh) * ES + ll] = acc[t][r];
+    __syncthreads();
+    const int oh = a.h >> 1, ow = a.w >> 1;
+    constexpr int OUTS = (WM / 2) * OCB * (TW / 2);
+#pragma unroll
+    for (int j = 0; j < OUTS / NTHREADS; ++j) {
+      const int idx = j * NTHREADS + tid;
+      const int pp = idx & 15, ol = (idx >> 4) % OCB, pr = idx / (16 * OCB);
+      const int oc = ocg * OCB + ol;
+      const int gy = y0 + 2 * pr, gx = x0 + 2 * pp;
+      if (oc < a.cout && gy + 1 < a.h && gx + 1 < a.w) {
+        const float2 r0 = *reinterpret_cast<const float2*>(smem + (2 * pr) * (NT * 32 * ES) + ol * ES + 2 * pp);
+        const float2 r1 = *reinterpret_cast<const float2*>(smem + (2 * pr + 1) * (NT * 32 * ES) + ol * ES + 2 * pp);
+        const float bb = a.bias ? a.bias[oc] : 0.f;
+        float q[4] = {r0.x, r0.y, r1.x, r1.y};
+#pragma unroll
+        for (int e = 0; e < 4; ++e) {
+          const float v = q[e] + bb;
+          q[e] = (v >= 0.f ? v : v * slope + 0.f) + 0.f;
+        }
+        a.y[(long long)n * a.y_ns + ((long long)oc * oh + (gy >> 1)) * ow + (gx >> 1)] =
+            fmaxf(fmaxf(q[0], q[1]), fmaxf(q[2], q[3]));
+      }
+    }
+    return;
+  }
   if (a.vec_ok) {
     constexpr int ES = 36;
     float* ep = smem + (wave % (WM * WN)) * (NT * 32 * ES);
@@ -651,7 +709,7 @@
 }
 
 
-template <int WM, int WN, int NT, int KS = 1>
+template <int WM, int WN, int NT, int KS = 1, bool POOL = false, bool UP = false>
 static int launch_conv(const Conv3x3Args& a0, int n, hipStream_t stream) {
   Conv3x3Args a = a0;
   a.vec_ok = (a.w % 4 == 0) && ((uintptr_t)a.y % 16 == 0) && (a.y_ns % 4 == 0) &&
@@ -683,11 +741,16 @@
   const bool xcd = xcd_env >= 0 ? xcd_env != 0 : blocks >= 512;
   a.nblocks = xcd ? (int)blocks : 0;
   const unsigned grid = xcd ? (unsigned)(8 * ((blocks + 7) / 8)) : (unsigned)blocks;
+  if constexpr (UP) {
+    hipLaunchKernelGGL((conv3x3_mfma_kernel<WM, WN, NT, false, 0, KS, POOL, true>),
+                       dim3(grid), dim3(WM * WN * KS * 64), lds, stream, a);
+    return check_launch("conv3x3_mfma");
+  }
   if (a.x2)
-    hipLaunchKernelGGL((conv3x3_mfma_kernel<WM, WN, NT, true, 0, KS>),
+    hipLaunchKernelGGL((conv3x3_mfma_kernel<WM, WN, NT, true, 0, KS, POOL>),
                        dim3(grid), dim3(WM * WN * KS * 64), lds, stream, a);
   else
-    hipLaunchKernelGGL((conv3x3_mfma_kernel<WM, WN, NT, false, 0, KS>),
+    hipLaunchKernelGGL((conv3x3_mfma_kernel<WM, WN, NT, false, 0, KS, POOL>),
                        dim3(grid), dim3(WM * WN * KS * 64), lds, stream, a);
   return check_launch("conv3x3_mfma");
 }
@@ -854,6 +917,43 @@
                       y_nstride, n, cin, cout, h, w, act, 1, nullptr, stream);
 }
 
+extern "C" int tg_conv3x3_fwd_pool(const float* x, int64_t x_nstride, int c1, const float* x2,
+                                   int64_t x2_nstride, const float* w_packed, int ocb,
+                                   const float* bias, float* y, int64_t y_nstride, int n, int cin,
+                                   int cout, int h, int w, int act, tg_stream_t stream) {
+  TG_REQUIRE(x && w_packed && y, TG_E_ARG, "conv3x3_fwd_pool: null pointer");
+  TG_REQUIRE(ocb == 32 && cout <= 32, TG_E_ARG, "conv3x3_fwd_pool: ocb=%d cout=%d (the 32-channel workgroup form only)", ocb, cout);
+  TG_REQUIRE(n > 0 && cin > 0 && cout > 0 && h >= 2 && w >= 2, TG_E_SHAPE,
+             "conv3x3_fwd_pool: n=%d cin=%d cout=%d h=%d w=%d", n, cin, cout, h, w);
+  TG_REQUIRE(c1 > 0 && c1 <= cin && (c1 == cin || x2), TG_E_ARG, "conv3x3_fwd_pool: c1=%d cin=%d needs a second source", c1, cin);
+  TG_REQUIRE(act >= TG_ACT_NONE && act <= TG_ACT_LRELU02, TG_E_ARG, "conv3x3_fwd_pool: act=%d (none|relu|lrelu)", act);
+  TG_REQUIRE((long long)(cin + CK) * h * w * 4 < (1ll << 31), TG_E_SHAPE,
+             "conv3x3_fwd_pool: one batch item must be < 2 GiB (cin=%d h=%d w=%d)", cin, h, w);
+  Conv3x3Args a{};
+  a.x = x; a.x2 = (c1 < cin) ? x2 : nullptr; a.wpk = w_packed; a.bias = bias;
+  a.y = y; a.x_ns = x_nstride; a.x2_ns = x2_nstride; a.y_ns = y_nstride;
+  a.c1 = c1; a.cin = cin; a.cout = cout; a.h = h; a.w = w; a.act = act;
+  a.ksplit = 1; a.part_ss = (long long)n * cout * h * w;
+  return launch_conv<4, 1, 1, 1, true>(a, n, (hipStream_t)stream);
+}
+
+extern "C" int tg_conv3x3_fwd_up2x(const float* x, int64_t x_nstride, const float* w_packed, int ocb,
+                                   const float* bias, float* y, int64_t y_nstride, int n, int cin,
+                                   int cout, int h, int w, int act, tg_stream_t stream) {
+  TG_REQUIRE(x && w_packed && y, TG_E_ARG, "conv3x3_fwd_up2x: null pointer");
+  TG_REQUIRE(ocb == 32 && cout <= 32, TG_E_ARG, "conv3x3_fwd_up2x: ocb=%d cout=%d (the 32-channel workgroup form only)", ocb, cout);
+  TG_REQUIRE(n > 0 && cin > 0 && cout > 0 && h >= 2 && w >= 2 && h % 2 == 0 && w % 2 == 0, TG_E_SHAPE,
+             "conv3x3_fwd_up2x: n=%d cin=%d cout=%d h=%d w=%d (even h, w: twice the map x holds)", n, cin, cout, h, w);
+  TG_REQUIRE(act >= TG_ACT_NONE && act <= TG_ACT_LRELU02, TG_E_ARG, "conv3x3_fwd_up2x: act=%d (none|relu|lrelu)", act);
+  TG_REQUIRE((long long)(cin + CK) * h * w * 4 < (1ll << 31), TG_E_SHAPE,
+             "conv3x3_fwd_up2x: one batch item must be < 2 GiB (cin=%d h=%d w=%d)", cin, h, w);
+  Conv3x3Args a{};
+  a.x = x; a.wpk = w_packed; a.bias = bias; a.y = y; a.x_ns = x_nstride; a.y_ns = y_nstride;
+  a.c1 = cin; a.cin = cin; a.cout = cout; a.h = h; a.w = w; a.act = act;
+  a.ksplit = 1; a.part_ss = (long long)n * cout * h * w;
+  return launch_conv<4, 1, 1, 1, false, true>(a, n, (hipStream_t)stream);
+}
+
 extern "C" int tg_conv3x3_fwd_phased(const float* x, int64_t x_nstride, const float* w_packed, int ocb,
                                      const float* bias, float* y, int64_t y_nstride, int n, int cin,
                                      int cout, int h, int w, int act, int tapsel, int cphase,
diff --git a/tecogan-pytorch_amd/csrc/tg_conv3x3_wino.hip b/tecogan-pytorch_amd/csrc/tg_conv3x3_wino.hip
--- a/tecogan-pytorch_amd/csrc/tg_conv3x3_wino.hip
+++ b/tecogan-pytorch_amd/csrc/tg_conv3x3_wino.hip
@@ -93,9 +93,14 @@
   static constexpr int PE = PR * PC;
   static constexpr int RS = TR == 1 ? W_RS : (TR == 2 ? 24 : 12);
   static_assert(PR * RS <= W_ICSTR, "patch of one channel fits the channel stride");
+  static constexpr int LPR = TR + 2, LPC = TC + 2, LPE = LPR * LPC;
+  static constexpr int LICS = 80;
+  static_assert(LPE <= LICS, "low-resolution patch of one channel fits its channel stride");
 };
 
-template <bool COH, int TR = 1>
+constexpr int FUSE_POOL = 1, FUSE_UP = 2;
+
+template <bool COH, int TR = 1, int FUSE = 0>
 __device__ __forceinline__ void wino_tile(const WinoArgs& a, int tx, int ty, int ocg, int n) {
   using G = WGeo3<TR>;
   __shared__ __attribute__((aligned(16))) float s_raw[W_ICS * W_ICSTR];
@@ -105,33 +110,42 @@
   const int wv = __builtin_amdgcn_readfirstlane(t >> 6);
   const int x0 = tx * (2 * G::TC), y0 = ty * (2 * TR);
   const int hw = a.h * a.w;
-
-  constexpr int RAW_ELEMS = W_ICS * G::PE;
+  constexpr bool UP = (FUSE & FUSE_UP) != 0;
+  const int lh = a.h >> 1, lw = a.w >> 1;
+  const int xhw = UP ? lh * lw : hw;
+
+  constexpr int RAW_PE = UP ? G::LPE : G::PE, RAW_PC = UP ? G::LPC : G::PC;
+  constexpr int RAW_ELEMS = W_ICS * RAW_PE;
   constexpr int RAW_PER_T = (RAW_ELEMS + 255) / 256;
   constexpr unsigned OOB = 0x80000000u;
   unsigned roff[RAW_PER_T];
 #pragma unroll
   for (int k = 0; k < RAW_PER_T; ++k) {
     const int e = t + 256 * k;
-    const int ic = e / G::PE, rem = e - ic * G::PE, r = rem / G::PC, c = rem - r * G::PC;
+    const int ic = e / RAW_PE, rem = e - ic * RAW_PE, r = rem / RAW_PC, c = rem - r * RAW_PC;
+    if constexpr (UP) {
+      const int ly = min(max((y0 >> 1) - 1 + r, 0), lh - 1), lx = min(max((x0 >> 1) - 1 + c, 0), lw - 1);
+      roff[k] = e < RAW_ELEMS ? (unsigned)(ic * xhw + ly * lw + lx) * 4u : OOB;
+    } else {
     const int gy = y0 - 1 + r, gx = x0 - 1 + c;
     roff[k] = (e < RAW_ELEMS && gy >= 0 && gy < a.h && gx >= 0 && gx < a.w)
                   ? (unsigned)(ic * hw + gy * a.w + gx) * 4u : OOB;
+    }
   }
   const __amdgpu_buffer_rsrc_t rx = __builtin_amdgcn_make_buffer_rsrc(
-      const_cast<float*>(a.x + (size_t)n * a.x_ns), 0, (unsigned)a.c1 * hw * 4u, 0x00020000);
+      const_cast<float*>(a.x + (size_t)n * a.x_ns), 0, (unsigned)a.c1 * xhw * 4u, 0x00020000);
   const __amdgpu_buffer_rsrc_t rx2 = __builtin_amdgcn_make_buffer_rsrc(
       const_cast<float*>(a.x2 ? a.x2 + (size_t)n * a.x2_ns : a.x), 0,
-      a.x2 ? (unsigned)(a.cin - a.c1) * hw * 4u : 0u, 0x00020000);
+      a.x2 ? (unsigned)(a.cin - a.c1) * xhw * 4u : 0u, 0x00020000);
   const bool dual = a.x2 != nullptr;
   auto load_raw = [&](int s, float (&reg)[RAW_PER_T]) {
-    const unsigned so = (unsigned)(s * W_ICS) * hw * 4u;
+    const unsigned so = (unsigned)(s * W_ICS) * xhw * 4u;
 #pragma unroll
     for (int k = 0; k < RAW_PER_T; ++k) {
       float v = __builtin_bit_cast(float, __builtin_amdgcn_raw_buffer_load_b32(rx, (int)(roff[k] + so), 0, COH ? AUX_SC1 : 0));
       if (dual)
         v += __builtin_bit_cast(float, __builtin_amdgcn_raw_buffer_load_b32(
-                 rx2, (int)(roff[k] + so - (unsigned)a.c1 * hw * 4u), 0, COH ? AUX_SC1 : 0));
+                 rx2, (int)(roff[k] + so - (unsigned)a.c1 * xhw * 4u), 0, COH ? AUX_SC1 : 0));
       reg[k] = v;
     }
   };
@@ -139,8 +153,8 @@
 #pragma unroll
     for (int k = 0; k < RAW_PER_T; ++k) {
       const int e = t + 256 * k;
-      const int ic = e / G::PE, rem = e - ic * G::PE, r = rem / G::PC, c = rem - r * G::PC;
-      if (e < RAW_ELEMS) s_raw[ic * W_ICSTR + r * G::RS + c] = reg[k];
+      const int ic = e / RAW_PE, rem = e - ic * RAW_PE, r = rem / RAW_PC, c = rem - r * RAW_PC;
+      if (e < RAW_ELEMS) s_raw[UP ? ic * G::LICS + r * G::LPC + c : ic * W_ICSTR + r * G::RS + c] = reg[k];
     }
   };
 
@@ -181,13 +195,43 @@
     __builtin_amdgcn_sched_barrier(0);
     load_uh(k + 2, 1, u);
   };
+  const int ta = (x0 >> 1) + (t & 15) % G::TC, tb = (y0 >> 1) + (t & 15) / G::TC;
+  const float* tl = s_raw + (t >> 4) * G::LICS + ((t & 15) / G::TC) * G::LPC + (t & 15) % G::TC;
+  const int ce = ta == 0 ? 2 : 1;
+  const float wc0 = ta == 0 ? 1.f : 0.25f, wc1 = ta == 0 ? 0.f : 0.75f;
+  const float wr0 = tb == 0 ? 1.f : 0.25f, wr1 = tb == 0 ? 0.f : 0.75f;
+  const bool zc0 = ta == 0, zc3 = 2 * ta + 2 >= a.w, zr0 = tb == 0, zr3 = 2 * tb + 2 >= a.h;
   auto transform_half = [&](int buf, int hp) {
     float d[3][4];
+    if constexpr (UP) {
+      float hq[3][4];
+#pragma unroll
+      for (int r = 0; r < 3; ++r) {
+        const float l0 = tl[r * G::LPC], l1 = tl[r * G::LPC + 1], l2 = tl[r * G::LPC + 2], le = tl[r * G::LPC + ce];
+        hq[r][0] = 0.75f * l0 + 0.25f * l1;
+        hq[r][1] = wc0 * l0 + wc1 * le;
+        hq[r][2] = 0.75f * l1 + 0.25f * l2;
+        hq[r][3] = 0.25f * l1 + 0.75f * l2;
+      }
+#pragma unroll
+      for (int c = 0; c < 4; ++c) {
+        const float he = tb == 0 ? hq[2][c] : hq[1][c];
+        float w4[4];
+        w4[0] = 0.75f * hq[0][c] + 0.25f * hq[1][c];
+        w4[1] = wr0 * hq[0][c] + wr1 * he;
+        w4[2] = 0.75f * hq[1][c] + 0.25f * hq[2][c];
+        w4[3] = 0.25f * hq[1][c] + 0.75f * hq[2][c];
+        const bool zc = (c == 0 && zc0) || (c == 3 && zc3);
+#pragma unroll
+        for (int r = 0; r < 3; ++r) d[r][c] = (zc || (r + hp == 0 && zr0) || (r + hp == 3 && zr3)) ? 0.f : w4[r + hp];
+      }
+    } else {
 #pragma unroll
     for (int r = 0; r < 3; ++r) {
       const float2 p0 = *reinterpret_cast<const float2*>(traw + (r + hp) * G::RS);
       const float2 p1 = *reinterpret_cast<const float2*>(traw + (r + hp) * G::RS + 2);
       d[r][0] = p0.x; d[r][1] = p0.y; d[r][2] = p1.x; d[r][3] = p1.y;
+    }
     }
     float qa[4], qb[4];
 #pragma unroll
@@ -262,6 +306,21 @@
     }
     if (oc >= a.cout || ox >= a.w) continue;
     const float bz = a.bias ? a.bias[oc] : 0.f;
+    if constexpr (FUSE & FUSE_POOL) {
+      if (ox + 1 >= a.w || oy0 + 1 >= a.h) continue;
+      float pv[2][2];
+#pragma unroll
+      for (int i = 0; i < 2; ++i) {
+        float v0 = ((sr[i][0] + sr[i][1]) + sr[i][2]) + bz;
+        float v1 = ((sr[i][1] - sr[i][2]) - sr[i][3]) + bz;
+        if (a.act == TG_ACT_TANH24) { v0 = apply_act(v0, a.act); v1 = apply_act(v1, a.act); }
+        else { v0 = __builtin_fmaxf(v0, slope * v0); v1 = __builtin_fmaxf(v1, slope * v1); }
+        pv[i][0] = v0; pv[i][1] = v1;
+      }
+      yn[((size_t)oc * (a.h >> 1) + (oy0 >> 1)) * (a.w >> 1) + (ox >> 1)] =
+          fmaxf(fmaxf(pv[0][0], pv[0][1]), fmaxf(pv[1][0], pv[1][1]));
+      continue;
+    }
 #pragma unroll
     for (int i = 0; i < 2; ++i) {
       const int oy = oy0 + i;
@@ -289,7 +348,7 @@
   }
 }
 
-template <int TR>
+template <int TR, int FUSE = 0>
 __global__ __launch_bounds__(256, 3) void conv3x3_wino_kernel(WinoArgs a) {
   int b = blockIdx.x;
   if (a.nblocks > 0) {
@@ -301,7 +360,7 @@
   const int ty = __builtin_amdgcn_readfirstlane(b % a.tiles_y); b /= a.tiles_y;
   const int ocg = __builtin_amdgcn_readfirstlane(b % a.nocg);
   const int n = __builtin_amdgcn_readfirstlane(b / a.nocg);
-  wino_tile<false, TR>(a, tx, ty, ocg, n);
+  wino_tile<false, TR, FUSE>(a, tx, ty, ocg, n);
 }
 
 struct WinoLayer {
@@ -399,7 +458,7 @@
 int conv3x3_wino_launch(const float* x, int64_t x_ns, int c1, const float* x2, int64_t x2_ns, const float* u,
                         const float* bias, const float* res, int64_t res_ns, const float* mask,
                         int64_t mask_ns, float* y, int64_t y_ns, int n, int cin, int cout, int h, int w,
-                        int act, tg_stream_t stream) {
+                        int act, tg_stream_t stream, int fuse) {
   WinoArgs a{};
   a.x = x; a.x2 = x2; a.u = u; a.bias = bias; a.res = res; a.mask = mask; a.y = y;
   a.x_ns = x_ns; a.x2_ns = x2_ns; a.res_ns = res_ns; a.mask_ns = mask_ns; a.y_ns = y_ns;
@@ -424,9 +483,21 @@
   const bool xcd = xcd_env >= 0 ? xcd_env != 0 : blocks >= 512;
   a.nblocks = xcd ? (int)blocks : 0;
   const unsigned grid = xcd ? (unsigned)(8 * ((blocks + 7) / 8)) : (unsigned)blocks;
-  if (tr == 1) hipLaunchKernelGGL(conv3x3_wino_kernel<1>, dim3(grid), dim3(256), 0, (hipStream_t)stream, a);
-  else if (tr == 2) hipLaunchKernelGGL(conv3x3_wino_kernel<2>, dim3(grid), dim3(256), 0, (hipStream_t)stream, a);
-  else hipLaunchKernelGGL(conv3x3_wino_kernel<4>, dim3(grid), dim3(256), 0, (hipStream_t)stream, a);
+  auto go = [&](auto kern) { hipLaunchKernelGGL(kern, dim3(grid), dim3(256), 0, (hipStream_t)stream, a); };
+  if (fuse == FUSE_POOL) {
+    if (tr == 1) go(conv3x3_wino_kernel<1, FUSE_POOL>);
+    else if (tr == 2) go(conv3x3_wino_kernel<2, FUSE_POOL>);
+    else go(conv3x3_wino_kernel<4, FUSE_POOL>);
+  } else if (fuse == FUSE_UP) {
+    if (tr == 1) go(conv3x3_wino_kernel<1, FUSE_UP>);
+    else if (tr == 2) go(conv3x3_wino_kernel<2, FUSE_UP>);
+    else go(conv3x3_wino_kernel<4, FUSE_UP>);
+  } else {
+    TG_REQUIRE(fuse == 0, TG_E_ARG, "conv3x3_wino: fuse=%d (0 | 1 pooled output | 2 up-sampled input)", fuse);
+    if (tr == 1) go(conv3x3_wino_kernel<1>);
+    else if (tr == 2) go(conv3x3_wino_kernel<2>);
+    else go(conv3x3_wino_kernel<4>);
+  }
   return check_launch("conv3x3_wino");
 }
 }
@@ -443,7 +514,22 @@
   TG_REQUIRE(act >= TG_ACT_NONE && act <= TG_ACT_TANH24, TG_E_ARG, "conv3x3_wino: act=%d", act);
   TG_REQUIRE((long long)cin * h * w < (1ll << 29), TG_E_SHAPE, "conv3x3_wino: image too large");
   return conv3x3_wino_launch(x, x_nstride, c1, x2, x2_nstride, u_packed, bias, res, res_nstride, relu_mask,
-                             mask_nstride, y, y_nstride, n, cin, cout, h, w, act, stream);
+                             mask_nstride, y, y_nstride, n, cin, cout, h, w, act, stream, 0);
+}
+
+extern "C" int tg_conv3x3_wino_fwd_fused(const float* x, int64_t x_nstride, const float* u_packed, const float* bias,
+                                         float* y, int64_t y_nstride, int n, int cin, int cout, int h, int w, int act,
+                                         int fuse, tg_stream_t stream) {
+  TG_REQUIRE(x && u_packed && y, TG_E_ARG, "conv3x3_wino_fused: null pointer");
+  TG_REQUIRE(fuse == TG_FUSE_POOL || fuse == TG_FUSE_UP2X, TG_E_ARG, "conv3x3_wino_fused: fuse=%d (TG_FUSE_POOL | TG_FUSE_UP2X)", fuse);
+  TG_REQUIRE(n > 0 && cin > 0 && cout > 0 && h >= 2 && w >= 2, TG_E_SHAPE, "conv3x3_wino_fused: n=%d cin=%d cout=%d h=%d w=%d",
+             n, cin, cout, h, w);
+  TG_REQUIRE(fuse != TG_FUSE_UP2X || (h % 2 == 0 && w % 2 == 0 && h >= 4 && w >= 4), TG_E_SHAPE,
+             "conv3x3_wino_fused: an up-sampled input needs even h, w >= 4 (h=%d w=%d)", h, w);
+  TG_REQUIRE(act >= TG_ACT_NONE && act <= TG_ACT_TANH24, TG_E_ARG, "conv3x3_wino_fused: act=%d", act);
+  TG_REQUIRE((long long)cin * h * w < (1ll << 29), TG_E_SHAPE, "conv3x3_wino_fused: image too large");
+  return conv3x3_wino_launch(x, x_nstride, cin, nullptr, 0, u_packed, bias, nullptr, 0, nullptr, 0, y, y_nstride, n, cin,
+                             cout, h, w, act, stream, fuse);
 }
 
 extern "C" int64_t tg_conv3x3_wino_chain_flag_ints(int n_layers, int n, int h, int w) {
diff --git a/tecogan-pytorch_amd/ops.py b/tecogan-pytorch_amd/ops.py
--- a/tecogan-pytorch_amd/ops.py
+++ b/tecogan-pytorch_amd/ops.py
@@ -1179,6 +1179,50 @@
     return y
 
 
+FUSE_POOL, FUSE_UP2X = 1, 2
+
+
+def conv3x3_wino_fused(x, u_packed, bias, cin, cout, fuse, act=ACT_NONE, out=None):
+    _chk(x, 'x'); _chk(u_packed, 'u_packed')
+    n, c1, xh, xw = x.shape
+    assert c1 == cin and fuse in (FUSE_POOL, FUSE_UP2X)
+    h, w = (2 * xh, 2 * xw) if fuse == FUSE_UP2X else (xh, xw)
+    oh, ow = (h // 2, w // 2) if fuse == FUSE_POOL else (h, w)
+    y = out if out is not None else torch.empty(n, cout, oh, ow, dtype=torch.float32, device=x.device)
+    _chk(y, 'out')
+    L.check(L.lib().tg_conv3x3_wino_fwd_fused(x.data_ptr(), x.stride(0), u_packed.data_ptr(), _ptr(bias), y.data_ptr(),
+                                              y.stride(0), n, cin, cout, h, w, act, fuse, _stream()),
+            'tg_conv3x3_wino_fwd_fused')
+    return y
+
+
+def conv3x3_pool(x, wpk, bias, cin, cout, ocb, act=ACT_NONE, x2=None, out=None):
+    _chk(x, 'x')
+    n, c1, h, w = x.shape
+    if x2 is not None:
+        _chk(x2, 'x2')
+        assert c1 + x2.shape[1] == cin
+    else:
+        assert c1 == cin
+    y = out if out is not None else torch.empty(n, cout, h // 2, w // 2, dtype=torch.float32, device=x.device)
+    _chk(y, 'out')
+    L.check(L.lib().tg_conv3x3_fwd_pool(x.data_ptr(), c1 * h * w, c1, _ptr(x2), 0 if x2 is None else x2.shape[1] * h * w,
+                                        wpk.data_ptr(), ocb, _ptr(bias), y.data_ptr(), y.stride(0), n, cin, cout, h, w,
+                                        act, _stream()), 'tg_conv3x3_fwd_pool')
+    return y
+
+
+def conv3x3_up2x(x, wpk, bias, cin, cout, ocb, act=ACT_NONE, out=None):
+    _chk(x, 'x')
+    n, c1, lh, lw = x.shape
+    assert c1 == cin
+    y = out if out is not None else torch.empty(n, cout, 2 * lh, 2 * lw, dtype=torch.float32, device=x.device)
+    _chk(y, 'out')
+    L.check(L.lib().tg_conv3x3_fwd_up2x(x.data_ptr(), x.stride(0), wpk.data_ptr(), ocb, _ptr(bias), y.data_ptr(),
+                                        y.stride(0), n, cin, cout, 2 * lh, 2 * lw, act, _stream()), 'tg_conv3x3_fwd_up2x')
+    return y
+
+
 class RowChain:
 
     def __init__(self, layers, n, h, w):
```
